# oval-group/GNN_branching

Hardware: NVIDIA B200
Metric: gnn_subdomains_scored_per_sec (higher is better)
Workload: dtype fp16x3 (fp32 accumulate)

## Files before the change

gnn_branching_b200/csrc/gnnb_api.cu:

```cuda
#include <math.h>
#include <stdio.h>
#include <stdlib.h>
#include <string.h>

#include <map>
#include <string>
#include <vector>

#include "gnnb_common.cuh"
#include "gnnb_train.cuh"

using namespace gnnb;

struct gnnb_ctx {
    int device = 0;
    int last_status = 0;
    std::string err;
    int64_t launches = 0;
    int math = GNNB_MATH_TC_FP16X3;
    int chunk = 0;
    int snapshot = 0;
    int fuse = 1;
    int rescore = 0;
    int64_t rescored = 0;
    bool have_gnn = false;
    float* d_gnn = nullptr;
    uint16_t* d_tc = nullptr;
    GnnParams gp{};
    float* d_train = nullptr;
    int64_t n_params = 0;
    size_t po_w[N_LIN] = {0}, po_b[N_LIN] = {0};
    int adam_steps = 0;
    float* train_ws = nullptr;
    size_t train_ws_cap = 0;
    float* kw_ws = nullptr;
    size_t kw_ws_cap = 0;
    int32_t* kw_iscratch = nullptr;
    int kw_iscratch_cap = 0;
    bool have_net = false;
    float* d_net = nullptr;
    std::vector<LayerDev> layers;
    std::vector<PropPlan*> plan_fwd, plan_bwd;
    std::vector<PropPlan*> plan_kw_own;
    std::vector<PropPlan*> plan_kw;
    std::vector<int> n;
    int zero_tap_layer = 0;
    std::vector<LayerTiling> tiling;
    std::vector<RowMap> rowmap;
    int32_t* d_maps = nullptr;
    LayerDev* d_layers = nullptr;
    int32_t* d_hidden_off = nullptr;
    int32_t* d_random_order = nullptr;
    const float** d_ptrs = nullptr;
    std::vector<int> hidden_off;
    int n_hidden = 0;
    std::vector<struct gnnb_queue*> queues;
    int ws_cap = 0;
    bool ws_host_staging = false;
    float* d_ws = nullptr;
    std::vector<float*> mu, relax_f, relax_b;
    std::vector<int32_t*> amb_cnt, amb_base, amb_rows;
    float* nb = nullptr;
    float* ws_scores = nullptr;
    float* ws_best = nullptr;
    int32_t* ws_idx = nullptr;
    struct Staging {
        std::vector<float*> inputs;
        float* mask = nullptr;
        float* best = nullptr;
        int32_t* idx = nullptr;
        float* scores = nullptr;
    } stg[2];
    float* res_best = nullptr;
    int32_t* res_idx = nullptr;
    int64_t res_cap = 0;
    cudaStream_t copy_stream = nullptr;
    cudaEvent_t ev_copied[2] = {nullptr, nullptr}, ev_free[2] = {nullptr, nullptr};
    unsigned long long* d_nan = nullptr;
    int32_t* d_resc = nullptr;
    int resc_cap = 0;
    RowGather* d_gather = nullptr;
    size_t gather_cap = 0;
    std::map<std::string, std::pair<float*, int64_t>> snaps;
    int profile = 0;
    struct Pending { int klass; int64_t rows; cudaEvent_t a, b; };
    std::vector<Pending> pending;
    std::vector<cudaEvent_t> ev_pool;
    double prof_ms[GNNB_K_COUNT] = {0};
    int64_t prof_launches[GNNB_K_COUNT] = {0};
    int64_t prof_rows[GNNB_K_COUNT] = {0};
};

struct gnnb_queue {
    gnnb_ctx* ctx;
    DomainQueue* q;
};

namespace {

int fail(gnnb_ctx* c, int status, const std::string& msg) {
    if (c) { c->last_status = status; c->err = msg; }
    return status;
}

int axis_taps(int i, int ksize, int stride, int pad, int n_out) {
    int t = 0;
    for (int k = 0; k < ksize; ++k) {
        const int a = i + pad - k;
        if (a >= 0 && a % stride == 0 && a / stride < n_out) ++t;
    }
    return t;
}

int first_zero_tap_layer(const std::vector<LayerDev>& layers) {
    for (size_t k = 1; k < layers.size(); ++k) {
        const LayerDev& L = layers[k];
        if (L.kind != GNNB_LAYER_CONV) continue;
        for (int y = 0; y < L.h_in; ++y)
            if (axis_taps(y, L.ksize, L.stride, L.pad, L.h_out) == 0) return (int)k + 1;
        for (int x = 0; x < L.w_in; ++x)
            if (axis_taps(x, L.ksize, L.stride, L.pad, L.w_out) == 0) return (int)k + 1;
    }
    return 0;
}

int check_zero_taps(gnnb_ctx* c) {
    if (!c->zero_tap_layer) return GNNB_OK;
    return fail(c, GNNB_ERR_UNSUPPORTED, "layer " + std::to_string(c->zero_tap_layer) +
                " (conv, stride > kernel) has input positions no tap reaches: the GNN's tap-count normalisation divides by zero");
}

template <class F>
void walk_inputs(const gnnb_frontier& fr, GnnInputs& in, const std::vector<int>& n, F f) {
    const int L = (int)n.size() - 2;
    auto at = [](const float* const* table, int k) { return table ? table[k] : nullptr; };
    for (int k = 0; k <= L + 1; ++k) {
        f(at(fr.lb, k), in.lb[k], (int64_t)n[k]);
        f(at(fr.ub, k), in.ub[k], (int64_t)n[k]);
    }
    for (int k = 0; k < L; ++k) {
        f(at(fr.dual, k), in.dual[k], (int64_t)n[k + 1] * 3);
        f(at(fr.prim_pre, k), in.pre[k], (int64_t)n[k + 1]);
        f(at(fr.prim_post, k), in.post[k], (int64_t)n[k + 1]);
    }
    f(fr.prim_out, in.pout, (int64_t)1);
    f(fr.primal_input, in.pin, (int64_t)n[0]);
    f(fr.wp, in.wp, (int64_t)n[L]);
    f(fr.bp, in.bp, (int64_t)1);
}

int frontier_inputs(gnnb_ctx* ctx, const gnnb_frontier* fr, bool mask, GnnInputs* out) {
    bool ok = !mask || fr->mask;
    walk_inputs(*fr, *out, ctx->n, [&](const float* src, const float*& slot, int64_t) { slot = src; ok = ok && src; });
    return ok ? GNNB_OK : fail(ctx, GNNB_ERR_INVALID, "null frontier array");
}

#define CU(call)                                                                                          \
    do {                                                                                                  \
        cudaError_t e__ = (call);                                                                         \
        if (e__ != cudaSuccess)                                                                           \
            return fail(ctx, GNNB_ERR_CUDA, std::string(#call) + ": " + cudaGetErrorString(e__));         \
    } while (0)

size_t align4(size_t x) { return (x + 3) & ~size_t(3); }

void free_workspace(gnnb_ctx* c) {
    if (c->d_ws) cudaFree(c->d_ws);
    c->d_ws = nullptr;
    c->ws_cap = 0;
    for (auto& kv : c->snaps) cudaFree(kv.second.first);
    c->snaps.clear();
}

int ensure_workspace(gnnb_ctx* ctx, int Bc, bool host_staging) {
    if (ctx->d_ws && ctx->ws_cap >= Bc && (ctx->ws_host_staging || !host_staging)) return GNNB_OK;
    free_workspace(ctx);
    const int L = (int)ctx->layers.size();
    int nmax = 0;
    for (int k = 0; k <= L; ++k) nmax = ctx->n[k] > nmax ? ctx->n[k] : nmax;
    size_t total = 0;
    auto take = [&](size_t elems) { size_t off = total; total += (elems + 63) & ~size_t(63); return off; };
    std::vector<size_t> o_mu(L + 2), o_rf(L + 1), o_rb(L + 1), o_lb(L + 2), o_ub(L + 2), o_du(L), o_pr(L), o_po(L);
    auto wrows = [&](int k) { return (size_t)Bc * (k <= L ? (size_t)ctx->rowmap[k].nslots : 128); };
    for (int k = 0; k <= L + 1; ++k) o_mu[k] = take(wrows(k) * P);
    for (int k = 1; k <= L; ++k) { o_rf[k] = take(wrows(k) * P); o_rb[k] = take(wrows(k) * P); }
    std::vector<size_t> o_ac(L + 1), o_ab(L + 1), o_ar(L + 1);
    for (int k = 1; k <= L; ++k) {
        const size_t rows = wrows(k), nt = rows / 128;
        o_ac[k] = take(nt + 1); o_ab[k] = take(nt + 1); o_ar[k] = take(rows);
    }
    size_t nb_rows = 0;
    for (int k = 0; k <= L; ++k) nb_rows = wrows(k) > nb_rows ? wrows(k) : nb_rows;
    const size_t o_nb = take(nb_rows * P);
    const size_t o_sc = take((size_t)Bc * ctx->n_hidden);
    const size_t o_best = take(Bc), o_idx = take(Bc);
    struct StgOff { std::vector<size_t> inputs; size_t mask, best, idx, sc; } so[2];
    if (host_staging) {
        GnnInputs unused(L);
        for (StgOff& o : so) {
            walk_inputs(gnnb_frontier{}, unused, ctx->n, [&](const float*, const float*&, int64_t per) {
                o.inputs.push_back(take((size_t)Bc * per));
            });
            o.mask = take((size_t)Bc * ctx->n_hidden);
            o.best = take((size_t)Bc * GNNB_TOPK_MAX); o.idx = take((size_t)Bc * GNNB_TOPK_MAX);
            o.sc = take((size_t)Bc * ctx->n_hidden);
        }
    }
    CU(cudaMalloc(&ctx->d_ws, total * sizeof(float)));
    float* base = ctx->d_ws;
    ctx->mu.assign(L + 2, nullptr); ctx->relax_f.assign(L + 1, nullptr); ctx->relax_b.assign(L + 1, nullptr);
    for (int k = 0; k <= L + 1; ++k) ctx->mu[k] = base + o_mu[k];
    for (int k = 1; k <= L; ++k) { ctx->relax_f[k] = base + o_rf[k]; ctx->relax_b[k] = base + o_rb[k]; }
    ctx->amb_cnt.assign(L + 1, nullptr); ctx->amb_base.assign(L + 1, nullptr); ctx->amb_rows.assign(L + 1, nullptr);
    for (int k = 1; k <= L; ++k) {
        ctx->amb_cnt[k] = reinterpret_cast<int32_t*>(base + o_ac[k]);
        ctx->amb_base[k] = reinterpret_cast<int32_t*>(base + o_ab[k]);
        ctx->amb_rows[k] = reinterpret_cast<int32_t*>(base + o_ar[k]);
    }
    ctx->nb = base + o_nb; ctx->ws_scores = base + o_sc; ctx->ws_best = base + o_best;
    ctx->ws_idx = reinterpret_cast<int32_t*>(base + o_idx);
    if (host_staging) {
        for (int i = 0; i < 2; ++i) {
            gnnb_ctx::Staging& g = ctx->stg[i];
            const StgOff& o = so[i];
            g.inputs.clear();
            for (size_t off : o.inputs) g.inputs.push_back(base + off);
            g.mask = base + o.mask;
            g.best = base + o.best; g.idx = reinterpret_cast<int32_t*>(base + o.idx); g.scores = base + o.sc;
        }
        if (!ctx->copy_stream) {
            CU(cudaStreamCreateWithFlags(&ctx->copy_stream, cudaStreamNonBlocking));
            for (int i = 0; i < 2; ++i) {
                CU(cudaEventCreateWithFlags(&ctx->ev_copied[i], cudaEventDisableTiming));
                CU(cudaEventCreateWithFlags(&ctx->ev_free[i], cudaEventDisableTiming));
            }
        }
    }
    ctx->ws_cap = Bc;
    ctx->ws_host_staging = host_staging;
    return GNNB_OK;
}

#define TRY_(expr) do { int s__ = (expr); if (s__ != GNNB_OK) return s__; } while (0)

int snap(gnnb_ctx* ctx, bool on, const std::string& name, const float* src, int64_t numel, cudaStream_t st) {
    if (!on) return GNNB_OK;
    auto it = ctx->snaps.find(name);
    if (it == ctx->snaps.end() || it->second.second < numel) {
        if (it != ctx->snaps.end()) cudaFree(it->second.first);
        float* p = nullptr;
        CU(cudaMalloc(&p, (size_t)numel * sizeof(float)));
        ctx->snaps[name] = std::make_pair(p, numel);
        it = ctx->snaps.find(name);
    }
    it->second.second = numel;
    CU(cudaMemcpyAsync(it->second.first, src, (size_t)numel * sizeof(float), cudaMemcpyDeviceToDevice, st));
    return GNNB_OK;
}

cudaEvent_t prof_event(gnnb_ctx* ctx) {
    if (!ctx->ev_pool.empty()) { cudaEvent_t e = ctx->ev_pool.back(); ctx->ev_pool.pop_back(); return e; }
    cudaEvent_t e = nullptr;
    cudaEventCreate(&e);
    return e;
}

struct ProfScope {
    gnnb_ctx* ctx; cudaStream_t st; cudaEvent_t a = nullptr, b = nullptr; int klass; int64_t rows;
    ProfScope(gnnb_ctx* c, int k, int64_t r, cudaStream_t s) : ctx(c), st(s), klass(k), rows(r) {
        if (ctx->profile) { a = prof_event(ctx); b = prof_event(ctx); cudaEventRecord(a, st); }
    }
    ~ProfScope() {
        if (ctx->profile) { cudaEventRecord(b, st); ctx->pending.push_back({klass, rows, a, b}); }
    }
};

int prof_collect(gnnb_ctx* ctx) {
    if (ctx->pending.empty()) return GNNB_OK;
    CU(cudaDeviceSynchronize());
    for (auto& p : ctx->pending) {
        float ms = 0.f;
        if (cudaEventElapsedTime(&ms, p.a, p.b) == cudaSuccess) {
            ctx->prof_ms[p.klass] += ms;
            ctx->prof_launches[p.klass] += 1;
            ctx->prof_rows[p.klass] += p.rows;
        }
        ctx->ev_pool.push_back(p.a);
        ctx->ev_pool.push_back(p.b);
    }
    ctx->pending.clear();
    return GNNB_OK;
}

int snap_img(gnnb_ctx* ctx, bool on, const std::string& name, const float* img, int k, int Bc, bool piece_major, cudaStream_t st) {
    if (!on) return GNNB_OK;
    const int64_t numel = (int64_t)Bc * ctx->n[k] * P;
    if (ctx->math != GNNB_MATH_TC_FP16X3) return snap(ctx, on, name, img, numel, st);
    TRY_(snap(ctx, on, name, img, numel, st));
    tc_unpack_tile_image(img, ctx->snaps[name].first, ctx->rowmap[k], (int64_t)Bc * ctx->rowmap[k].nslots, piece_major, st);
    return GNNB_OK;
}

#define TRY(expr) do { int s__ = (expr); if (s__ != GNNB_OK) return s__; } while (0)

int run_chunk(gnnb_ctx* ctx, const GnnInputs& in, const float* mask, int Bc, int math, const NanDoms& nd, float* scores, int k,
              float* best_score, int32_t* best_idx, gnnb_winner* winners, cudaStream_t st) {
    const int L = (int)ctx->layers.size();
    const GnnParams& g = ctx->gp;
    const bool tc = math == GNNB_MATH_TC_FP16X3;
    const bool snaps = ctx->snapshot && math == ctx->math;
    int64_t* lc = &ctx->launches;
    auto name = [](const char* fmt, int a, int b) { char buf[64]; snprintf(buf, sizeof buf, fmt, a, b); return std::string(buf); };

    auto R = [&](int k) { return (int64_t)Bc * (tc ? ctx->rowmap[k].nslots : ctx->n[k]); };
    const RowMap nomap{nullptr, 0, 0};
    auto M = [&](int k) { return tc ? ctx->rowmap[k] : nomap; };
    const bool fused = tc && ctx->fuse;

    const bool amb_all = tc && L <= AMB_MAX_LAYERS;
    if (amb_all) {
        ProfScope ps(ctx, GNNB_K_RELAX, 0, st);
        AmbLayers al{};
        al.n = L;
        for (int k = 1; k <= L; ++k) {
            al.lb[k - 1] = in.lb[k]; al.ub[k - 1] = in.ub[k]; al.map[k - 1] = M(k); al.rows[k - 1] = R(k);
            al.cnt[k - 1] = ctx->amb_cnt[k]; al.base[k - 1] = ctx->amb_base[k]; al.out_rows[k - 1] = ctx->amb_rows[k];
        }
        amb_compact_all(al, st, lc);
    }
    {
        std::vector<NodeInputs> nis(L + 1);
        for (int k = 1; k <= L; ++k)
            nis[k] = NodeInputs{in.lb[k], in.ub[k], in.dual[k - 1], in.pre[k - 1], in.post[k - 1], ctx->layers[k - 1].bias_node,
                                ctx->n[k], R(k), ctx->amb_rows[k], ctx->amb_base[k], M(k)};
        if (tc) {
            for (int k0 = 1; k0 <= L; k0 += AMB_MAX_LAYERS) {
                const int nl = (L - k0 + 1) < AMB_MAX_LAYERS ? (L - k0 + 1) : AMB_MAX_LAYERS;
                int64_t nodes = 0;
                for (int k = k0; k < k0 + nl; ++k) {
                    nodes += (int64_t)Bc * ctx->n[k];
                    if (!amb_all) amb_compact(in.lb[k], in.ub[k], M(k), nis[k].rows, ctx->amb_cnt[k], ctx->amb_base[k], ctx->amb_rows[k], st, lc);
                }
                ProfScope ps(ctx, GNNB_K_RELAX, nodes, st);
                tc_relax(g, &nis[k0], &ctx->relax_f[k0], &ctx->relax_b[k0], nl, st, lc);
            }
        }
        for (int k = 1; k <= L; ++k) {
            if (!tc) {
                ProfScope ps(ctx, GNNB_K_RELAX, (int64_t)Bc * ctx->n[k], st);
                simt_relax(g, nis[k], ctx->relax_f[k], ctx->relax_b[k], st, lc);
            }
            TRY(snap(ctx, snaps, name(tc ? "relaxp_f%d" : "relax_f%d", k, 0), ctx->relax_f[k], (int64_t)Bc * ctx->n[k] * P, st));
            TRY(snap(ctx, snaps, name(tc ? "relaxp_b%d" : "relax_b%d", k, 0), ctx->relax_b[k], (int64_t)Bc * ctx->n[k] * P, st));
        }
    }
    {
        ProfScope ps(ctx, GNNB_K_INPUT_EMBED, (int64_t)Bc * ctx->n[0], st);
        if (tc) tc_input_embed(g, in.lb[0], in.pin, in.ub[0], ctx->mu[0], M(0), R(0), st, lc);
        else simt_input_embed(g, in.lb[0], in.pin, in.ub[0], ctx->mu[0], R(0), st, lc);
    }
    TRY(snap_img(ctx, snaps, "mu0_embed", ctx->mu[0], 0, Bc, false, st));

    for (int t = 0; t < g.T; ++t) {
        const bool last = (t == g.T - 1);
        for (int k = 1; k <= L; ++k) {
            const int64_t rows = R(k), nodes = (int64_t)Bc * ctx->n[k];
            if (fused) {
                ProfScope ps(ctx, GNNB_K_LAYER_FWD, nodes, st);
                tc_fused(g, ctx->plan_fwd[k - 1], ctx->mu[k - 1], false, in.lb[k], in.ub[k], ctx->relax_f[k], ctx->amb_base[k],
                         ctx->mu[k], nullptr, M(k), 0, 0, rows, ctx->d_nan, nd, ctx->snapshot ? ctx->nb : nullptr, false, st, lc);
            } else {
                ProfScope ps(ctx, GNNB_K_PROP_FWD, nodes, st);
                if (tc) prop_tc_run(ctx->plan_fwd[k - 1], ctx->mu[k - 1], ctx->nb, Bc, st, lc);
                else prop_forward(ctx->layers[k - 1], ctx->mu[k - 1], ctx->nb, Bc, st, lc);
            }
            TRY(snap_img(ctx, snaps, name("t%d_fwd_nb%d", t, k), ctx->nb, k, Bc, true, st));
            if (!fused) {
                ProfScope ps(ctx, GNNB_K_UPDATE_FWD, nodes, st);
                if (tc) tc_update(g, false, in.lb[k], in.ub[k], ctx->nb, ctx->relax_f[k], ctx->amb_base[k], ctx->mu[k], nullptr, M(k), 0, 0, rows, ctx->d_nan, nd, st, lc);
                else simt_update(g, false, in.lb[k], in.ub[k], ctx->nb, ctx->relax_f[k], ctx->mu[k], nullptr, ctx->n[k], 0, 0, rows, ctx->d_nan, st, lc);
            }
            TRY(snap_img(ctx, snaps, name("t%d_fwd_mu%d", t, k), ctx->mu[k], k, Bc, false, st));
        }
        {
            ProfScope ps(ctx, GNNB_K_OUTPUT, Bc, st);
            output_node(g, in.wp, in.bp, ctx->mu[L], tc, tc ? ctx->rowmap[L].nslots : ctx->n[L], in.lb[L + 1], in.ub[L + 1], in.pout,
                        ctx->mu[L + 1], ctx->n[L], Bc, st, lc);
        }
        TRY(snap(ctx, snaps, name("t%d_mu_out", t, 0), ctx->mu[L + 1], (int64_t)Bc * P, st));
        for (int k = L; k >= 1; --k) {
            const int64_t rows = R(k), nodes = (int64_t)Bc * ctx->n[k];
            float* sc = last ? scores : nullptr;
            float* mu_k = (last && k == 1 && tc && !ctx->snapshot) ? nullptr : ctx->mu[k];
            const bool fused_k = fused && k < L;
            if (fused_k) {
                ProfScope ps(ctx, last ? GNNB_K_LAYER_BWD_SCORE : GNNB_K_LAYER_BWD, nodes, st);
                tc_fused(g, ctx->plan_bwd[k], ctx->mu[k + 1], true, in.lb[k], in.ub[k], ctx->relax_b[k], ctx->amb_base[k],
                         mu_k, sc, M(k), ctx->n_hidden, ctx->hidden_off[k], rows, ctx->d_nan, nd, ctx->snapshot ? ctx->nb : nullptr, false, st, lc);
            } else {
                ProfScope ps(ctx, GNNB_K_PROP_BWD, nodes, st);
                if (k == L && tc) prop_tc_property_backward(in.wp, ctx->mu[L + 1], ctx->nb, ctx->n[L], ctx->rowmap[L].nslots, Bc, st, lc);
                else if (k == L) prop_property_backward(in.wp, ctx->mu[L + 1], ctx->nb, ctx->n[L], Bc, st, lc);
                else if (tc) prop_tc_run(ctx->plan_bwd[k], ctx->mu[k + 1], ctx->nb, Bc, st, lc);
                else prop_backward(ctx->layers[k], ctx->mu[k + 1], ctx->nb, Bc, true, st, lc);
            }
            TRY(snap_img(ctx, snaps, name("t%d_bwd_nb%d", t, k), ctx->nb, k, Bc, true, st));
            if (!fused_k) {
                ProfScope ps(ctx, last ? GNNB_K_UPDATE_BWD_SCORE : GNNB_K_UPDATE_BWD, nodes, st);
                if (tc) tc_update(g, true, in.lb[k], in.ub[k], ctx->nb, ctx->relax_b[k], ctx->amb_base[k], mu_k, sc, M(k), ctx->n_hidden, ctx->hidden_off[k], rows, ctx->d_nan, nd, st, lc);
                else simt_update(g, true, in.lb[k], in.ub[k], ctx->nb, ctx->relax_b[k], ctx->mu[k], sc, ctx->n[k], ctx->n_hidden, ctx->hidden_off[k], rows, ctx->d_nan, st, lc);
            }
            TRY(snap_img(ctx, snaps, name("t%d_bwd_mu%d", t, k), ctx->mu[k], k, Bc, false, st));
        }
        if (!last && fused) {
            ProfScope ps(ctx, GNNB_K_INPUT_UPDATE, (int64_t)Bc * ctx->n[0], st);
            tc_fused(g, ctx->plan_bwd[0], ctx->mu[1], true, in.lb[0], in.ub[0], nullptr, nullptr, ctx->mu[0], nullptr, M(0), 0, 0, R(0),
                     ctx->d_nan, nd, nullptr, true, st, lc);
            TRY(snap_img(ctx, snaps, name("t%d_mu0", t, 0), ctx->mu[0], 0, Bc, false, st));
        } else if (!last) {
            {
                ProfScope ps(ctx, GNNB_K_PROP_BWD, (int64_t)Bc * ctx->n[0], st);
                if (tc) prop_tc_run(ctx->plan_bwd[0], ctx->mu[1], ctx->nb, Bc, st, lc);
                else prop_backward(ctx->layers[0], ctx->mu[1], ctx->nb, Bc, false, st, lc);
            }
            {
                ProfScope ps(ctx, GNNB_K_INPUT_UPDATE, (int64_t)Bc * ctx->n[0], st);
                if (tc) tc_input_update(g, in.lb[0], in.ub[0], ctx->nb, ctx->mu[0], M(0), R(0), st, lc);
                else simt_input_update(g, in.lb[0], in.ub[0], ctx->nb, ctx->mu[0], R(0), st, lc);
            }
            TRY(snap_img(ctx, snaps, name("t%d_mu0", t, 0), ctx->mu[0], 0, Bc, false, st));
        }
    }
    {
        ProfScope ps(ctx, GNNB_K_ARGMAX, Bc, st);
        if (k == 1) masked_argmax(scores, mask, ctx->n_hidden, Bc, best_score, best_idx, winners, st, lc);
        else masked_topk(scores, mask, ctx->n_hidden, Bc, k, best_score, best_idx, st, lc);
    }
    CU(cudaGetLastError());
    return GNNB_OK;
}

int ensure_nan_doms(gnnb_ctx* ctx, int B) {
    if (ctx->resc_cap >= B) return GNNB_OK;
    if (ctx->d_resc) { cudaFree(ctx->d_resc); ctx->d_resc = nullptr; ctx->resc_cap = 0; }
    CU(cudaMalloc(&ctx->d_resc, (1 + 2 * (size_t)B) * sizeof(int32_t)));
    CU(cudaMemset(ctx->d_resc, 0, (1 + 2 * (size_t)B) * sizeof(int32_t)));
    ctx->resc_cap = B;
    return GNNB_OK;
}

int ensure_kw_iscratch(gnnb_ctx* ctx, int B, cudaStream_t st) {
    if (ctx->kw_iscratch_cap >= B) return GNNB_OK;
    if (ctx->kw_iscratch) { CU(cudaStreamSynchronize(st)); cudaFree(ctx->kw_iscratch); ctx->kw_iscratch = nullptr; ctx->kw_iscratch_cap = 0; }
    CU(cudaMalloc(&ctx->kw_iscratch, (3 * (size_t)B + 1) * sizeof(int32_t)));
    ctx->kw_iscratch_cap = B;
    return GNNB_OK;
}

NanDoms nan_doms(gnnb_ctx* ctx) { return NanDoms{ctx->d_resc, ctx->d_resc + 1, ctx->d_resc + 1 + ctx->resc_cap, 0}; }

void reset_nan_doms(gnnb_ctx* ctx, cudaStream_t st) {
    cudaStreamSynchronize(st);
    cudaMemset(ctx->d_resc, 0, (1 + 2 * (size_t)ctx->resc_cap) * sizeof(int32_t));
}

int rescore_flagged(gnnb_ctx* ctx, const gnnb_frontier* in, int chunk, int k, float* best, int32_t* idx, gnnb_winner* winners,
                    float* scores, cudaStream_t st) {
    const bool host = in->mem == GNNB_MEM_HOST;
    const int nh = ctx->n_hidden;
    const NanDoms nd = nan_doms(ctx);
    int32_t count = 0;
    CU(cudaMemcpyAsync(&count, nd.count, sizeof count, cudaMemcpyDeviceToHost, st));
    CU(cudaStreamSynchronize(st));
    ctx->rescored = count;
    if (count == 0) return GNNB_OK;
    std::vector<int32_t> rows;
    if (host) {
        rows.resize(count);
        CU(cudaMemcpyAsync(rows.data(), nd.list, (size_t)count * sizeof(int32_t), cudaMemcpyDeviceToHost, st));
        CU(cudaStreamSynchronize(st));
    }
    CU(cudaMemsetAsync(nd.count, 0, sizeof(int32_t), st));
    CU(cudaMemsetAsync(ctx->d_nan, 0, sizeof(unsigned long long), st));
    gnnb_ctx::Staging& sg = ctx->stg[0];
    std::vector<RowGather> tab;
    GnnInputs cp((int)ctx->layers.size());
    walk_inputs(*in, cp, ctx->n, [&](const float* src, const float*& slot, int64_t per) {
        float* dst = sg.inputs[tab.size()];
        tab.push_back(RowGather{src, dst, per});
        slot = dst;
    });
    tab.push_back(RowGather{in->mask, sg.mask, nh});
    if (!host) {
        if (ctx->gather_cap < tab.size()) {
            if (ctx->d_gather) cudaFree(ctx->d_gather);
            ctx->d_gather = nullptr; ctx->gather_cap = 0;
            CU(cudaMalloc(&ctx->d_gather, tab.size() * sizeof(RowGather)));
            ctx->gather_cap = tab.size();
        }
        CU(cudaMemcpyAsync(ctx->d_gather, tab.data(), tab.size() * sizeof(RowGather), cudaMemcpyHostToDevice, st));
    }
    for (int s0 = 0, Bs = 0; s0 < count; s0 += Bs) {
        Bs = (count - s0) < chunk ? (count - s0) : chunk;
        if (host) {
            for (int i = 0; i < Bs; ++i)
                for (const RowGather& t : tab)
                    CU(cudaMemcpyAsync(t.dst + i * t.per, t.src + rows[s0 + i] * t.per, t.per * sizeof(float), cudaMemcpyHostToDevice, st));
        } else {
            gather_rows(ctx->d_gather, (int)tab.size(), nd.list + s0, Bs, st, &ctx->launches);
        }
        TRY(run_chunk(ctx, cp, sg.mask, Bs, GNNB_MATH_SIMT_FP32, NanDoms{nullptr, nullptr, nullptr, 0}, sg.scores, k, sg.best, sg.idx, nullptr, st));
        scatter_rescored(nd.list + s0, Bs, k, sg.best, sg.idx, sg.scores, nh, best, idx, winners, host ? nullptr : scores, nd.flag, st,
                         &ctx->launches);
        if (host && scores)
            for (int i = 0; i < Bs; ++i)
                CU(cudaMemcpyAsync(scores + (size_t)rows[s0 + i] * nh, sg.scores + (size_t)i * nh, (size_t)nh * sizeof(float),
                                   cudaMemcpyDeviceToHost, st));
    }
    CU(cudaEventRecord(ctx->ev_free[0], st));
    CU(cudaGetLastError());
    return GNNB_OK;
}

int upload_gnn(gnnb_ctx* ctx, const float* const* tensors, int T) {
    std::vector<size_t> o_w(N_LIN), o_b(N_LIN);
    size_t total = 0;
    for (int l = 0; l < N_LIN; ++l) {
        o_w[l] = total; total += align4((size_t)lin_in(l) * lin_out(l));
        o_b[l] = total; total += align4(lin_out(l));
    }
    std::vector<float> blob(total, 0.f);
    for (int l = 0; l < N_LIN; ++l) {
        const int K = lin_in(l), N = lin_out(l);
        const float* W = tensors[2 * l];
        for (int nn = 0; nn < N; ++nn)
            for (int k = 0; k < K; ++k) blob[o_w[l] + (size_t)k * N + nn] = W[(size_t)nn * K + k];
        memcpy(&blob[o_b[l]], tensors[2 * l + 1], sizeof(float) * N);
    }
    std::vector<float> cw((size_t)N_TCLIN * P * P, 0.f), cb((size_t)N_TCLIN * P, 0.f);
    auto compose = [&](int id, int outer, int half, int inner, bool add_outer_bias) {
        const float* Wo = tensors[2 * outer];
        const float* bo = tensors[2 * outer + 1];
        const int Ko = lin_in(outer);
        for (int nn = 0; nn < P; ++nn) {
            double bacc = add_outer_bias ? (double)bo[nn] : 0.0;
            for (int k = 0; k < P; ++k) {
                double acc = 0.0;
                if (inner < 0) acc = Wo[(size_t)nn * Ko + half * P + k];
                else
                    for (int j = 0; j < P; ++j) acc += (double)Wo[(size_t)nn * Ko + half * P + j] * (double)tensors[2 * inner][(size_t)j * P + k];
                cw[((size_t)id * P + nn) * P + k] = (float)acc;
            }
            if (inner >= 0)
                for (int j = 0; j < P; ++j) bacc += (double)Wo[(size_t)nn * Ko + half * P + j] * (double)tensors[2 * inner + 1][j];
            cb[(size_t)id * P + nn] = (float)bacc;
        }
    };
    compose(T_FWD_R, FC4, 0, FC1_1, false);
    compose(T_FWD_C, FC4, 1, FC3_2, true);
    compose(T_BWD_R, BC4, 0, BC2_1, false);
    compose(T_BWD_C, BC4, 1, BC3_1, true);
    compose(T_INP_C, INP_B2, 0, INP_B_1, true);
    compose(T_INP_NB, INP_B2, 1, -1, false);
    std::vector<size_t> o_tc(N_LIN, 0);
    size_t tc_total = 0;
    for (int l = 0; l < N_LIN; ++l)
        if (lin_in(l) >= P && lin_out(l) == P) { o_tc[l] = tc_total; tc_total += (size_t)tc_packed_elems(lin_in(l)); }
    std::vector<size_t> o_tcx(N_TCLIN, 0);
    for (int i = 0; i < N_TCLIN; ++i) { o_tcx[i] = tc_total; tc_total += (size_t)tc_packed_elems(P); }
    std::vector<uint16_t> tcblob(tc_total ? tc_total : 1, 0);
    for (int l = 0; l < N_LIN; ++l)
        if (lin_in(l) >= P && lin_out(l) == P) tc_pack_weight(tensors[2 * l], lin_in(l), &tcblob[o_tc[l]]);
    for (int i = 0; i < N_TCLIN; ++i) tc_pack_weight(&cw[(size_t)i * P * P], P, &tcblob[o_tcx[i]]);
    const size_t o_cb = total;
    total += cb.size();
    blob.resize(total, 0.f);
    memcpy(&blob[o_cb], cb.data(), cb.size() * sizeof(float));
    CU(cudaDeviceSynchronize());
    if (!ctx->d_gnn) CU(cudaMalloc(&ctx->d_gnn, total * sizeof(float)));
    if (!ctx->d_tc) CU(cudaMalloc(&ctx->d_tc, tcblob.size() * sizeof(uint16_t)));
    CU(cudaMemcpy(ctx->d_gnn, blob.data(), total * sizeof(float), cudaMemcpyHostToDevice));
    CU(cudaMemcpy(ctx->d_tc, tcblob.data(), tcblob.size() * sizeof(uint16_t), cudaMemcpyHostToDevice));
    for (int l = 0; l < N_LIN; ++l) {
        ctx->gp.wt[l] = ctx->d_gnn + o_w[l];
        ctx->gp.bias[l] = ctx->d_gnn + o_b[l];
        ctx->gp.tc[l] = (lin_in(l) >= P && lin_out(l) == P) ? ctx->d_tc + o_tc[l] : nullptr;
    }
    for (int i = 0; i < N_TCLIN; ++i) {
        ctx->gp.tcx_w[i] = ctx->d_tc + o_tcx[i];
        ctx->gp.tcx_b[i] = ctx->d_gnn + o_cb + (size_t)i * P;
    }
    ctx->gp.T = T;
    if (!ctx->d_train) {
        size_t np = 0;
        for (int l = 0; l < N_LIN; ++l) {
            ctx->po_w[l] = np; np += align4((size_t)lin_in(l) * lin_out(l));
            ctx->po_b[l] = np; np += align4(lin_out(l));
        }
        ctx->n_params = (int64_t)np;
        CU(cudaMalloc(&ctx->d_train, 4 * np * sizeof(float)));
        CU(cudaMemset(ctx->d_train, 0, 4 * np * sizeof(float)));
        ctx->adam_steps = 0;
    }
    {
        std::vector<float> master((size_t)ctx->n_params, 0.f);
        for (int l = 0; l < N_LIN; ++l) {
            memcpy(&master[ctx->po_w[l]], tensors[2 * l], sizeof(float) * lin_in(l) * lin_out(l));
            memcpy(&master[ctx->po_b[l]], tensors[2 * l + 1], sizeof(float) * lin_out(l));
        }
        CU(cudaMemcpy(ctx->d_train, master.data(), master.size() * sizeof(float), cudaMemcpyHostToDevice));
    }
    ctx->have_gnn = true;
    return GNNB_OK;
}

TrainParams train_params(gnnb_ctx* ctx) {
    TrainParams tp;
    float* grad = ctx->d_train + ctx->n_params;
    for (int l = 0; l < N_LIN; ++l) {
        tp.w[l] = ctx->d_train + ctx->po_w[l]; tp.b[l] = ctx->d_train + ctx->po_b[l];
        tp.dw[l] = grad + ctx->po_w[l]; tp.db[l] = grad + ctx->po_b[l];
    }
    return tp;
}

int download_quarter(gnnb_ctx* ctx, int quarter, float* const* tensors, const int64_t* numels, int n_tensors) {
    if (!ctx || !tensors || !numels) return fail(ctx, GNNB_ERR_INVALID, "null argument");
    if (!ctx->have_gnn) return fail(ctx, GNNB_ERR_STATE, "gnnb_set_gnn_weights must be called first");
    if (n_tensors != 2 * N_LIN) return fail(ctx, GNNB_ERR_INVALID, "expected 52 tensors (weight, bias of 26 linears)");
    for (int l = 0; l < N_LIN; ++l)
        if (numels[2 * l] != (int64_t)lin_in(l) * lin_out(l) || numels[2 * l + 1] != lin_out(l))
            return fail(ctx, GNNB_ERR_INVALID, "tensor " + std::to_string(2 * l) + " has the wrong number of elements");
    CU(cudaSetDevice(ctx->device));
    CU(cudaDeviceSynchronize());
    std::vector<float> host((size_t)ctx->n_params);
    CU(cudaMemcpy(host.data(), ctx->d_train + (size_t)quarter * ctx->n_params, host.size() * sizeof(float), cudaMemcpyDeviceToHost));
    for (int l = 0; l < N_LIN; ++l) {
        memcpy(tensors[2 * l], &host[ctx->po_w[l]], sizeof(float) * lin_in(l) * lin_out(l));
        memcpy(tensors[2 * l + 1], &host[ctx->po_b[l]], sizeof(float) * lin_out(l));
    }
    return GNNB_OK;
}

}

extern "C" {

int gnnb_abi_version(void) { return 1; }

int gnnb_create(gnnb_ctx** out, int device) {
    if (!out) return GNNB_ERR_INVALID;
    *out = nullptr;
    gnnb_ctx* ctx = new gnnb_ctx();
    ctx->device = device;
    cudaError_t e = cudaSetDevice(device);
    if (e != cudaSuccess) { delete ctx; return GNNB_ERR_CUDA; }
    cudaDeviceProp prop;
    e = cudaGetDeviceProperties(&prop, device);
    if (e != cudaSuccess) { delete ctx; return GNNB_ERR_CUDA; }
    if (prop.major != 10) {
        fprintf(stderr, "libgnnb: device %d is sm_%d%d; this library is built for sm_100a (B200) only\n", device, prop.major, prop.minor);
        delete ctx;
        return GNNB_ERR_UNSUPPORTED;
    }
    if (cudaMalloc(&ctx->d_nan, sizeof(unsigned long long)) != cudaSuccess ||
        cudaMemset(ctx->d_nan, 0, sizeof(unsigned long long)) != cudaSuccess ||
        simt_init() != 0 || prop_init(64 * 1024) != 0 || tc_init() != 0 || prop_tc_init() != 0 || kw_init() != 0 || train_init() != 0) {
        fprintf(stderr, "libgnnb: initialisation failed: %s\n", cudaGetErrorString(cudaGetLastError()));
        if (ctx->d_nan) cudaFree(ctx->d_nan);
        delete ctx;
        return GNNB_ERR_CUDA;
    }
    *out = ctx;
    return GNNB_OK;
}

void gnnb_destroy(gnnb_ctx* ctx) {
    if (!ctx) return;
    cudaSetDevice(ctx->device);
    free_workspace(ctx);
    if (ctx->d_gnn) cudaFree(ctx->d_gnn);
    if (ctx->d_tc) cudaFree(ctx->d_tc);
    if (ctx->d_train) cudaFree(ctx->d_train);
    if (ctx->train_ws) cudaFree(ctx->train_ws);
    if (ctx->kw_ws) cudaFree(ctx->kw_ws);
    if (ctx->kw_iscratch) cudaFree(ctx->kw_iscratch);
    if (ctx->d_net) cudaFree(ctx->d_net);
    if (ctx->d_maps) cudaFree(ctx->d_maps);
    if (ctx->d_layers) cudaFree(ctx->d_layers);
    if (ctx->d_hidden_off) cudaFree(ctx->d_hidden_off);
    if (ctx->d_random_order) cudaFree(ctx->d_random_order);
    if (ctx->d_ptrs) cudaFree(ctx->d_ptrs);
    if (ctx->d_nan) cudaFree(ctx->d_nan);
    if (ctx->d_resc) cudaFree(ctx->d_resc);
    if (ctx->d_gather) cudaFree(ctx->d_gather);
    for (PropPlan* p : ctx->plan_fwd) prop_plan_free(p);
    for (PropPlan* p : ctx->plan_bwd) prop_plan_free(p);
    for (PropPlan* p : ctx->plan_kw_own) prop_plan_free(p);
    if (ctx->copy_stream) cudaStreamDestroy(ctx->copy_stream);
    if (ctx->res_best) cudaFree(ctx->res_best);
    if (ctx->res_idx) cudaFree(ctx->res_idx);
    for (int i = 0; i < 2; ++i) { if (ctx->ev_copied[i]) cudaEventDestroy(ctx->ev_copied[i]); if (ctx->ev_free[i]) cudaEventDestroy(ctx->ev_free[i]); }
    for (auto& p : ctx->pending) { cudaEventDestroy(p.a); cudaEventDestroy(p.b); }
    for (auto e : ctx->ev_pool) cudaEventDestroy(e);
    for (gnnb_queue* q : ctx->queues) q->ctx = nullptr;
    delete ctx;
}

int gnnb_set_gnn_weights(gnnb_ctx* ctx, const float* const* tensors, const int64_t* numels, int n_tensors, int T, int p) {
    if (!ctx || !tensors || !numels) return fail(ctx, GNNB_ERR_INVALID, "null argument");
    if (p != P) return fail(ctx, GNNB_ERR_UNSUPPORTED, "embedding size p must be 64");
    if (T < 1) return fail(ctx, GNNB_ERR_INVALID, "T must be >= 1");
    if (n_tensors != 2 * N_LIN) return fail(ctx, GNNB_ERR_INVALID, "expected 52 tensors (weight, bias of 26 linears)");
    for (int l = 0; l < N_LIN; ++l) {
        if (numels[2 * l] != (int64_t)lin_in(l) * lin_out(l) || numels[2 * l + 1] != lin_out(l))
            return fail(ctx, GNNB_ERR_INVALID, "tensor " + std::to_string(2 * l) + " has the wrong number of elements");
    }
    CU(cudaSetDevice(ctx->device));
    return upload_gnn(ctx, tensors, T);
}

int gnnb_set_network(gnnb_ctx* ctx, const gnnb_layer_desc* layers, int n_layers, int c0, int h0, int w0) {
    if (!ctx || !layers || n_layers < 1) return fail(ctx, GNNB_ERR_INVALID, "null argument");
    if (!ctx->queues.empty()) return fail(ctx, GNNB_ERR_STATE, "gnnb_set_network while domain queues of the previous network exist");
    CU(cudaSetDevice(ctx->device));
    std::vector<LayerDev> devs(n_layers);
    std::vector<int> n(n_layers + 2);
    n[0] = c0 * h0 * w0;
    int pc = c0, ph = h0, pw = w0;
    bool flat = false;
    size_t total = 0;
    std::vector<size_t> o_w(n_layers), o_b(n_layers);
    for (int k = 0; k < n_layers; ++k) {
        const gnnb_layer_desc& d = layers[k];
        LayerDev& L = devs[k];
        L.kind = d.kind;
        L.c_in = d.c_in; L.h_in = d.h_in; L.w_in = d.w_in; L.c_out = d.c_out; L.h_out = d.h_out; L.w_out = d.w_out;
        L.ksize = d.ksize; L.stride = d.stride; L.pad = d.pad;
        L.n_in = d.c_in * d.h_in * d.w_in;
        L.n_out = d.c_out * d.h_out * d.w_out;
        if (!d.weight || !d.bias) return fail(ctx, GNNB_ERR_INVALID, "layer weight/bias is null");
        if (L.n_in != n[k]) return fail(ctx, GNNB_ERR_INVALID, "layer " + std::to_string(k) + ": input size does not match the previous layer");
        size_t wn;
        if (d.kind == GNNB_LAYER_CONV) {
            if (flat || d.c_in != pc || d.h_in != ph || d.w_in != pw) return fail(ctx, GNNB_ERR_INVALID, "conv layer input shape mismatch");
            if (d.ksize < 1 || d.stride < 1 || d.pad < 0) return fail(ctx, GNNB_ERR_INVALID, "bad conv geometry");
            if (d.h_out != (d.h_in + 2 * d.pad - d.ksize) / d.stride + 1 || d.w_out != (d.w_in + 2 * d.pad - d.ksize) / d.stride + 1)
                return fail(ctx, GNNB_ERR_INVALID, "conv output shape mismatch");
            if ((d.h_out - 1) * d.stride - 2 * d.pad + d.ksize != d.h_in || (d.w_out - 1) * d.stride - 2 * d.pad + d.ksize != d.w_in)
                return fail(ctx, GNNB_ERR_UNSUPPORTED, "conv geometry needs output_padding in the backward pass");
            if ((size_t)d.c_in * d.ksize * d.ksize * d.c_out * sizeof(float) > 64 * 1024)
                return fail(ctx, GNNB_ERR_UNSUPPORTED, "conv weights exceed the 64 KB shared-memory staging buffer");
            wn = (size_t)d.c_out * d.c_in * d.ksize * d.ksize;
            pc = d.c_out; ph = d.h_out; pw = d.w_out;
        } else if (d.kind == GNNB_LAYER_LINEAR) {
            if (d.h_in != 1 || d.w_in != 1 || d.h_out != 1 || d.w_out != 1) return fail(ctx, GNNB_ERR_INVALID, "linear layers use c_in/c_out only");
            wn = (size_t)L.n_out * L.n_in;
            flat = true;
        } else {
            return fail(ctx, GNNB_ERR_INVALID, "unknown layer kind");
        }
        n[k + 1] = L.n_out;
        o_w[k] = total; total += align4(wn);
        o_b[k] = total; total += align4(L.n_out);
    }
    n[n_layers + 1] = 1;
    std::vector<float> blob(total, 0.f);
    for (int k = 0; k < n_layers; ++k) {
        const gnnb_layer_desc& d = layers[k];
        const LayerDev& L = devs[k];
        const size_t wn = d.kind == GNNB_LAYER_CONV ? (size_t)d.c_out * d.c_in * d.ksize * d.ksize : (size_t)L.n_out * L.n_in;
        memcpy(&blob[o_w[k]], d.weight, wn * sizeof(float));
        const int per = d.kind == GNNB_LAYER_CONV ? d.h_out * d.w_out : 1;
        for (int j = 0; j < L.n_out; ++j) blob[o_b[k] + j] = d.bias[j / per];
    }
    struct Staged {
        float* d_net = nullptr;
        int32_t* d_maps = nullptr;
        LayerDev* d_layers = nullptr;
        int32_t *d_hidden_off = nullptr, *d_random_order = nullptr;
        const float** d_ptrs = nullptr;
        std::vector<PropPlan*> plan_fwd, plan_bwd, plan_kw_own;
        bool keep = false;
        ~Staged() {
            if (keep) return;
            if (d_net) cudaFree(d_net);
            if (d_maps) cudaFree(d_maps);
            if (d_layers) cudaFree(d_layers);
            if (d_hidden_off) cudaFree(d_hidden_off);
            if (d_random_order) cudaFree(d_random_order);
            if (d_ptrs) cudaFree(d_ptrs);
            for (PropPlan* p : plan_fwd) prop_plan_free(p);
            for (PropPlan* p : plan_bwd) prop_plan_free(p);
            for (PropPlan* p : plan_kw_own) prop_plan_free(p);
        }
    } sg;
    CU(cudaMalloc(&sg.d_net, total * sizeof(float)));
    CU(cudaMemcpy(sg.d_net, blob.data(), total * sizeof(float), cudaMemcpyHostToDevice));
    for (int k = 0; k < n_layers; ++k) { devs[k].weight = sg.d_net + o_w[k]; devs[k].bias_node = sg.d_net + o_b[k]; }
    sg.plan_fwd.assign(n_layers, nullptr);
    sg.plan_bwd.assign(n_layers, nullptr);
    sg.plan_kw_own.assign(n_layers, nullptr);
    std::vector<LayerTiling> tiling(n_layers + 1);
    std::vector<RowMap> rowmap(n_layers + 1, RowMap{nullptr, 0, 0});
    tiling[0] = make_tiling(c0, h0, w0);
    for (int k = 0; k < n_layers; ++k)
        tiling[k + 1] = devs[k].kind == GNNB_LAYER_CONV ? make_tiling(devs[k].c_out, devs[k].h_out, devs[k].w_out)
                                                       : make_tiling(devs[k].n_out, 1, 1);
    {
        size_t total_slots = 0;
        for (const LayerTiling& t : tiling) total_slots += t.node_of_slot.size();
        CU(cudaMalloc(&sg.d_maps, total_slots * sizeof(int32_t)));
        size_t off = 0;
        for (int k = 0; k <= n_layers; ++k) {
            const LayerTiling& t = tiling[k];
            CU(cudaMemcpy(sg.d_maps + off, t.node_of_slot.data(), t.node_of_slot.size() * sizeof(int32_t), cudaMemcpyHostToDevice));
            rowmap[k] = RowMap{sg.d_maps + off, n[k], (int)t.node_of_slot.size()};
            off += t.node_of_slot.size();
        }
    }
    for (int k = 0; k < n_layers; ++k) {
        sg.plan_fwd[k] = prop_plan_build(devs[k], layers[k].weight, false, false, tiling[k + 1], tiling[k]);
        sg.plan_bwd[k] = prop_plan_build(devs[k], layers[k].weight, true, k > 0, tiling[k], tiling[k + 1]);
        if (!sg.plan_fwd[k] || !sg.plan_bwd[k]) return fail(ctx, GNNB_ERR_CUDA, "building the propagation plans failed");
        if (k > 0 && devs[k].kind == GNNB_LAYER_CONV) {
            sg.plan_kw_own[k] = prop_plan_build(devs[k], layers[k].weight, true, false, tiling[k], tiling[k + 1]);
            if (!sg.plan_kw_own[k]) return fail(ctx, GNNB_ERR_CUDA, "building the propagation plans failed");
        }
    }
    std::vector<int> hidden_off(n_layers + 2, 0);
    int n_hidden = 0;
    for (int k = 1; k <= n_layers; ++k) { hidden_off[k] = n_hidden; n_hidden += n[k]; }
    CU(cudaMalloc(&sg.d_layers, n_layers * sizeof(LayerDev)));
    CU(cudaMemcpy(sg.d_layers, devs.data(), n_layers * sizeof(LayerDev), cudaMemcpyHostToDevice));
    CU(cudaMalloc(&sg.d_hidden_off, (n_layers + 1) * sizeof(int32_t)));
    CU(cudaMemcpy(sg.d_hidden_off, hidden_off.data() + 1, (n_layers + 1) * sizeof(int32_t), cudaMemcpyHostToDevice));
    CU(cudaMalloc(&sg.d_random_order, n_layers * sizeof(int32_t)));
    CU(cudaMalloc(&sg.d_ptrs, 2 * (n_layers + 2) * sizeof(float*)));
    CU(cudaDeviceSynchronize());
    ctx->have_net = false;
    free_workspace(ctx);
    if (ctx->d_net) cudaFree(ctx->d_net);
    if (ctx->d_maps) cudaFree(ctx->d_maps);
    if (ctx->d_layers) cudaFree(ctx->d_layers);
    if (ctx->d_hidden_off) cudaFree(ctx->d_hidden_off);
    if (ctx->d_random_order) cudaFree(ctx->d_random_order);
    if (ctx->d_ptrs) cudaFree(ctx->d_ptrs);
    for (PropPlan* p : ctx->plan_fwd) prop_plan_free(p);
    for (PropPlan* p : ctx->plan_bwd) prop_plan_free(p);
    for (PropPlan* p : ctx->plan_kw_own) prop_plan_free(p);
    sg.keep = true;
    ctx->d_net = sg.d_net; ctx->d_maps = sg.d_maps; ctx->d_layers = sg.d_layers; ctx->d_hidden_off = sg.d_hidden_off;
    ctx->d_random_order = sg.d_random_order; ctx->d_ptrs = sg.d_ptrs;
    ctx->plan_fwd = sg.plan_fwd; ctx->plan_bwd = sg.plan_bwd; ctx->plan_kw_own = sg.plan_kw_own;
    ctx->plan_kw.assign(n_layers, nullptr);
    for (int k = 0; k < n_layers; ++k) ctx->plan_kw[k] = sg.plan_kw_own[k] ? sg.plan_kw_own[k] : sg.plan_bwd[k];
    ctx->tiling = tiling; ctx->rowmap = rowmap;
    ctx->layers = devs;
    ctx->n = n;
    ctx->zero_tap_layer = first_zero_tap_layer(devs);
    ctx->hidden_off = hidden_off;
    ctx->n_hidden = n_hidden;
    ctx->have_net = true;
    return GNNB_OK;
}

int gnnb_set_option(gnnb_ctx* ctx, const char* key, int64_t value) {
    if (!ctx || !key) return fail(ctx, GNNB_ERR_INVALID, "null argument");
    const std::string k(key);
    if (k == "math") {
        if (value != GNNB_MATH_TC_FP16X3 && value != GNNB_MATH_SIMT_FP32) return fail(ctx, GNNB_ERR_INVALID, "unknown math mode");
        if (value == GNNB_MATH_TC_FP16X3 && !tc_available()) return fail(ctx, GNNB_ERR_UNSUPPORTED, "tensor-core path not built");
        ctx->math = (int)value;
    } else if (k == "chunk") {
        if (value < 0) return fail(ctx, GNNB_ERR_INVALID, "chunk must be >= 0");
        ctx->chunk = (int)value;
    } else if (k == "fuse") {
        ctx->fuse = value ? 1 : 0;
    } else if (k == "snapshot") {
        ctx->snapshot = value ? 1 : 0;
    } else if (k == "profile") {
        ctx->profile = value ? 1 : 0;
    } else if (k == "rescore") {
        ctx->rescore = value ? 1 : 0;
    } else {
        return fail(ctx, GNNB_ERR_INVALID, "unknown option " + k);
    }
    return GNNB_OK;
}

int64_t gnnb_get_option(gnnb_ctx* ctx, const char* key) {
    if (!ctx || !key) return -1;
    const std::string k(key);
    if (k == "math") return ctx->math;
    if (k == "chunk") return ctx->chunk;
    if (k == "snapshot") return ctx->snapshot;
    if (k == "fuse") return ctx->fuse;
    if (k == "profile") return ctx->profile;
    if (k == "rescore") return ctx->rescore;
    if (k == "rescored") return ctx->rescored;
    if (k == "n_hidden") return ctx->n_hidden;
    if (k == "workspace_domains") return ctx->ws_cap;
    if (k.rfind("plan_density_pct_", 0) == 0) {
        const bool bwd = k[17] == 'b';
        const size_t i = (size_t)atoi(k.c_str() + 18);
        const auto& v = bwd ? ctx->plan_bwd : ctx->plan_fwd;
        return i < v.size() ? (int64_t)(100.0 * prop_plan_density(v[i])) : -1;
    }
    return -1;
}

static int score_impl(gnnb_ctx* ctx, const gnnb_frontier* in, int k, float* best_score, int32_t* best_idx, gnnb_winner* winners,
                      float* scores, void* stream) {
    if (!ctx || !in || ((!best_score || !best_idx) && !winners)) return fail(ctx, GNNB_ERR_INVALID, "null argument");
    if (!ctx->have_gnn || !ctx->have_net) return fail(ctx, GNNB_ERR_STATE, "gnnb_set_gnn_weights and gnnb_set_network must be called first");
    if (in->B < 0) return fail(ctx, GNNB_ERR_INVALID, "negative batch");
    ctx->rescored = 0;
    TRY(check_zero_taps(ctx));
    if (in->B == 0) return GNNB_OK;
    GnnInputs cp((int)ctx->layers.size());
    TRY(frontier_inputs(ctx, in, true, &cp));
    CU(cudaSetDevice(ctx->device));
    cudaStream_t st = (cudaStream_t)stream;
    const bool host = in->mem == GNNB_MEM_HOST;
    int chunk = ctx->chunk > 0 ? ctx->chunk : 1024;
    if (chunk > in->B) chunk = in->B;
    const bool resc = ctx->rescore && ctx->math == GNNB_MATH_TC_FP16X3;
    TRY(ensure_workspace(ctx, chunk, host || resc));
    NanDoms nd{nullptr, nullptr, nullptr, 0};
    if (resc) {
        TRY(ensure_nan_doms(ctx, in->B));
        nd = nan_doms(ctx);
    }
    const int64_t n_res = (int64_t)in->B * k;
    if (host && !winners && ctx->res_cap < n_res) {
        if (ctx->res_best) cudaFree(ctx->res_best);
        if (ctx->res_idx) cudaFree(ctx->res_idx);
        ctx->res_best = nullptr; ctx->res_idx = nullptr; ctx->res_cap = 0;
        CU(cudaMalloc(&ctx->res_best, (size_t)n_res * sizeof(float)));
        CU(cudaMalloc(&ctx->res_idx, (size_t)n_res * sizeof(int32_t)));
        ctx->res_cap = n_res;
    }

    int wave = 0, ramp = host ? (chunk < 128 ? chunk : 128) : chunk;
    for (int c0 = 0, Bc = 0; c0 < in->B; c0 += Bc, ++wave) {
        Bc = (in->B - c0) < ramp ? (in->B - c0) : ramp;
        ramp = ramp + ramp / 2 > chunk ? chunk : ramp + ramp / 2;
        gnnb_ctx::Staging& sg = ctx->stg[wave & 1];
        cudaStream_t cs = host ? ctx->copy_stream : st;
        if (host) CU(cudaStreamWaitEvent(cs, ctx->ev_free[wave & 1], 0));
        auto stage = [&](const float* src, float* dst, size_t per_domain) -> const float* {
            const float* p = src + (size_t)c0 * per_domain;
            if (!host) return p;
            cudaMemcpyAsync(dst, p, (size_t)Bc * per_domain * sizeof(float), cudaMemcpyHostToDevice, cs);
            return dst;
        };
        size_t a = 0;
        walk_inputs(*in, cp, ctx->n, [&](const float* src, const float*& slot, int64_t per) {
            slot = stage(src, host ? sg.inputs[a++] : nullptr, per);
        });
        const float* mask = stage(in->mask, sg.mask, ctx->n_hidden);
        CU(cudaGetLastError());
        if (host) {
            CU(cudaEventRecord(ctx->ev_copied[wave & 1], cs));
            CU(cudaStreamWaitEvent(st, ctx->ev_copied[wave & 1], 0));
        }

        float* d_scores = host ? sg.scores : (scores ? scores + (size_t)c0 * ctx->n_hidden : ctx->ws_scores);
        float* d_best = winners ? nullptr : (host ? ctx->res_best : best_score) + (size_t)c0 * k;
        int32_t* d_idx = winners ? nullptr : (host ? ctx->res_idx : best_idx) + (size_t)c0 * k;
        {
            nd.dom0 = c0;
            const int rc = run_chunk(ctx, cp, mask, Bc, ctx->math, nd, d_scores, k, d_best, d_idx, winners ? winners + c0 : nullptr, st);
            if (rc != GNNB_OK) {
                if (host) cudaStreamSynchronize(ctx->copy_stream);
                cudaStreamSynchronize(st);
                if (resc) reset_nan_doms(ctx, st);
                return rc;
            }
        }
        if (host) {
            if (scores)
                CU(cudaMemcpyAsync(scores + (size_t)c0 * ctx->n_hidden, d_scores, (size_t)Bc * ctx->n_hidden * sizeof(float),
                                   cudaMemcpyDeviceToHost, st));
            CU(cudaEventRecord(ctx->ev_free[wave & 1], st));
        }
    }
    if (resc) {
        const int rc = rescore_flagged(ctx, in, chunk, k, winners ? nullptr : (host ? ctx->res_best : best_score),
                                       winners ? nullptr : (host ? ctx->res_idx : best_idx), winners, scores, st);
        if (rc != GNNB_OK) {
            reset_nan_doms(ctx, st);
            return rc;
        }
    }
    if (host) {
        if (!winners) {
            CU(cudaMemcpyAsync(best_score, ctx->res_best, (size_t)n_res * sizeof(float), cudaMemcpyDeviceToHost, st));
            CU(cudaMemcpyAsync(best_idx, ctx->res_idx, (size_t)n_res * sizeof(int32_t), cudaMemcpyDeviceToHost, st));
        }
        return gnnb_check(ctx, stream, nullptr);
    }
    return GNNB_OK;
}

int gnnb_score(gnnb_ctx* ctx, const gnnb_frontier* in, float* best_score, int32_t* best_idx, float* scores, void* stream) {
    if (!best_score || !best_idx) return fail(ctx, GNNB_ERR_INVALID, "null argument");
    return score_impl(ctx, in, 1, best_score, best_idx, nullptr, scores, stream);
}

int gnnb_score_winners(gnnb_ctx* ctx, const gnnb_frontier* in, gnnb_winner* winners, float* scores, void* stream) {
    if (!winners) return fail(ctx, GNNB_ERR_INVALID, "null argument");
    if (in && in->mem == GNNB_MEM_HOST && scores) return fail(ctx, GNNB_ERR_INVALID, "dense scores of a HOST frontier: use gnnb_score");
    return score_impl(ctx, in, 1, nullptr, nullptr, winners, scores, stream);
}

int gnnb_score_topk(gnnb_ctx* ctx, const gnnb_frontier* in, int32_t k, float* top_score, int32_t* top_idx, float* scores, void* stream) {
    if (k < 1 || k > GNNB_TOPK_MAX) return fail(ctx, GNNB_ERR_INVALID, "k must be in [1, GNNB_TOPK_MAX]");
    if (!top_score || !top_idx) return fail(ctx, GNNB_ERR_INVALID, "null argument");
    return score_impl(ctx, in, k, top_score, top_idx, nullptr, scores, stream);
}

int gnnb_topk(gnnb_ctx* ctx, int32_t B, int32_t n, const float* scores, const float* mask, int32_t k, float* top_score,
              int32_t* top_idx, void* stream) {
    if (!ctx) return GNNB_ERR_INVALID;
    if (k < 1 || k > GNNB_TOPK_MAX) return fail(ctx, GNNB_ERR_INVALID, "k must be in [1, GNNB_TOPK_MAX]");
    if (!scores || !top_score || !top_idx) return fail(ctx, GNNB_ERR_INVALID, "null argument");
    if (B < 0 || n < 0) return fail(ctx, GNNB_ERR_INVALID, "negative size");
    if (B == 0) return GNNB_OK;
    CU(cudaSetDevice(ctx->device));
    cudaStream_t st = (cudaStream_t)stream;
    {
        ProfScope ps(ctx, GNNB_K_ARGMAX, B, st);
        masked_topk(scores, mask, n, B, k, top_score, top_idx, st, &ctx->launches);
    }
    CU(cudaGetLastError());
    return GNNB_OK;
}

int gnnb_babsr(gnnb_ctx* ctx, const gnnb_frontier* in, int32_t sparsest_layer, float decision_threshold,
               const int32_t* random_order, const int32_t* icp_counter_in, int32_t* decision, int32_t* icp_counter_out,
               int32_t* kind, float* scores, void* stream) {
    if (!ctx || !in || !random_order || !decision || !icp_counter_out) return fail(ctx, GNNB_ERR_INVALID, "null argument");
    if (!ctx->have_net) return fail(ctx, GNNB_ERR_STATE, "gnnb_set_network must be called first");
    if (in->B < 0) return fail(ctx, GNNB_ERR_INVALID, "negative batch");
    if (in->B == 0) return GNNB_OK;
    if (!in->lb || !in->ub || !in->wp || !in->mask) return fail(ctx, GNNB_ERR_INVALID, "null frontier field");
    const int L = (int)ctx->layers.size(), B = in->B;
    if (L > babsr_max_layers()) return fail(ctx, GNNB_ERR_UNSUPPORTED, "too many layers for the BaBSR kernel");
    CU(cudaSetDevice(ctx->device));
    cudaStream_t st = (cudaStream_t)stream;
    const bool host = in->mem == GNNB_MEM_HOST;
    const std::vector<int>& n = ctx->n;
    int nmax = 0;
    for (int k = 0; k <= L; ++k) nmax = n[k] > nmax ? n[k] : nmax;
    float* tmp = nullptr;
    std::vector<const float*> ptrs(2 * (L + 2), nullptr);
    const float *d_wp = in->wp, *d_mask = in->mask;
    const int32_t* d_cin = icp_counter_in;
    int32_t *d_dec = decision, *d_cout = icp_counter_out, *d_kind = kind;
    float* d_scores = scores;
    if (host) {
        size_t total = 0;
        auto take = [&](size_t elems) { size_t o = total; total += align4(elems); return o; };
        std::vector<size_t> o_lb(L + 2), o_ub(L + 2);
        for (int k = 1; k <= L; ++k) { o_lb[k] = take((size_t)B * n[k]); o_ub[k] = take((size_t)B * n[k]); }
        const size_t o_wp = take((size_t)B * n[L]), o_mask = take((size_t)B * ctx->n_hidden), o_cin = take(B), o_dec = take(2 * (size_t)B),
                     o_cout = take(B), o_kind = take(B), o_sc = take(scores ? (size_t)B * ctx->n_hidden : 0);
        CU(cudaMalloc(&tmp, total * sizeof(float)));
        auto up = [&](size_t off, const void* src, size_t elems) {
            cudaMemcpyAsync(tmp + off, src, elems * sizeof(float), cudaMemcpyHostToDevice, st);
            return tmp + off;
        };
        for (int k = 1; k <= L; ++k) {
            if (!in->lb[k] || !in->ub[k]) { cudaFree(tmp); return fail(ctx, GNNB_ERR_INVALID, "null bound array"); }
            ptrs[k] = up(o_lb[k], in->lb[k], (size_t)B * n[k]);
            ptrs[L + 2 + k] = up(o_ub[k], in->ub[k], (size_t)B * n[k]);
        }
        d_wp = up(o_wp, in->wp, (size_t)B * n[L]);
        d_mask = up(o_mask, in->mask, (size_t)B * ctx->n_hidden);
        d_cin = icp_counter_in ? reinterpret_cast<const int32_t*>(up(o_cin, icp_counter_in, B)) : nullptr;
        d_dec = reinterpret_cast<int32_t*>(tmp + o_dec); d_cout = reinterpret_cast<int32_t*>(tmp + o_cout);
        d_kind = kind ? reinterpret_cast<int32_t*>(tmp + o_kind) : nullptr;
        d_scores = scores ? tmp + o_sc : nullptr;
    } else {
        for (int k = 1; k <= L; ++k) {
            if (!in->lb[k] || !in->ub[k]) return fail(ctx, GNNB_ERR_INVALID, "null bound array");
            ptrs[k] = in->lb[k];
            ptrs[L + 2 + k] = in->ub[k];
        }
    }
    cudaError_t e = cudaMemcpyAsync(ctx->d_ptrs, ptrs.data(), ptrs.size() * sizeof(float*), cudaMemcpyHostToDevice, st);
    if (e == cudaSuccess) e = cudaMemcpyAsync(ctx->d_random_order, random_order, L * sizeof(int32_t), cudaMemcpyHostToDevice, st);
    int rc = 0;
    if (e == cudaSuccess)
        rc = babsr_run(ctx->d_layers, L, ctx->n_hidden, nmax, ctx->d_ptrs, ctx->d_ptrs + (L + 2), d_wp, d_mask, ctx->d_hidden_off,
                       ctx->d_random_order, d_cin, sparsest_layer, decision_threshold, d_dec, d_cout, d_kind, d_scores, B, st,
                       &ctx->launches);
    if (e == cudaSuccess && rc == 0 && host) {
        cudaMemcpyAsync(decision, d_dec, 2 * (size_t)B * sizeof(int32_t), cudaMemcpyDeviceToHost, st);
        cudaMemcpyAsync(icp_counter_out, d_cout, (size_t)B * sizeof(int32_t), cudaMemcpyDeviceToHost, st);
        if (kind) cudaMemcpyAsync(kind, d_kind, (size_t)B * sizeof(int32_t), cudaMemcpyDeviceToHost, st);
        if (scores) cudaMemcpyAsync(scores, d_scores, (size_t)B * ctx->n_hidden * sizeof(float), cudaMemcpyDeviceToHost, st);
        e = cudaStreamSynchronize(st);
    }
    if (tmp) { cudaStreamSynchronize(st); cudaFree(tmp); }
    if (e != cudaSuccess) return fail(ctx, GNNB_ERR_CUDA, std::string("gnnb_babsr: ") + cudaGetErrorString(e));
    if (rc != 0) return fail(ctx, GNNB_ERR_UNSUPPORTED, "a layer is too large for the BaBSR kernel's shared-memory buffers");
    CU(cudaGetLastError());
    return GNNB_OK;
}

int gnnb_score_grad(gnnb_ctx* ctx, const gnnb_frontier* in, int32_t n_terms, const int32_t* term_domain, const int32_t* term_index,
                    const float* term_coeff, float* term_scores, void* stream) {
    if (!ctx || !in || !term_domain || !term_index || !term_coeff) return fail(ctx, GNNB_ERR_INVALID, "null argument");
    if (!ctx->have_gnn || !ctx->have_net) return fail(ctx, GNNB_ERR_STATE, "gnnb_set_gnn_weights and gnnb_set_network must be called first");
    if (in->B < 1 || n_terms < 1) return fail(ctx, GNNB_ERR_INVALID, "need at least one subdomain and one term");
    TRY(check_zero_taps(ctx));
    GnnInputs ti((int)ctx->layers.size());
    TRY(frontier_inputs(ctx, in, false, &ti));
    for (int i = 0; i < n_terms; ++i)
        if (term_domain[i] < 0 || term_domain[i] >= in->B || term_index[i] < 0 || term_index[i] >= ctx->n_hidden)
            return fail(ctx, GNNB_ERR_INVALID, "term " + std::to_string(i) + " is out of range");
    CU(cudaSetDevice(ctx->device));
    cudaStream_t st = (cudaStream_t)stream;
    const int B = in->B;
    float* tmp = nullptr;
    if (in->mem == GNNB_MEM_HOST) {
        size_t total = 0;
        walk_inputs(*in, ti, ctx->n, [&](const float*, const float*&, int64_t per) { total += align4((size_t)B * per); });
        CU(cudaMalloc(&tmp, total * sizeof(float)));
        float* dst = tmp;
        walk_inputs(*in, ti, ctx->n, [&](const float* src, const float*& slot, int64_t per) {
            cudaMemcpyAsync(dst, src, (size_t)B * per * sizeof(float), cudaMemcpyHostToDevice, st);
            slot = dst;
            dst += align4((size_t)B * per);
        });
    }
    cudaMemsetAsync(ctx->d_train + ctx->n_params, 0, (size_t)ctx->n_params * sizeof(float), st);
    std::string err;
    const int rc = train_backward(ctx->gp, train_params(ctx), ctx->layers, ctx->n, ctx->hidden_off, ti, B, n_terms, term_domain, term_index,
                                  term_coeff, term_scores, &ctx->train_ws, &ctx->train_ws_cap, st, &ctx->launches, &err);
    if (tmp) { cudaStreamSynchronize(st); cudaFree(tmp); }
    if (rc != GNNB_OK) return fail(ctx, rc, err);
    return GNNB_OK;
}

int gnnb_get_gradients(gnnb_ctx* ctx, float* const* tensors, const int64_t* numels, int n_tensors) {
    return download_quarter(ctx, 1, tensors, numels, n_tensors);
}

int gnnb_get_gnn_weights(gnnb_ctx* ctx, float* const* tensors, const int64_t* numels, int n_tensors) {
    return download_quarter(ctx, 0, tensors, numels, n_tensors);
}

// ... 291 lines not shown
```

gnn_branching_b200/csrc/gnnb_common.cuh:

```cuda
#pragma once

#include <cuda_runtime.h>
#include <stdint.h>

#include <string>
#include <vector>

#include "../../include/gnnb.h"

namespace gnnb {

constexpr int P = 64;

enum Lin : int {
    INP_F = 0, INP_F_1, INP_B, INP_B_1, INP_B2, INP_B2_2, FC1, FC1_1, FC3, FC3_2, FC4, FC4_2,
    OUT1, OUT2, OUT3, BC1, BC1_1, BC1_2, BC2, BC2_1, BC3, BC3_1, BC4, BC4_1, FNODE, FSCORE, N_LIN
};

__host__ __device__ constexpr int lin_in(int l) {
    return l == INP_F ? 3 : l == INP_B ? 2 : (l == FC1 || l == BC1) ? 7 : l == OUT1 ? 4
         : (l == INP_B2 || l == FC3 || l == FC4 || l == OUT2 || l == BC3 || l == BC4) ? 2 * P
         : l == BC2 ? 3 * P : P;
}
__host__ __device__ constexpr int lin_out(int l) { return l == FSCORE ? 1 : P; }

enum TcLin : int {
    T_FWD_R = 0,
    T_FWD_C,
    T_BWD_R,
    T_BWD_C,
    T_INP_C,
    T_INP_NB,
    N_TCLIN
};

struct GnnParams {
    const float* wt[N_LIN];
    const float* bias[N_LIN];
    const uint16_t* tc[N_LIN];
    const uint16_t* tcx_w[N_TCLIN];
    const float* tcx_b[N_TCLIN];
    int T;
};

struct LayerDev {
    int kind;
    int c_in, h_in, w_in, c_out, h_out, w_out, ksize, stride, pad;
    int n_in, n_out;
    const float* weight;
    const float* bias_node;
};

struct RowMap {
    const int32_t* node_of_slot;
    int n;
    int nslots;
};
__device__ __forceinline__ int64_t natural_row(const RowMap& m, int64_t grow) {
    const int64_t b = grow / m.nslots;
    const int node = __ldg(m.node_of_slot + (grow - b * m.nslots));
    return node < 0 ? -1 : b * m.n + node;
}
struct LayerTiling {
    std::vector<int32_t> node_of_slot, slot_of_node;
    int ntiles = 0;
};
LayerTiling make_tiling(int C, int H, int W);

struct NodeInputs {
    const float* lb;
    const float* ub;
    const float* dual;
    const float* prim_pre;
    const float* prim_post;
    const float* bias_node;
    int n;
    int64_t rows;
    const int32_t* amb_rows;
    const int32_t* amb_base;
    RowMap map;
};

struct NanDoms {
    int32_t* count;
    int32_t* flag;
    int32_t* list;
    int dom0;
};

void simt_relax(const GnnParams& g, const NodeInputs& in, float* relax_f, float* relax_b, cudaStream_t st, int64_t* launches);
void simt_update(const GnnParams& g, bool backward, const float* lb, const float* ub, const float* nb, const float* relax,
                 float* mu_out, float* scores , int n, int64_t score_stride, int64_t score_off, int64_t rows,
                 unsigned long long* nan_count, cudaStream_t st, int64_t* launches);
void simt_input_embed(const GnnParams& g, const float* lb0, const float* x, const float* ub0, float* mu0, int64_t rows,
                      cudaStream_t st, int64_t* launches);
void simt_input_update(const GnnParams& g, const float* lb0, const float* ub0, const float* nb, float* mu0, int64_t rows,
                       cudaStream_t st, int64_t* launches);

int simt_init();

void tc_relax(const GnnParams& g, const NodeInputs* in, float* const* relax_f, float* const* relax_b, int n_layers, cudaStream_t st,
              int64_t* launches);
void tc_update(const GnnParams& g, bool backward, const float* lb, const float* ub, const float* nb, const float* relax,
               const int32_t* amb_base, float* mu_out, float* scores, RowMap map, int64_t score_stride, int64_t score_off, int64_t rows,
               unsigned long long* nan_count, const NanDoms& nan_doms, cudaStream_t st, int64_t* launches);
struct PropPlan;
void tc_fused(const GnnParams& g, const PropPlan* plan, const float* mu_in, bool backward, const float* lb, const float* ub,
              const float* relax, const int32_t* amb_base, float* mu_out, float* scores, RowMap map, int64_t score_stride, int64_t score_off,
              int64_t rows, unsigned long long* nan_count, const NanDoms& nan_doms, float* nb_dbg, bool input_layer, cudaStream_t st,
              int64_t* launches);
void amb_compact(const float* lb, const float* ub, RowMap map, int64_t rows, int32_t* cnt, int32_t* amb_base, int32_t* amb_rows,
                 cudaStream_t st, int64_t* launches);
constexpr int AMB_MAX_LAYERS = 16;
struct AmbLayers {
    const float* lb[AMB_MAX_LAYERS];
    const float* ub[AMB_MAX_LAYERS];
    RowMap map[AMB_MAX_LAYERS];
    int64_t rows[AMB_MAX_LAYERS];
    int32_t* cnt[AMB_MAX_LAYERS];
    int32_t* base[AMB_MAX_LAYERS];
    int32_t* out_rows[AMB_MAX_LAYERS];
    int tile0[AMB_MAX_LAYERS + 1];
    int n;
};
void amb_compact_all(AmbLayers a, cudaStream_t st, int64_t* launches);
void tc_input_embed(const GnnParams& g, const float* lb0, const float* x, const float* ub0, float* mu0, RowMap map, int64_t rows,
                    cudaStream_t st, int64_t* launches);
void tc_input_update(const GnnParams& g, const float* lb0, const float* ub0, const float* nb, float* mu0, RowMap map, int64_t rows,
                     cudaStream_t st, int64_t* launches);
int64_t tc_pack_weight(const float* w_host, int K, uint16_t* dst_host);
int64_t tc_packed_elems(int K);
int tc_init();
bool tc_available();
void tc_unpack_tile_image(const float* img, float* out, RowMap map, int64_t rows, bool piece_major, cudaStream_t st);

int prop_init(int max_smem_bytes);
void prop_forward(const LayerDev& L, const float* mu_prev, float* nb, int Bc, cudaStream_t st, int64_t* launches);
void prop_backward(const LayerDev& L, const float* mu_next, float* nb, int Bc, bool normalise, cudaStream_t st, int64_t* launches);
void prop_property_backward(const float* wp, const float* mu_out, float* nb, int nL, int Bc, cudaStream_t st, int64_t* launches);
void output_node(const GnnParams& g, const float* wp, const float* bp, const float* mu_L, bool mu_image, int mu_stride, const float* lb_out,
                 const float* ub_out, const float* prim_out, float* mu_out, int nL, int Bc, cudaStream_t st, int64_t* launches);
void masked_argmax(const float* scores, const float* mask, int n_hidden, int Bc, float* best_score, int32_t* best_idx,
                   gnnb_winner* winners, cudaStream_t st, int64_t* launches);
void masked_topk(const float* scores, const float* mask, int n, int Bc, int k, float* top_score, int32_t* top_idx, cudaStream_t st,
                 int64_t* launches);
struct RowGather { const float* src; float* dst; int64_t per; };
struct GnnInputs {
    std::vector<const float*> lb, ub;
    std::vector<const float*> dual, pre, post;
    const float *pout = nullptr, *pin = nullptr, *wp = nullptr, *bp = nullptr;
    explicit GnnInputs(int L) : lb(L + 2), ub(L + 2), dual(L), pre(L), post(L) {}
};
void gather_rows(const RowGather* tab, int n_arrays, const int32_t* rows, int n, cudaStream_t st, int64_t* launches);
void scatter_rescored(const int32_t* rows, int n, int k, const float* sub_best, const int32_t* sub_idx, const float* sub_scores,
                      int n_hidden, float* best_score, int32_t* best_idx, gnnb_winner* winners, float* scores, int32_t* flag,
                      cudaStream_t st, int64_t* launches);

struct PropPlan;
int prop_tc_init();
PropPlan* prop_plan_build(const LayerDev& L, const float* host_weight, bool backward, bool normalise, const LayerTiling& out,
                          const LayerTiling& in);
void prop_plan_free(PropPlan* p);
double prop_plan_density(const PropPlan* p);
void prop_tc_run(const PropPlan* plan, const float* mu_in, float* nb_img, int Bc, cudaStream_t st, int64_t* launches);
void prop_tc_property_backward(const float* wp, const float* mu_out, float* nb_img, int nL, int nslots, int Bc, cudaStream_t st, int64_t* launches);

int babsr_max_layers();
int babsr_run(const LayerDev* d_layers, int L, int n_hidden, int nmax, const float* const* d_lb, const float* const* d_ub,
              const float* wp, const float* mask, const int32_t* d_hidden_off, const int32_t* d_random_order,
              const int32_t* counter_in, int sparsest_layer, float threshold, int32_t* decision, int32_t* counter_out,
              int32_t* kind, float* scores, int B, cudaStream_t st, int64_t* launches);

struct DomainQueue;
int queue_create(int device, const std::vector<int>& n, int n_hidden, int64_t capacity, DomainQueue** out, std::string* err);
void queue_destroy(DomainQueue* q);
const std::string& queue_error(const DomainQueue* q);
int64_t queue_size(const DomainQueue* q);
int64_t queue_capacity(const DomainQueue* q);
int queue_global_lb(DomainQueue* q, float* out, cudaStream_t st);
int queue_add(DomainQueue* q, int B, const float* lower, const float* upper, const float* const* lb, const float* const* ub,
              const int8_t* mask, const int32_t* decision, const uint8_t* keep, int32_t* added, cudaStream_t st, int64_t* launches);
int queue_pick(DomainQueue* q, int max_B, float threshold, bool discard, int32_t* picked, float* lower, float* upper, float* const* lb,
               float* const* ub, int8_t* mask, int32_t* decision, cudaStream_t st, int64_t* launches);
int queue_prune(DomainQueue* q, float threshold, cudaStream_t st, int64_t* launches);
float* queue_stage(DomainQueue* q, size_t bytes);

struct KwTc { const std::vector<PropPlan*>* plans; const std::vector<RowMap>* maps; };
int kw_init();
int kw_bounds(const std::vector<LayerDev>& layers, const std::vector<int>& n, int B, const float* x, float eps, const float* wp, const float* bp,
              const float* const* prov_lb, const float* const* prov_ub, float* const* out_lb, float* const* out_ub, const KwTc* tc, float** ws,
              size_t* ws_cap, cudaStream_t st, int64_t* launches, std::string* err);
int child_bounds(const std::vector<LayerDev>& layers, const std::vector<int>& n, int B, const float* x, float eps, const float* wp, const float* bp,
                 const float* const* parent_lb, const float* const* parent_ub, const int32_t* dec_layer, const int32_t* dec_index,
                 const int32_t* choice, float* const* out_lb, float* const* out_ub, int8_t* const* out_mask, int32_t* second_pass,
                 int32_t* iscratch, const KwTc* tc, float** ws, size_t* ws_cap, cudaStream_t st, int64_t* launches, std::string* err);

int root_bounds(const std::vector<LayerDev>& layers, const std::vector<int>& n, int B, const float* x, float eps, const float* wp, const float* bp,
                float* const* out_lb, float* const* out_ub, int8_t* const* out_mask, int32_t* second_pass, int32_t* iscratch, const KwTc* tc,
                float** ws, size_t* ws_cap, cudaStream_t st, int64_t* launches, std::string* err);

struct Ratio { float r0, r1, beta, amb; };
__device__ __forceinline__ Ratio compute_ratio(float l, float u) {
    Ratio r;
    float lt = l - fmaxf(l, 0.0f);
    float ut = fmaxf(u, 0.0f);
    if (u != u) ut = u;
    if (l != l) lt = l;
    r.r0 = __fdiv_rn(ut, __fsub_rn(ut, lt));
    r.beta = __fmul_rn(__fmul_rn(-1.0f, lt), r.r0);
    r.amb = (r.beta > 0.0f) ? 1.0f : 0.0f;
    r.r1 = __fadd_rn(__fmul_rn(__fsub_rn(1.0f, __fmul_rn(2.0f, __fmul_rn(r.r0, r.amb))), r.amb), r.r0);
    return r;
}

}
```

gnn_branching_b200/csrc/gnnb_tc.cu:

```cuda
#include "gnnb_prop_body.cuh"
#include "gnnb_umma.cuh"

namespace gnnb {
namespace {

using namespace tcx;

constexpr uint32_t ACOL = 0, DCOL = 64, WG_COLS = 128;

struct WG {
    uint32_t land;
    uint32_t mbar_mma, mbar_tma;
    uint32_t ph_mma, ph_tma;
    uint32_t tmem;
    uint32_t tmem0;
    uint32_t acol;
    int t;
    int bar_threads;
    int wg;
    bool lead_warp;
};

__device__ __forceinline__ void wg_barrier(const WG& c) { named_bar(1 + c.wg, c.bar_threads); }

__device__ __forceinline__ void issue_ts(const WG& c, uint32_t b_hi, uint32_t b_lo, uint32_t N, uint32_t dcol, bool accumulate) {
    const uint32_t idesc = make_idesc(N);
    const uint32_t d = c.tmem0 + dcol, a = c.tmem0 + c.acol;
#pragma unroll
    for (int pass = 0; pass < 3; ++pass) {
        const uint64_t bd = make_desc(pass == 2 ? b_lo : b_hi);
#pragma unroll
        for (int k = 0; k < 4; ++k)
            umma_ts(d, a + 16 * k + (pass == 1 ? 8 : 0), bd + 2 * k, idesc, (accumulate || pass > 0 || k > 0) ? 1u : 0u);
    }
}
__device__ __forceinline__ void issue_ss(const WG& c, uint32_t b_hi, uint32_t b_lo, uint32_t N, uint32_t dcol, bool accumulate) {
    const uint32_t idesc = make_idesc(N);
    const uint32_t d = c.tmem0 + dcol;
#pragma unroll
    for (int pass = 0; pass < 3; ++pass) {
        const uint64_t ad = make_desc_nosw(pass == 1 ? c.land + APLANE : c.land, NB_PIECE, 128u);
        const uint64_t bd = make_desc(pass == 2 ? b_lo : b_hi);
#pragma unroll
        for (int k = 0; k < 4; ++k)
            umma(d, ad + (uint64_t)(k * ((2 * NB_PIECE) >> 4)), bd + 2 * k, idesc, (accumulate || pass > 0 || k > 0) ? 1u : 0u);
    }
}

__device__ __forceinline__ void gemm_sync(const WG& c) {
    tmem_st_wait();
    tc_fence_before();
    wg_barrier(c);
}
__device__ __forceinline__ void gemm_finish(WG& c) {
    mbar_wait(c.mbar_mma, c.ph_mma);
    c.ph_mma ^= 1u;
    tc_fence_after();
}
__device__ __forceinline__ void gemm_ts_start(WG& c, uint32_t b_hi, uint32_t b_lo, uint32_t N, uint32_t dcol, bool accumulate = false) {
    gemm_sync(c);
    if (c.lead_warp) {
        tc_fence_after();
        if (elect_one()) {
            issue_ts(c, b_hi, b_lo, N, dcol, accumulate);
            umma_commit(c.mbar_mma);
        }
        __syncwarp();
    }
}
__device__ __forceinline__ void gemm_ts(WG& c, uint32_t b_hi, uint32_t b_lo, uint32_t N, uint32_t dcol, bool accumulate = false) {
    gemm_ts_start(c, b_hi, b_lo, N, dcol, accumulate);
    gemm_finish(c);
}
__device__ __forceinline__ void gemm_ss(WG& c, uint32_t b_hi, uint32_t b_lo, uint32_t N, uint32_t dcol, bool accumulate = false) {
    gemm_sync(c);
    if (c.lead_warp) {
        tc_fence_after();
        mbar_wait(c.mbar_tma, c.ph_tma);
        if (elect_one()) {
            issue_ss(c, b_hi, b_lo, N, dcol, accumulate);
            umma_commit(c.mbar_mma);
        }
        __syncwarp();
    }
    c.ph_tma ^= 1u;
    gemm_finish(c);
}

__device__ __forceinline__ void a_store16(const WG& c, int ks, const float (&v)[16]) {
    uint32_t w[16];
#pragma unroll
    for (int i = 0; i < 8; ++i) split2(v[2 * i], v[2 * i + 1], w[i], w[8 + i]);
    tmem_st16(c.tmem + c.acol + 16 * ks, w);
}

__device__ __forceinline__ float4 lds4(const float* p) { return *reinterpret_cast<const float4*>(p); }
__device__ __forceinline__ void lds16(const float* p, float (&b)[16]) {
#pragma unroll
    for (int i = 0; i < 4; ++i) {
        const float4 x = lds4(p + 4 * i);
        b[4 * i] = x.x; b[4 * i + 1] = x.y; b[4 * i + 2] = x.z; b[4 * i + 3] = x.w;
    }
}

__device__ __forceinline__ float4 ldg4_now(const float* p) {
    float4 v;
    asm volatile("ld.global.nc.v4.f32 {%0, %1, %2, %3}, [%4];" : "=f"(v.x), "=f"(v.y), "=f"(v.z), "=f"(v.w) : "l"(p));
    return v;
}
__device__ __forceinline__ float ldg1_now(const float* p) {
    float v;
    asm volatile("ld.global.nc.f32 %0, [%1];" : "=f"(v) : "l"(p));
    return v;
}
__device__ __forceinline__ int ldgi_now(const int32_t* p) {
    int v;
    asm volatile("ld.global.nc.s32 %0, [%1];" : "=r"(v) : "l"(p));
    return v;
}

template <bool RELU>
__device__ __forceinline__ void epilogue_to_a(const WG& c, uint32_t dcol, const float* __restrict__ bias_s) {
#pragma unroll
    for (int q = 0; q < 4; ++q) {
        float v[16], bb[16];
        tmem_ld16_sync(c.tmem + dcol + q * 16, v);
        lds16(bias_s + q * 16, bb);
#pragma unroll
        for (int j = 0; j < 16; ++j) {
            const float x = v[j] + bb[j];
            v[j] = RELU ? relu_nan(x) : x;
        }
        a_store16(c, q, v);
    }
}

template <int K>
__device__ __forceinline__ void first_layer_to_a(const WG& c, const float (&feat)[K], const float* __restrict__ wt_s,
                                                 const float* __restrict__ bias_s) {
#pragma unroll
    for (int q = 0; q < 4; ++q) {
        float o[16];
        lds16(bias_s + q * 16, o);
#pragma unroll
        for (int k = 0; k < K; ++k) {
            float w[16];
            lds16(wt_s + k * P + q * 16, w);
#pragma unroll
            for (int j = 0; j < 16; ++j) o[j] = fmaf(feat[k], w[j], o[j]);
        }
#pragma unroll
        for (int j = 0; j < 16; ++j) o[j] = relu_nan(o[j]);
        a_store16(c, q, o);
    }
}

template <bool TO_A>
__device__ __forceinline__ bool epilogue_to_mu(const WG& c, uint32_t dcol, const float* __restrict__ bias_s, float rowscale,
                                               bool valid, bool stage = true) {
    bool bad = false;
#pragma unroll
    for (int q = 0; q < 4; ++q) {
        float v[16], bb[16];
        tmem_ld16_sync(c.tmem + dcol + q * 16, v);
        lds16(bias_s + q * 16, bb);
#pragma unroll
        for (int j = 0; j < 16; ++j) {
            v[j] = (v[j] + bb[j]) * rowscale;
            bad |= (v[j] != v[j]);
        }
        uint32_t w[16];
#pragma unroll
        for (int i = 0; i < 8; ++i) split2(v[2 * i], v[2 * i + 1], w[i], w[8 + i]);
#pragma unroll
        for (int h = 0; h < 2 && stage; ++h) {
            const uint32_t off = swz((uint32_t)c.t, (uint32_t)(q * 2 + h));
            asm volatile("st.shared.v4.b32 [%0], {%1, %2, %3, %4};" ::"r"(c.land + off), "r"(w[4 * h]), "r"(w[4 * h + 1]),
                         "r"(w[4 * h + 2]), "r"(w[4 * h + 3]) : "memory");
            asm volatile("st.shared.v4.b32 [%0], {%1, %2, %3, %4};" ::"r"(c.land + APLANE + off), "r"(w[8 + 4 * h]),
                         "r"(w[8 + 4 * h + 1]), "r"(w[8 + 4 * h + 2]), "r"(w[8 + 4 * h + 3]) : "memory");
        }
        if (TO_A) tmem_st16(c.tmem + c.acol + 16 * q, w);
    }
    return bad && valid;
}
__device__ __forceinline__ void commit_tile(const WG& c, void* dst_tile) {
    fence_proxy_async();
    wg_barrier(c);
    if (c.t == 0) bulk_s2g(dst_tile, c.land, ABUF);
}
__device__ __forceinline__ void request_nb(const WG& c, const void* src) {
    if (c.t == 0) {
        bulk_wait_read();
        mbar_expect_tx(c.mbar_tma, ABUF);
        bulk_g2s(c.land, src, ABUF, c.mbar_tma);
    }
}

__device__ __forceinline__ void epilogue_to_rlx(const WG& c, uint32_t dcol, const float* __restrict__ bias_s, float rowscale,
                                                float* __restrict__ dst_tile) {
#pragma unroll
    for (int q = 0; q < 4; ++q) {
        float v[16], bb[16];
        tmem_ld16_sync(c.tmem + dcol + q * 16, v);
        lds16(bias_s + q * 16, bb);
#pragma unroll
        for (int h = 0; h < 4; ++h) {
            const float4 o = make_float4((v[h * 4 + 0] + bb[h * 4 + 0]) * rowscale, (v[h * 4 + 1] + bb[h * 4 + 1]) * rowscale,
                                         (v[h * 4 + 2] + bb[h * 4 + 2]) * rowscale, (v[h * 4 + 3] + bb[h * 4 + 3]) * rowscale);
            *reinterpret_cast<float4*>(dst_tile + ((size_t)(q * 4 + h) * TILE + c.t) * 4) = o;
        }
    }
}

constexpr int NWG = 4;
struct Tail {
    float bias[6][P];
    float w_small[2][8 * P];
    float vec[P];
    uint64_t mbar[1 + 2 * NWG];
    uint32_t tmem_slot;
    int32_t wcnt[NWG][4];
};

struct CtaSetup {
    unsigned char* base;
    uint32_t w;
    Tail* tail;
    uint32_t tmem_base;
};

__device__ __forceinline__ unsigned char* smem_dyn() {
    extern __shared__ unsigned char smem_raw_[];
    return smem_raw_;
}

template <bool LAND, int NW>
__device__ __forceinline__ CtaSetup cta_setup(unsigned char* smem_raw, uint32_t wbytes, const uint16_t* const (&wsrc)[NW],
                                              const uint32_t (&woff)[NW], const uint32_t (&wlen)[NW]) {
    CtaSetup s;
    s.base = smem_raw + ((1024u - (smem_u32(smem_raw) & 1023u)) & 1023u);
    s.w = smem_u32(s.base);
    s.tail = reinterpret_cast<Tail*>(s.base + wbytes + (LAND ? NWG * ABUF : 0));
    if (threadIdx.x == 0) {
        for (int i = 0; i < 1 + 2 * NWG; ++i) mbar_init(smem_u32(&s.tail->mbar[i]), 1);
        fence_mbar_init();
    }
    __syncwarp();
    if (threadIdx.x < 32) tmem_alloc(smem_u32(&s.tail->tmem_slot), 512);
    tc_fence_before();
    __syncthreads();
    tc_fence_after();
    s.tmem_base = s.tail->tmem_slot;
    if (threadIdx.x == 0) {
        const uint32_t mb = smem_u32(&s.tail->mbar[0]);
        uint32_t total = 0;
        for (int i = 0; i < NW; ++i) total += wlen[i];
        mbar_expect_tx(mb, total);
        for (int i = 0; i < NW; ++i) bulk_g2s(s.w + woff[i], wsrc[i], wlen[i], mb);
    }
    return s;
}
__device__ __forceinline__ WG make_wg(const CtaSetup& s, uint32_t wbytes) {
    WG c;
    c.wg = uniform((int)(threadIdx.x >> 7));
    c.lead_warp = (uniform((int)(threadIdx.x >> 5)) & 3) == 0;
    c.t = threadIdx.x & 127;
    c.land = s.w + wbytes + (uint32_t)c.wg * ABUF;
    c.mbar_mma = smem_u32(&s.tail->mbar[1 + 2 * c.wg]);
    c.mbar_tma = smem_u32(&s.tail->mbar[2 + 2 * c.wg]);
    c.ph_mma = 0;
    c.ph_tma = 0;
    c.acol = ACOL;
    c.bar_threads = 128;
    c.tmem0 = ((uint32_t)uniform((int)s.tmem_base) & 0x0000FFFFu) + (uint32_t)c.wg * WG_COLS;
    c.tmem = s.tmem_base + ((uint32_t)((c.t >> 5) * 32) << 16) + (uint32_t)c.wg * WG_COLS;
    return c;
}
__device__ __forceinline__ void cta_teardown(const CtaSetup& s) {
    tc_fence_before();
    __syncthreads();
    if (threadIdx.x < 32) tmem_dealloc(s.tmem_base, 512);
}
__device__ __forceinline__ void copy_vec(float* dst, const float* __restrict__ src, int n, float scale = ASCALE) {
    for (int i = threadIdx.x; i < n; i += blockDim.x) dst[i] = src[i] * scale;
}

constexpr uint32_t UPD_W3 = 0, UPD_WC = 4 * WPLANE, UPD_W42 = 6 * WPLANE, UPD_FN = 8 * WPLANE, UPD_WBYTES = 10 * WPLANE;

struct UpdArgs {
    GnnParams g;
    int backward;
    const float *lb, *ub;
    const uint16_t* nb_img;
    const float* rlx;
    const int32_t* amb_base;
    uint16_t* mu_out;
    float* scores;
    RowMap map;
    int64_t score_stride, score_off;
    int Bc;
    unsigned long long* nan_count;
    NanDoms nan_doms;
};

__device__ __forceinline__ bool nan_watch(const NanDoms& nd, int dom, bool nan_row) {
    if (nan_row && nd.flag != nullptr && atomicExch(nd.flag + nd.dom0 + dom, 1) == 0) nd.list[atomicAdd(nd.count, 1)] = nd.dom0 + dom;
    return nan_row;
}

__device__ __forceinline__ void update_body(const UpdArgs& a, unsigned char* smem_raw, int rank, int nranks, bool pdl = false) {
    const GnnParams& g = a.g;
    const int backward = a.backward;
    const float* __restrict__ lb = a.lb;
    const float* __restrict__ ub = a.ub;
    const uint16_t* __restrict__ nb_img = a.nb_img;
    const float* __restrict__ rlx = a.rlx;
    const int32_t* __restrict__ amb_base = a.amb_base;
    uint16_t* __restrict__ mu_out = a.mu_out;
    float* __restrict__ scores = a.scores;
    const RowMap map = a.map;
    const int64_t score_stride = a.score_stride, score_off = a.score_off;
    const int l3 = backward ? BC3 : FC3, l4b = backward ? BC4_1 : FC4_2, lc = backward ? T_BWD_C : T_FWD_C;
    const uint16_t* const wsrc[4] = {g.tc[l3], g.tcx_w[lc], g.tc[l4b], g.tc[FNODE]};
    const uint32_t woff[4] = {UPD_W3, UPD_WC, UPD_W42, UPD_FN};
    const uint32_t wlen[4] = {4 * WPLANE, 2 * WPLANE, 2 * WPLANE, 2 * WPLANE};
    CtaSetup s = cta_setup<true, 4>(smem_raw, UPD_WBYTES, wsrc, woff, wlen);
    Tail& tl = *s.tail;
    copy_vec(tl.bias[0], g.bias[l3], P); copy_vec(tl.bias[1], g.tcx_b[lc], P); copy_vec(tl.bias[2], g.bias[l4b], P);
    copy_vec(tl.bias[3], g.bias[FNODE], P); copy_vec(tl.vec, g.wt[FSCORE], P, 1.0f);
    const float bscore = g.bias[FSCORE][0];
    __syncthreads();
    mbar_wait(smem_u32(&tl.mbar[0]), 0);
    if (pdl) { pdl_trigger(); pdl_wait(); }
    WG c = make_wg(s, UPD_WBYTES);
    const uint32_t W = s.w;
    const int tiles_per_dom = map.nslots / TILE;
    const int64_t nitems = (int64_t)tiles_per_dom * ((a.Bc + NWG - 1) / NWG);
    bool bad = false;
    GNNB_TR_DECL;
    int64_t nrow_n = -1;
    float l_n = 0.f, u_n = 1.f;
    int slot0_n = 0;
    auto fetch_row = [&](int64_t it) {
        nrow_n = -1; l_n = 0.f; u_n = 1.f; slot0_n = 0;
        if (it >= nitems) return;
        const int d = (int)(it / tiles_per_dom) * NWG + c.wg;
        if (d >= a.Bc) return;
        const int64_t tl_ = (int64_t)d * tiles_per_dom + it % tiles_per_dom;
        nrow_n = natural_row(map, tl_ * TILE + c.t);
        if (nrow_n >= 0) { l_n = ldg1_now(lb + nrow_n); u_n = ldg1_now(ub + nrow_n); }
        slot0_n = __ldg(amb_base + tl_);
    };
    fetch_row(rank);
    for (int64_t item = rank; item < nitems; item += nranks) {
        const int dom = (int)(item / tiles_per_dom) * NWG + c.wg;
        const int64_t nrow = nrow_n;
        const float l = l_n, u = u_n;
        const int slot0 = slot0_n;
        if (dom >= a.Bc) {
            fetch_row(item + nranks);
            continue;
        }
        const int64_t tile = (int64_t)dom * tiles_per_dom + item % tiles_per_dom;
        const int64_t row0 = tile * TILE, grow = row0 + c.t;
        request_nb(c, nb_img + (size_t)tile * (ABUF / 2));
        fetch_row(item + nranks);
        const Ratio q = compute_ratio(l, u);
        const float gate = (q.r0 != 0.0f) ? 1.0f : 0.0f;
        const bool amb = (q.amb != 0.0f) && nrow >= 0;
        const unsigned bal = __ballot_sync(0xffffffffu, amb);
        if ((c.t & 31) == 0) tl.wcnt[c.wg][c.t >> 5] = __popc(bal);
        GNNB_TR(0);
        gemm_ss(c, W + UPD_W3, W + UPD_W3 + 2 * WPLANE, 128, 0);
        GNNB_TR(1);
        if (c.t == 0 && item + nranks < nitems) {
            const int64_t nitem = item + nranks;
            const int ndom = (int)(nitem / tiles_per_dom) * NWG + c.wg;
            if (ndom < a.Bc) prefetch_l2(nb_img + (size_t)((int64_t)ndom * tiles_per_dom + nitem % tiles_per_dom) * (ABUF / 2), ABUF);
        }
        int slot = slot0 + __popc(bal & ((1u << (c.t & 31)) - 1u));
#pragma unroll
        for (int w = 0; w < 3; ++w) slot += (w < (c.t >> 5)) ? tl.wcnt[c.wg][w] : 0;
        const float* rt = rlx + (size_t)(slot >> 7) * (TILE * P) + (size_t)(slot & (TILE - 1)) * 4;
        if (amb) {
#pragma unroll
            for (int i = 0; i < 16; ++i) asm volatile("prefetch.global.L2 [%0];" ::"l"(rt + (size_t)i * (TILE * 4)));
        }
#pragma unroll
        for (int qd = 0; qd < 4; ++qd) {
            float a[16], b[16], bb[16];
            {
                uint32_t ra[16], rb[16];
                tmem_ld16(c.tmem + qd * 16, ra);
                tmem_ld16(c.tmem + 64 + qd * 16, rb);
                tmem_wait16(ra, a);
                tmem_wait16(rb, b);
            }
            lds16(tl.bias[0] + qd * 16, bb);
#pragma unroll
            for (int j = 0; j < 16; ++j) a[j] = relu_nan(fmaf(q.r0, a[j], fmaf(q.r1, b[j], bb[j])));
            a_store16(c, qd, a);
        }
        GNNB_TR(2);
        gemm_ts_start(c, W + UPD_WC, W + UPD_WC + WPLANE, 64, DCOL);
        float4 rx[16];
        {
#pragma unroll
            for (int i = 0; i < 16; ++i) rx[i] = amb ? ldg4_now(rt + (size_t)i * (TILE * 4)) : make_float4(0.f, 0.f, 0.f, 0.f);
        }
        gemm_finish(c);
        GNNB_TR(3);
#pragma unroll
        for (int qd = 0; qd < 4; ++qd) {
            float v[16], bb[16];
            tmem_ld16_sync(c.tmem + DCOL + qd * 16, v);
            lds16(tl.bias[1] + qd * 16, bb);
#pragma unroll
            for (int h = 0; h < 4; ++h) {
                const float4 x = rx[qd * 4 + h];
                v[h * 4 + 0] = relu_nan(v[h * 4 + 0] + x.x + bb[h * 4 + 0]);
                v[h * 4 + 1] = relu_nan(v[h * 4 + 1] + x.y + bb[h * 4 + 1]);
                v[h * 4 + 2] = relu_nan(v[h * 4 + 2] + x.z + bb[h * 4 + 2]);
                v[h * 4 + 3] = relu_nan(v[h * 4 + 3] + x.w + bb[h * 4 + 3]);
            }
            a_store16(c, qd, v);
        }
        GNNB_TR(4);
        gemm_ts(c, W + UPD_W42, W + UPD_W42 + WPLANE, 64, DCOL);
        GNNB_TR(5);
        if (scores == nullptr) {
            bad |= nan_watch(a.nan_doms, dom, epilogue_to_mu<false>(c, DCOL, tl.bias[2], gate, nrow >= 0));
            commit_tile(c, mu_out + (size_t)tile * (ABUF / 2));
        } else {
            bad |= nan_watch(a.nan_doms, dom, epilogue_to_mu<true>(c, DCOL, tl.bias[2], gate, nrow >= 0, mu_out != nullptr));
            if (mu_out != nullptr) commit_tile(c, mu_out + (size_t)tile * (ABUF / 2));
            gemm_ts(c, W + UPD_FN, W + UPD_FN + WPLANE, 64, DCOL);
            float sc = 0.f;
#pragma unroll
            for (int qd = 0; qd < 4; ++qd) {
                float v[16], bb[16], ww[16];
                tmem_ld16_sync(c.tmem + DCOL + qd * 16, v);
                lds16(tl.bias[3] + qd * 16, bb);
                lds16(tl.vec + qd * 16, ww);
#pragma unroll
                for (int j = 0; j < 16; ++j) sc = fmaf(relu_nan(v[j] + bb[j]), ww[j], sc);
            }
            if (nrow >= 0) scores[(nrow / map.n) * score_stride + score_off + (nrow % map.n)] = fmaf(sc, AINV, bscore);
        }
        GNNB_TR(6);
        GNNB_TR_NEXT();
    }
    GNNB_TR_PRINT("update[top gemm1 epi1 gemm2 epi2 gemm3 epi3]", 7);
    if (bad) atomicAdd(a.nan_count, 1ULL);
    if (c.t == 0) bulk_wait_all();
    cta_teardown(s);
}

__global__ void __launch_bounds__(128 * NWG, 1) k_tc_update(UpdArgs a) {
    update_body(a, smem_dyn(), (int)blockIdx.x, (int)gridDim.x, true);
}

namespace fz {
constexpr int PD = 2;
constexpr int CW = 2;
constexpr int NS_MAX = 8;
constexpr uint32_t W_KS = 8192;
constexpr uint32_t B_ROWS = 16;
constexpr uint32_t B_DOM = B_ROWS * 128;
constexpr uint32_t B_PLANE = PD * B_DOM;
constexpr uint32_t B_STAGE = 2 * B_PLANE;
constexpr uint32_t STAGE = W_KS + B_STAGE;
constexpr uint32_t STG_PLANE = 32 * 128;
constexpr uint32_t STG_WARP = 2 * STG_PLANE;
constexpr uint32_t STG_BYTES = CW * 4 * STG_WARP;
constexpr uint32_t INF_WN = 0, INF_WI = 2 * WPLANE, INF_B22 = 4 * WPLANE;
constexpr int THREADS = 768;
constexpr int GATHER_WARP0 = 2, GATHER_WARPS = 6, CHAIN_WARP0 = 8;
constexpr uint32_t ACC_COL = 0, ACC_WIN = PD * 64, D_COL = 256, D_WIN = 128;

struct Tail {
    float bias[4][P];
    float vec[P];
    uint64_t wts, full[NS_MAX], empty[NS_MAX], acc_full[2], acc_empty[2], mma[CW];
    uint32_t tmem_slot;
    int32_t wcnt[2 * CW][4];
};
constexpr size_t smem_for(uint32_t wbytes, int staging, int n_stages) {
    return 1024 + wbytes + (size_t)staging * (STG_BYTES / 2) + (size_t)n_stages * STAGE + sizeof(Tail);
}
constexpr size_t SMEM_MAX = 232448;
}

struct FusedArgs {
    UpdArgs u;
    PropPlanDev plan;
    const uint16_t* mu_in;
    uint16_t* nb_dbg;
    int n_stages;
    int mma_group;
    int input_layer;
};

__device__ __forceinline__ void tmem_ld32_sync(uint32_t taddr, float (&v0)[16], float (&v1)[16]) {
    uint32_t r0[16], r1[16];
    tmem_ld16(taddr, r0);
    tmem_ld16(taddr + 16, r1);
    tmem_wait16(r0, v0);
    tmem_wait16(r1, v1);
}

__device__ __forceinline__ void split16(const float (&v)[16], uint32_t (&w)[16]) {
#pragma unroll
    for (int i = 0; i < 8; ++i) split2(v[2 * i], v[2 * i + 1], w[i], w[8 + i]);
}
__device__ __forceinline__ void sts128(uint32_t addr, uint32_t a, uint32_t b, uint32_t c, uint32_t d) {
    asm volatile("st.shared.v4.b32 [%0], {%1, %2, %3, %4};" ::"r"(addr), "r"(a), "r"(b), "r"(c), "r"(d) : "memory");
}

#ifdef GNNB_TRACE
__device__ long long g_e3_trace[4];
#define E3TR(i) do { if (blockIdx.x == 1 && threadIdx.x == fz::CHAIN_WARP0 * 32) { const long long n_ = clock64(); g_e3_trace[i] += n_ - e3t_; e3t_ = n_; } } while (0)
#else
#define E3TR(i) do {} while (0)
#endif
struct NoOp { __device__ __forceinline__ void operator()() const {} };
template <bool TO_A, class Between = NoOp>
__device__ __forceinline__ bool epilogue_to_mu_pair(const WG& c, int h, int pair_bar, uint32_t dcol, const float* __restrict__ bias_s,
                                                    float rowscale, bool valid, unsigned char* img, uint32_t stage, Between between = Between()) {
    bool bad = false;
#ifdef GNNB_TRACE
    long long e3t_ = clock64();
#endif
    const uint32_t rl = (uint32_t)c.t & 31u;
    const bool issuer = h == 0 && rl == 0;
    unsigned char* dst = img + ((uint32_t)c.t >> 5) * fz::STG_PLANE;
    uint32_t lo[TO_A ? 16 : 1];
    if (img != nullptr) {
        if (issuer) bulk_wait_read();
        named_bar(pair_bar, 64);
    }
    E3TR(0);
    {
        float v0[16], v1[16];
        tmem_ld32_sync(c.tmem + dcol + h * 32, v0, v1);
        E3TR(1);
#pragma unroll
        for (int qq = 0; qq < 2; ++qq) {
            float (&v)[16] = qq ? v1 : v0;
            const int q = 2 * h + qq;
            float bb[16];
            lds16(bias_s + q * 16, bb);
#pragma unroll
            for (int j = 0; j < 16; ++j) {
                v[j] = (v[j] + bb[j]) * rowscale;
                bad |= (v[j] != v[j]);
            }
            uint32_t w[16];
            split16(v, w);
            if (img != nullptr) {
                const uint32_t o0 = stage + swz(rl, (uint32_t)(2 * q)), o1 = stage + swz(rl, (uint32_t)(2 * q + 1));
                sts128(o0, w[0], w[1], w[2], w[3]);
                sts128(o1, w[4], w[5], w[6], w[7]);
                if (!TO_A) {
                    sts128(o0 + fz::STG_PLANE, w[8], w[9], w[10], w[11]);
                    sts128(o1 + fz::STG_PLANE, w[12], w[13], w[14], w[15]);
                }
            }
            if (TO_A) {
#pragma unroll
                for (int i = 0; i < 8; ++i) lo[qq * 8 + i] = w[8 + i];
                tmem_st16(c.tmem + c.acol + 16 * q, w);
            }
        }
    }
    E3TR(2);
    if (!TO_A) between();
    if (img != nullptr) {
        fence_proxy_async();
        named_bar(pair_bar, 64);
        if (!TO_A) {
            if (issuer) {
                bulk_s2g_nocommit(dst, stage, fz::STG_PLANE);
                bulk_s2g_nocommit(dst + APLANE, stage + fz::STG_PLANE, fz::STG_PLANE);
                bulk_commit();
            }
        } else {
            if (issuer) { bulk_s2g(dst, stage, fz::STG_PLANE); bulk_wait_read(); }
            named_bar(pair_bar, 64);
#pragma unroll
            for (int qq = 0; qq < 2; ++qq) {
                const int q = 2 * h + qq;
                sts128(stage + swz(rl, (uint32_t)(2 * q)), lo[qq * 8], lo[qq * 8 + 1], lo[qq * 8 + 2], lo[qq * 8 + 3]);
                sts128(stage + swz(rl, (uint32_t)(2 * q + 1)), lo[qq * 8 + 4], lo[qq * 8 + 5], lo[qq * 8 + 6], lo[qq * 8 + 7]);
            }
            fence_proxy_async();
            named_bar(pair_bar, 64);
            if (issuer) bulk_s2g(dst + APLANE, stage, fz::STG_PLANE);
        }
    }
    E3TR(3);
    return bad && valid;
}

struct ItemCursor {
    int pair, tile, dq, dr, ntiles, npairs;
    __device__ __forceinline__ ItemCursor(int rank, int nranks, int ntiles_, int npairs_)
        : pair(rank / ntiles_), tile(rank % ntiles_), dq(nranks / ntiles_), dr(nranks % ntiles_), ntiles(ntiles_), npairs(npairs_) {}
    __device__ __forceinline__ bool valid() const { return pair < npairs; }
    __device__ __forceinline__ void next() {
        tile += dr; pair += dq;
        if (tile >= ntiles) { tile -= ntiles; ++pair; }
    }
};

template <bool INPUT_LAYER>
__device__ __forceinline__ void fused_body(const FusedArgs& fa) {
    using namespace fz;
    const UpdArgs& a = fa.u;
    const GnnParams& g = a.g;
    const PropPlanDev& plan = fa.plan;
    const bool with_score = a.scores != nullptr;
    const uint32_t wbytes = with_score ? UPD_WBYTES : UPD_FN;
    const int NS = fa.n_stages;
    unsigned char* base = smem_dyn();
    base += (1024u - (smem_u32(base) & 1023u)) & 1023u;
    const uint32_t stg_warp = a.mu_out == nullptr ? 0u : (with_score ? STG_PLANE : STG_WARP), stg_bytes = CW * 4 * stg_warp;
    const uint32_t W = smem_u32(base), stg = W + wbytes, ring = stg + stg_bytes;
    fz::Tail* tl = reinterpret_cast<fz::Tail*>(base + wbytes + stg_bytes + (size_t)NS * STAGE);
    const int warp = uniform((int)(threadIdx.x >> 5)), lane = threadIdx.x & 31;
    if (threadIdx.x == 0) {
        mbar_init(smem_u32(&tl->wts), 1);
        for (int i = 0; i < NS; ++i) { mbar_init(smem_u32(&tl->full[i]), 1 + 32); mbar_init(smem_u32(&tl->empty[i]), 1); }
        for (int i = 0; i < 2; ++i) { mbar_init(smem_u32(&tl->acc_full[i]), 1); mbar_init(smem_u32(&tl->acc_empty[i]), PD); }
        for (int i = 0; i < CW; ++i) mbar_init(smem_u32(&tl->mma[i]), 1);
        fence_mbar_init();
    }
    __syncwarp();
    if (warp == 0) tmem_alloc(smem_u32(&tl->tmem_slot), 512);
    tc_fence_before();
    __syncthreads();
    tc_fence_after();
    const uint32_t tmem_base = tl->tmem_slot;
    const int l3 = a.backward ? BC3 : FC3, l4b = a.backward ? BC4_1 : FC4_2, lc = a.backward ? T_BWD_C : T_FWD_C;
    constexpr bool inp = INPUT_LAYER;
    if (threadIdx.x == 0) {
        const uint32_t mb = smem_u32(&tl->wts);
        if (!inp) {
            mbar_expect_tx(mb, wbytes);
            bulk_g2s(W + UPD_W3, g.tc[l3], 4 * WPLANE, mb);
            bulk_g2s(W + UPD_WC, g.tcx_w[lc], 2 * WPLANE, mb);
            bulk_g2s(W + UPD_W42, g.tc[l4b], 2 * WPLANE, mb);
            if (with_score) bulk_g2s(W + UPD_FN, g.tc[FNODE], 2 * WPLANE, mb);
        } else {
            mbar_expect_tx(mb, 6 * WPLANE);
            bulk_g2s(W + INF_WN, g.tcx_w[T_INP_NB], 2 * WPLANE, mb);
            bulk_g2s(W + INF_WI, g.tcx_w[T_INP_C], 2 * WPLANE, mb);
            bulk_g2s(W + INF_B22, g.tc[INP_B2_2], 2 * WPLANE, mb);
        }
    }
    if (!inp) {
        copy_vec(tl->bias[0], g.bias[l3], P); copy_vec(tl->bias[1], g.tcx_b[lc], P); copy_vec(tl->bias[2], g.bias[l4b], P);
        copy_vec(tl->bias[3], g.bias[FNODE], P); copy_vec(tl->vec, g.wt[FSCORE], P, 1.0f);
    } else {
        copy_vec(tl->bias[0], g.tcx_b[T_INP_C], P); copy_vec(tl->bias[1], g.bias[INP_B2_2], P); copy_vec(tl->bias[2], g.bias[INP_B], P);
        copy_vec(tl->bias[3], g.wt[INP_B], 2 * P);
    }
    __syncthreads();
    pdl_trigger(); pdl_wait();

    const int ntiles = plan.ntiles, npairs = (a.Bc + PD - 1) / PD;
    const int rank = (int)blockIdx.x, nranks = (int)gridDim.x;

    if (warp == 0) {
        if (lane == 0) {
            uint32_t slot = 0, ph = 0;
            for (ItemCursor cur(rank, nranks, ntiles, npairs); cur.valid(); cur.next()) {
                const int ks0 = plan.tile_ks0[cur.tile], ks1 = plan.tile_ks0[cur.tile + 1];
                for (int ks = ks0; ks < ks1; ++ks) {
                    mbar_wait(smem_u32(&tl->empty[slot]), ph ^ 1u);
                    const uint32_t full = smem_u32(&tl->full[slot]);
                    mbar_expect_tx(full, W_KS);
                    bulk_g2s(ring + slot * STAGE, plan.ks_w + (size_t)ks * (W_KS / 2), W_KS, full);
                    if (++slot == (uint32_t)NS) { slot = 0; ph ^= 1u; }
                }
            }
        }
    } else if (warp == 1) {
        const uint32_t idesc = (1u << 4) | (1u << 16) | ((uint32_t)(PD * 64 >> 3) << 17) | ((uint32_t)(TILE >> 4) << 24);
        uint32_t t = 0, it = 0, slot = 0, ph = 0;
        const int group = fa.mma_group;
        const uint64_t d_a_hi = make_desc_nosw(ring, NB_PIECE, 128u), d_a_lo = make_desc_nosw(ring + W_KS / 2, NB_PIECE, 128u);
        const uint64_t d_b_hi = make_desc_mn(ring + W_KS, B_DOM), d_b_lo = make_desc_mn(ring + W_KS + B_PLANE, B_DOM);
        uint32_t lag_slot0 = 0, lag_slot1 = 0, lag_ph0 = 0, lag_ph1 = 0;
        bool have_lag = false, have_prev = false;
#ifdef GNNB_TRACE
        long long t_acc = 0, t_b = 0, t_lag = 0, t_all = clock64(), t0_;
#define FTR_BEGIN() t0_ = clock64()
#define FTR_END(x) x += clock64() - t0_
#else
#define FTR_BEGIN()
#define FTR_END(x)
#endif
        for (ItemCursor cur(rank, nranks, ntiles, npairs); cur.valid(); cur.next(), ++it) {
            const int ks0 = uniform(plan.tile_ks0[cur.tile]), ks1 = uniform(plan.tile_ks0[cur.tile + 1]);
            const uint32_t buf = it & 1u, bufph = (it >> 1) & 1u;
            FTR_BEGIN();
            mbar_wait(smem_u32(&tl->acc_empty[buf]), bufph ^ 1u);
            FTR_END(t_acc);
            tc_fence_after();
            const uint32_t d = (tmem_base & 0x0000FFFFu) + ACC_COL + buf * ACC_WIN;
            uint32_t accum = 0;
            for (int ks = ks0; ks < ks1;) {
                const int n = ks1 - ks < group ? ks1 - ks : group;
                FTR_BEGIN();
                if (have_lag) mbar_wait(smem_u32(&tl->empty[lag_slot0]), lag_ph0);
                FTR_END(t_lag);
                lag_slot0 = lag_slot1; lag_ph0 = lag_ph1; have_lag = have_prev;
                for (int i = 0; i < n; ++i, ++t) {
                    FTR_BEGIN();
                    mbar_wait(smem_u32(&tl->full[slot]), ph);
                    FTR_END(t_b);
                    tc_fence_after();
                    const uint64_t soff = (uint64_t)(slot * (STAGE >> 4));
                    const uint64_t a_hi = d_a_hi + soff, a_lo = d_a_lo + soff, b_hi = d_b_hi + soff, b_lo = d_b_lo + soff;
                    if (elect_one()) {
                        umma(d, a_hi, b_hi, idesc, accum);
                        umma(d, a_lo, b_hi, idesc, 1u);
                        umma(d, a_hi, b_lo, idesc, 1u);
                        umma_commit(smem_u32(&tl->empty[slot]));
                    }
                    __syncwarp();
                    accum = 1u;
                    lag_slot1 = slot; lag_ph1 = ph;
                    if (++slot == (uint32_t)NS) { slot = 0; ph ^= 1u; }
                }
                have_prev = true;
                ks += n;
            }
            if (elect_one()) umma_commit(smem_u32(&tl->acc_full[buf]));
            __syncwarp();
        }
#ifdef GNNB_TRACE
        if (rank == 1 && lane == 0) printf("TRACE fused-mma: items %u ksteps %u total %lld | wait acc_empty %lld, lag %lld, stage full %lld\n", it, t,
                                           clock64() - t_all, t_acc, t_lag, t_b);
#endif
    } else if (warp >= GATHER_WARP0 && warp < GATHER_WARP0 + GATHER_WARPS) {
        const int gw = warp - GATHER_WARP0;
        const int GW = GATHER_WARPS < NS ? GATHER_WARPS : NS;
        const unsigned char* mu_bytes = reinterpret_cast<const unsigned char*>(fa.mu_in);
#ifdef GNNB_TRACE
        long long g_wait = 0, g_all = clock64();
#endif
        uint32_t slot = 0, ph = 0;
        int turn = 0;
        for (ItemCursor cur(rank, nranks, ntiles, npairs); cur.valid(); cur.next()) {
            const int ks0 = __ldg(plan.tile_ks0 + cur.tile), ks1 = __ldg(plan.tile_ks0 + cur.tile + 1);
            const int dm0 = cur.pair * PD;
            const uint32_t jp = (uint32_t)(lane & 7);
            const unsigned char* base0 = mu_bytes + (int64_t)dm0 * (plan.nslots_in >> 7) * (int64_t)ABUF + jp * 16u;
            const uint32_t sz0 = dm0 < a.Bc ? 16u : 0u, sz1 = dm0 + 1 < a.Bc ? 16u : 0u;
            const unsigned char* base1 = sz1 ? base0 + (int64_t)(plan.nslots_in >> 7) * (int64_t)ABUF : base0;
            for (int ks = ks0; ks < ks1; ++ks) {
                const uint32_t slot_ = slot, ph_ = ph;
                const bool mine = turn == gw;
                if (++slot == (uint32_t)NS) { slot = 0; ph ^= 1u; }
                if (++turn == GW) turn = 0;
                if (!mine) continue;
                const int idx = __ldg(plan.ks_rows + (size_t)ks * 16 + (lane & 15));
                const int off = idx < 0 ? -1 : (idx << 7) + ((idx >> 7) << 14);
#ifdef GNNB_TRACE
                const long long g0_ = clock64();
#endif
                mbar_wait(smem_u32(&tl->empty[slot_]), ph_ ^ 1u);
#ifdef GNNB_TRACE
                g_wait += clock64() - g0_;
#endif
                const uint32_t dst0 = ring + slot_ * STAGE + W_KS;
#pragma unroll
                for (int q = 0; q < 4; ++q) {
                    const int k = q * 4 + (lane >> 3);
                    const int o = __shfl_sync(0xffffffffu, off, k);
                    const bool ok = o >= 0;
                    const uint32_t oo = ok ? (uint32_t)o : 0u, r7 = (oo >> 7) & 7u;
                    const uint32_t dst = dst0 + swz((uint32_t)k, jp ^ r7);
                    const uint32_t z0 = ok ? sz0 : 0u, z1 = ok ? sz1 : 0u;
                    cp_async16_sz(dst, base0 + oo, z0);
                    cp_async16_sz(dst + B_PLANE, base0 + oo + APLANE, z0);
                    cp_async16_sz(dst + B_DOM, base1 + oo, z1);
                    cp_async16_sz(dst + B_DOM + B_PLANE, base1 + oo + APLANE, z1);
                }
                cp_async_arrive(smem_u32(&tl->full[slot_]));
            }
        }
#ifdef GNNB_TRACE
        if (rank == 1 && gw == 0 && lane == 0) printf("TRACE fused-gather: total %lld, wait stage empty %lld\n", clock64() - g_all, g_wait);
#endif
    } else if (warp >= CHAIN_WARP0) {
        const float* __restrict__ lb = a.lb;
        const float* __restrict__ ub = a.ub;
        const float* __restrict__ rlx = a.rlx;
        const int32_t* __restrict__ amb_base = a.amb_base;
        float* __restrict__ scores = a.scores;
        const RowMap map = a.map;
        const float bscore = g.bias[FSCORE][0];
        const int cw = warp - CHAIN_WARP0;
        const int j = uniform(cw >> 3), h = uniform((cw >> 2) & 1);
        WG c;
        c.wg = j;
        c.bar_threads = 256;
        c.lead_warp = (cw & 7) == 0;
        c.t = threadIdx.x & 127;
        c.land = 0;
        c.mbar_mma = smem_u32(&tl->mma[j]);
        c.mbar_tma = 0;
        c.ph_mma = 0;
        c.ph_tma = 0;
        c.acol = ACC_COL;
        c.tmem0 = (uint32_t)uniform((int)tmem_base) & 0x0000FFFFu;
        c.tmem = tmem_base + ((uint32_t)((c.t >> 5) * 32) << 16);
        const uint32_t D = D_COL + D_WIN * (uint32_t)j;
        const int pw = j * 4 + (cw & 3);
        const uint32_t stage = stg + (uint32_t)pw * stg_warp;
        const int pair_bar = 3 + pw;
        const int Q0 = 2 * h;
        mbar_wait(smem_u32(&tl->wts), 0);
        bool bad = false;
        int node_n = -1, node_nn = -1;
        float l_n = 0.f, u_n = 1.f;
        int slot0_n = 0;
        auto fetch_node = [&](const ItemCursor& cu) -> int {
            if (!cu.valid() || cu.pair * PD + j >= a.Bc) return -1;
            return ldgi_now(map.node_of_slot + cu.tile * TILE + c.t);
        };
        auto fetch_bounds = [&](const ItemCursor& cu, int node_) {
            node_n = node_; l_n = 0.f; u_n = 1.f; slot0_n = 0;
            if (!cu.valid()) return;
            const int d_ = cu.pair * PD + j;
            if (d_ >= a.Bc) return;
            if (node_ >= 0) { l_n = ldg1_now(lb + (int64_t)d_ * map.n + node_); u_n = ldg1_now(ub + (int64_t)d_ * map.n + node_); }
            if (amb_base != nullptr) slot0_n = ldgi_now(amb_base + (int64_t)d_ * ntiles + cu.tile);
        };
        ItemCursor cur(rank, nranks, ntiles, npairs), cur1 = cur, cur2 = cur;
        cur1.next();
        cur2.next(); cur2.next();
        fetch_bounds(cur, fetch_node(cur));
        node_nn = fetch_node(cur1);
        uint32_t it = 0;
#ifdef GNNB_TRACE
        long long c_wait = 0, c_ph[8] = {0, 0, 0, 0, 0, 0, 0, 0}, c_all = clock64(), c0_;
        int c_tiles = 0;
#define CTR(i) do { const long long n_ = clock64(); c_ph[i] += n_ - c0_; c0_ = n_; } while (0)
#else
#define CTR(i) do {} while (0)
#endif
        auto start_item = [&](const ItemCursor& cu, uint32_t it_, int node_, float l_, float u_) -> bool {
            const uint32_t buf = it_ & 1u, bufph = (it_ >> 1) & 1u;
            const int dom_ = cu.pair * PD + j;
#ifdef GNNB_TRACE
            const long long w0_ = clock64();
#endif
            mbar_wait(smem_u32(&tl->acc_full[buf]), bufph);
#ifdef GNNB_TRACE
            c_wait += clock64() - w0_;
#endif
            tc_fence_after();
            if (dom_ >= a.Bc) {
                if (h == 0 && c.t == 0) mbar_arrive(smem_u32(&tl->acc_empty[buf]));
                return false;
            }
            const int64_t tile = (int64_t)dom_ * ntiles + cu.tile;
            c.acol = ACC_COL + buf * ACC_WIN + 64u * (uint32_t)j;
            {
                unsigned char* dbg = fa.nb_dbg ? reinterpret_cast<unsigned char*>(fa.nb_dbg) + tile * (int64_t)ABUF + (uint32_t)c.t * 16u : nullptr;
                float v0[16], v1[16];
                tmem_ld32_sync(c.tmem + c.acol + h * 32, v0, v1);
#pragma unroll
                for (int qq = 0; qq < 2; ++qq) {
                    const int qd = Q0 + qq;
                    uint32_t w[16];
                    split16(qq ? v1 : v0, w);
                    tmem_st16(c.tmem + c.acol + 16 * qd, w);
                    if (dbg != nullptr) {
#pragma unroll
                        for (int hh = 0; hh < 2; ++hh) {
                            const uint32_t off = (uint32_t)(qd * 2 + hh) * NB_PIECE;
                            *reinterpret_cast<uint4*>(dbg + off) = make_uint4(w[4 * hh], w[4 * hh + 1], w[4 * hh + 2], w[4 * hh + 3]);
                            *reinterpret_cast<uint4*>(dbg + APLANE + off) = make_uint4(w[8 + 4 * hh], w[8 + 4 * hh + 1], w[8 + 4 * hh + 2], w[8 + 4 * hh + 3]);
                        }
                    }
                }
            }
            if (inp) {
                {
                    const float* w0 = &tl->bias[3][0];
#pragma unroll
                    for (int qq = 0; qq < 2; ++qq) {
                        const int qd = Q0 + qq;
                        float o[16], wl[16], wu[16];
                        lds16(tl->bias[2] + qd * 16, o);
                        lds16(w0 + qd * 16, wl);
                        lds16(w0 + P + qd * 16, wu);
#pragma unroll
                        for (int i = 0; i < 16; ++i) o[i] = relu_nan(fmaf(node_ >= 0 ? l_ : 0.f, wl[i], fmaf(node_ >= 0 ? u_ : 0.f, wu[i], o[i])));
                        uint32_t w[16];
                        split16(o, w);
                        tmem_st16(c.tmem + D + 64 + 16 * qd, w);
                    }
                }
                gemm_sync(c);
                if (c.lead_warp) {
                    tc_fence_after();
                    if (elect_one()) {
                        WG c2 = c;
                        c2.acol = D + 64;
                        issue_ts(c, W + INF_WN, W + INF_WN + WPLANE, 64, D, false);
                        issue_ts(c2, W + INF_WI, W + INF_WI + WPLANE, 64, D, true);
                        umma_commit(c.mbar_mma);
                    }
                    __syncwarp();
                }
            } else {
                gemm_ts_start(c, W + UPD_W3, W + UPD_W3 + 2 * WPLANE, 128, D);
            }
            return true;
        };
        bool have = cur.valid() ? start_item(cur, 0, node_n, l_n, u_n) : false;
        for (; cur.valid(); cur.next(), cur1.next(), cur2.next(), ++it) {
            const uint32_t buf = it & 1u;
            const uint32_t acc_empty = smem_u32(&tl->acc_empty[buf]);
            const int dom = cur.pair * PD + j;
            const int node = node_n;
            const float l = l_n, u = u_n;
            const int slot0 = slot0_n;
            fetch_bounds(cur1, node_nn);
            node_nn = fetch_node(cur2);
            auto advance = [&]() { have = cur1.valid() ? start_item(cur1, it + 1, node_n, l_n, u_n) : false; };
            if (!have) {
                advance();
                continue;
            }
            const int64_t tile = (int64_t)dom * ntiles + cur.tile;
#ifdef GNNB_TRACE
            c0_ = clock64(); ++c_tiles;
#endif
            const Ratio q = compute_ratio(l, u);
            const float gate = (q.r0 != 0.0f) ? 1.0f : 0.0f;
            const bool amb = (q.amb != 0.0f) && node >= 0;
            const unsigned bal = __ballot_sync(0xffffffffu, amb);
            if ((c.t & 31) == 0) tl->wcnt[j * 2 + h][c.t >> 5] = __popc(bal);
            unsigned char* img = a.mu_out ? reinterpret_cast<unsigned char*>(a.mu_out) + tile * (int64_t)ABUF : nullptr;
            if (inp) {
                gemm_finish(c);
                if (h == 0 && c.t == 0) mbar_arrive(acc_empty);
                c.acol = D + 64;
                CTR(1);
                {
                    float v0[16], v1[16];
                    tmem_ld32_sync(c.tmem + D + h * 32, v0, v1);
#pragma unroll
                    for (int qq = 0; qq < 2; ++qq) {
                        float (&v)[16] = qq ? v1 : v0;
                        const int qd = Q0 + qq;
                        float bb[16];
                        lds16(tl->bias[0] + qd * 16, bb);
#pragma unroll
                        for (int i = 0; i < 16; ++i) v[i] = relu_nan(v[i] + bb[i]);
                        a_store16(c, qd, v);
                    }
                }
                CTR(2);
                gemm_ts_start(c, W + INF_B22, W + INF_B22 + WPLANE, 64, D);
                gemm_finish(c);
                CTR(3);
                bad |= nan_watch(a.nan_doms, dom, epilogue_to_mu_pair<false>(c, h, pair_bar, D, tl->bias[1], 1.0f, node >= 0, img, stage, advance));
                CTR(6);
                continue;
            }
            gemm_finish(c);
            if (h == 0 && c.t == 0) mbar_arrive(acc_empty);
            c.acol = D + 64;
            CTR(1);
#pragma unroll
            for (int qq = 0; qq < 2; ++qq) {
                const int qd = Q0 + qq;
                float x[16], y[16], bb[16];
                {
                    uint32_t ra[16], rb[16];
                    tmem_ld16(c.tmem + D + qd * 16, ra);
                    tmem_ld16(c.tmem + D + 64 + qd * 16, rb);
                    tmem_wait16(ra, x);
                    tmem_wait16(rb, y);
                }
                lds16(tl->bias[0] + qd * 16, bb);
#pragma unroll
                for (int i = 0; i < 16; ++i) x[i] = relu_nan(fmaf(q.r0, x[i], fmaf(q.r1, y[i], bb[i])));
                a_store16(c, qd, x);
            }
            CTR(2);
            gemm_ts_start(c, W + UPD_WC, W + UPD_WC + WPLANE, 64, D);
            int slot = slot0 + __popc(bal & ((1u << (c.t & 31)) - 1u));
#pragma unroll
            for (int w = 0; w < 3; ++w) slot += (w < (c.t >> 5)) ? tl->wcnt[j * 2 + h][w] : 0;
            const float* rt = rlx + (size_t)(slot >> 7) * (TILE * P) + (size_t)(slot & (TILE - 1)) * 4 + (size_t)(8 * h) * (TILE * 4);
            float4 rx[8];
#pragma unroll
            for (int i = 0; i < 8; ++i) rx[i] = amb ? ldg4_now(rt + (size_t)i * (TILE * 4)) : make_float4(0.f, 0.f, 0.f, 0.f);
            gemm_finish(c);
            CTR(3);
            {
                float v0[16], v1[16];
                tmem_ld32_sync(c.tmem + D + h * 32, v0, v1);
#pragma unroll
                for (int qq = 0; qq < 2; ++qq) {
                    float (&v)[16] = qq ? v1 : v0;
                    const int qd = Q0 + qq;
                    float bb[16];
                    lds16(tl->bias[1] + qd * 16, bb);
#pragma unroll
                    for (int hh = 0; hh < 4; ++hh) {
                        const float4 x = rx[qq * 4 + hh];
                        v[hh * 4 + 0] = relu_nan(v[hh * 4 + 0] + x.x + bb[hh * 4 + 0]);
                        v[hh * 4 + 1] = relu_nan(v[hh * 4 + 1] + x.y + bb[hh * 4 + 1]);
                        v[hh * 4 + 2] = relu_nan(v[hh * 4 + 2] + x.z + bb[hh * 4 + 2]);
                        v[hh * 4 + 3] = relu_nan(v[hh * 4 + 3] + x.w + bb[hh * 4 + 3]);
                    }
                    a_store16(c, qd, v);
                }
            }
            CTR(4);
            gemm_ts_start(c, W + UPD_W42, W + UPD_W42 + WPLANE, 64, D);
            gemm_finish(c);
            CTR(5);
            if (!with_score) {
                bad |= nan_watch(a.nan_doms, dom, epilogue_to_mu_pair<false>(c, h, pair_bar, D, tl->bias[2], gate, node >= 0, img, stage, advance));
            } else {
                bad |= nan_watch(a.nan_doms, dom, epilogue_to_mu_pair<true>(c, h, pair_bar, D, tl->bias[2], gate, node >= 0, img, stage));
                gemm_ts_start(c, W + UPD_FN, W + UPD_FN + WPLANE, 64, D);
                gemm_finish(c);
                float sc = 0.f;
                {
                    float v0[16], v1[16];
                    tmem_ld32_sync(c.tmem + D + h * 32, v0, v1);
#pragma unroll
                    for (int qq = 0; qq < 2; ++qq) {
                        const int qd = Q0 + qq;
                        float bb[16], ww[16];
                        lds16(tl->bias[3] + qd * 16, bb);
                        lds16(tl->vec + qd * 16, ww);
#pragma unroll
                        for (int i = 0; i < 16; ++i) sc = fmaf(relu_nan((qq ? v1 : v0)[i] + bb[i]), ww[i], sc);
                    }
                }
                if (h == 1) {
                    tmem_st1(c.tmem + D + 64, __float_as_uint(sc));
                    tmem_st_wait();
                }
                tc_fence_before();
                wg_barrier(c);
                tc_fence_after();
                if (h == 0) {
                    sc += __uint_as_float(tmem_ld1_sync(c.tmem + D + 64));
                    if (node >= 0) scores[(int64_t)dom * a.score_stride + a.score_off + node] = fmaf(sc, AINV, bscore);
                }
                advance();
            }
            CTR(6);
        }
#ifdef GNNB_TRACE
        if (rank == 1 && threadIdx.x == CHAIN_WARP0 * 32)
            printf("TRACE fused-chain wg0: tiles %d total %lld | wait acc_full %lld | per tile: convert %lld gemm1 %lld epi1 %lld gemm2 %lld epi2 %lld gemm3 %lld epi3 %lld\n",
                   c_tiles, clock64() - c_all, c_wait, c_ph[0] / max(c_tiles, 1), c_ph[1] / max(c_tiles, 1), c_ph[2] / max(c_tiles, 1), c_ph[3] / max(c_tiles, 1),
                   c_ph[4] / max(c_tiles, 1), c_ph[5] / max(c_tiles, 1), c_ph[6] / max(c_tiles, 1));
        if (rank == 1 && threadIdx.x == CHAIN_WARP0 * 32) {
            printf("TRACE fused-e3 (cumulative over launches): wait prev store %lld, tmem load %lld, compute + stage %lld, fence + issue %lld\n",
                   g_e3_trace[0], g_e3_trace[1], g_e3_trace[2], g_e3_trace[3]);
        }
#endif
        if (bad) atomicAdd(a.nan_count, 1ULL);
        if (h == 0 && (c.t & 31) == 0) bulk_wait_all();
    }
    tc_fence_before();
    __syncthreads();
    if (warp == 0) tmem_dealloc(tmem_base, 512);
}

__global__ void __launch_bounds__(fz::THREADS, 1) k_tc_fused(FusedArgs fa) { fused_body<false>(fa); }
__global__ void __launch_bounds__(fz::THREADS, 1) k_tc_fused_input(FusedArgs fa) { fused_body<true>(fa); }

constexpr uint32_t RLX_FR = 0, RLX_BC11 = 2 * WPLANE, RLX_BC12 = 4 * WPLANE, RLX_BC2 = 6 * WPLANE, RLX_BR = 12 * WPLANE;
constexpr uint32_t RLX_WBYTES = 14 * WPLANE;

struct RelaxLayers {
    NodeInputs in[AMB_MAX_LAYERS];
    float* rlx_f[AMB_MAX_LAYERS];
    float* rlx_b[AMB_MAX_LAYERS];
    int n;
};

__global__ void __launch_bounds__(128 * NWG, 1) k_tc_relax(GnnParams g, const __grid_constant__ RelaxLayers rl) {
    const uint16_t* const wsrc[5] = {g.tcx_w[T_FWD_R], g.tc[BC1_1], g.tc[BC1_2], g.tc[BC2], g.tcx_w[T_BWD_R]};
    const uint32_t woff[5] = {RLX_FR, RLX_BC11, RLX_BC12, RLX_BC2, RLX_BR};
    const uint32_t wlen[5] = {2 * WPLANE, 2 * WPLANE, 2 * WPLANE, 6 * WPLANE, 2 * WPLANE};
    CtaSetup s = cta_setup<false, 5>(smem_dyn(), RLX_WBYTES, wsrc, woff, wlen);
    Tail& tl = *s.tail;
    copy_vec(tl.bias[0], g.tcx_b[T_FWD_R], P); copy_vec(tl.bias[1], g.bias[BC1_1], P); copy_vec(tl.bias[2], g.bias[BC1_2], P);
    copy_vec(tl.bias[3], g.bias[BC2], P); copy_vec(tl.bias[4], g.tcx_b[T_BWD_R], P);
    copy_vec(tl.w_small[0], g.wt[FC1], 7 * P); copy_vec(tl.w_small[1], g.wt[BC1], 7 * P);
    copy_vec(tl.bias[5], g.bias[FC1], P); copy_vec(tl.vec, g.bias[BC1], P);
    __syncthreads();
    mbar_wait(smem_u32(&tl.mbar[0]), 0);
    pdl_trigger(); pdl_wait();
    WG c = make_wg(s, RLX_WBYTES);
    const uint32_t W = s.w;
    int tile0[AMB_MAX_LAYERS + 1];
    tile0[0] = 0;
#pragma unroll 1
    for (int k = 0; k < rl.n; ++k) {
        const int namb_k = __ldg(rl.in[k].amb_base + (rl.in[k].rows + TILE - 1) / TILE);
        tile0[k + 1] = tile0[k] + (namb_k + TILE - 1) / TILE;
    }
    const int total_tiles = tile0[rl.n];
    int k = 0;
    for (int gt = (int)blockIdx.x * NWG + c.wg; gt < total_tiles; gt += (int)gridDim.x * NWG) {
        while (gt >= tile0[k + 1]) ++k;
        const NodeInputs& in = rl.in[k];
        float* __restrict__ rlx_f = rl.rlx_f[k];
        float* __restrict__ rlx_b = rl.rlx_b[k];
        const int64_t tile = gt - tile0[k];
        const int64_t namb = __ldg(in.amb_base + (in.rows + TILE - 1) / TILE);
        const int64_t slot = tile * TILE + c.t;
        float l = 0.f, u = 1.f, d1 = 0.f, d2 = 0.f, pp = 0.f, po = 0.f, bs = 0.f;
        if (slot < namb) {
            const int64_t grow = natural_row(in.map, __ldg(in.amb_rows + slot));
            l = in.lb[grow]; u = in.ub[grow];
            d1 = in.dual[grow * 3 + 1]; d2 = in.dual[grow * 3 + 2];
            pp = in.prim_pre[grow]; po = in.prim_post[grow];
            bs = in.bias_node[grow % in.map.n];
        }
        const Ratio q = compute_ratio(l, u);
        {
            const float feat[7] = {q.beta, l, u, d1 - d2, pp, po, bs};
            first_layer_to_a<7>(c, feat, tl.w_small[0], tl.bias[5]);
        }
        gemm_ts(c, W + RLX_FR, W + RLX_FR + WPLANE, 64, DCOL);
        epilogue_to_rlx(c, DCOL, tl.bias[0], q.amb, rlx_f + (size_t)tile * (TILE * P));
        {
            const float feat[7] = {l, u, q.beta, -d2 + d1, po, pp, bs};
            first_layer_to_a<7>(c, feat, tl.w_small[1], tl.vec);
        }
        gemm_ts(c, W + RLX_BC11, W + RLX_BC11 + WPLANE, 64, DCOL);
        epilogue_to_a<true>(c, DCOL, tl.bias[1]);
        gemm_ts(c, W + RLX_BC12, W + RLX_BC12 + WPLANE, 64, DCOL);
        epilogue_to_a<false>(c, DCOL, tl.bias[2]);
        float acc[64];
        gemm_ts(c, W + RLX_BC2, W + RLX_BC2 + 3 * WPLANE, 64, DCOL);
#pragma unroll
        for (int qd = 0; qd < 4; ++qd) {
            float v[16], bb[16];
            tmem_ld16_sync(c.tmem + DCOL + qd * 16, v);
            lds16(tl.bias[3] + qd * 16, bb);
#pragma unroll
            for (int j = 0; j < 16; ++j) acc[qd * 16 + j] = v[j] + bb[j];
        }
        gemm_ts(c, W + RLX_BC2 + WPLANE, W + RLX_BC2 + 4 * WPLANE, 64, DCOL);
        {
            const float nd2 = -d2;
#pragma unroll
            for (int qd = 0; qd < 4; ++qd) {
                float v[16];
                tmem_ld16_sync(c.tmem + DCOL + qd * 16, v);
#pragma unroll
                for (int j = 0; j < 16; ++j) acc[qd * 16 + j] = fmaf(nd2, v[j], acc[qd * 16 + j]);
            }
        }
        gemm_ts(c, W + RLX_BC2 + 2 * WPLANE, W + RLX_BC2 + 5 * WPLANE, 64, DCOL);
#pragma unroll
        for (int qd = 0; qd < 4; ++qd) {
            float v[16];
            tmem_ld16_sync(c.tmem + DCOL + qd * 16, v);
#pragma unroll
            for (int j = 0; j < 16; ++j) v[j] = relu_nan(fmaf(d1, v[j], acc[qd * 16 + j]));
            a_store16(c, qd, v);
        }
        gemm_ts(c, W + RLX_BR, W + RLX_BR + WPLANE, 64, DCOL);
        epilogue_to_rlx(c, DCOL, tl.bias[4], q.amb, rlx_b + (size_t)tile * (TILE * P));
    }
    cta_teardown(s);
}

constexpr uint32_t EMB_WBYTES = 2 * WPLANE;

__global__ void __launch_bounds__(128 * NWG, 1) k_tc_input_embed(GnnParams g, const float* __restrict__ lb0,
                                                                 const float* __restrict__ x, const float* __restrict__ ub0,
                                                                 uint16_t* __restrict__ mu0, RowMap map, int64_t rows) {
    const uint16_t* const wsrc[1] = {g.tc[INP_F_1]};
    const uint32_t woff[1] = {0};
    const uint32_t wlen[1] = {2 * WPLANE};
    CtaSetup s = cta_setup<true, 1>(smem_dyn(), EMB_WBYTES, wsrc, woff, wlen);
    Tail& tl = *s.tail;
    copy_vec(tl.bias[0], g.bias[INP_F_1], P); copy_vec(tl.bias[5], g.bias[INP_F], P); copy_vec(tl.w_small[0], g.wt[INP_F], 3 * P);
    __syncthreads();
    mbar_wait(smem_u32(&tl.mbar[0]), 0);
    pdl_trigger(); pdl_wait();
    WG c = make_wg(s, EMB_WBYTES);
    const int64_t ntiles = (rows + TILE - 1) / TILE;
    for (int64_t tile = (int64_t)blockIdx.x * NWG + c.wg; tile < ntiles; tile += (int64_t)gridDim.x * NWG) {
        const int64_t row0 = tile * TILE, grow = row0 + c.t;
        float feat[3] = {0.f, 0.f, 0.f};
        const int64_t nrow = grow < rows ? natural_row(map, grow) : -1;
        if (nrow >= 0) { feat[0] = lb0[nrow]; feat[1] = x[nrow]; feat[2] = ub0[nrow]; }
        first_layer_to_a<3>(c, feat, tl.w_small[0], tl.bias[5]);
        if (c.t == 0) bulk_wait_read();
        gemm_ts(c, s.w, s.w + WPLANE, 64, DCOL);
        epilogue_to_mu<false>(c, DCOL, tl.bias[0], 1.0f, nrow >= 0);
        commit_tile(c, mu0 + (size_t)tile * (ABUF / 2));
    }
    if (c.t == 0) bulk_wait_all();
    cta_teardown(s);
}

constexpr uint32_t INU_WI = 0, INU_WN = 2 * WPLANE, INU_B22 = 4 * WPLANE, INU_WBYTES = 6 * WPLANE;

__global__ void __launch_bounds__(128 * NWG, 1) k_tc_input_update(GnnParams g, const float* __restrict__ lb0,
                                                                  const float* __restrict__ ub0, const uint16_t* __restrict__ nb_img,
                                                                  uint16_t* __restrict__ mu0, RowMap map, int64_t rows) {
    const uint16_t* const wsrc[3] = {g.tcx_w[T_INP_C], g.tcx_w[T_INP_NB], g.tc[INP_B2_2]};
    const uint32_t woff[3] = {INU_WI, INU_WN, INU_B22};
    const uint32_t wlen[3] = {2 * WPLANE, 2 * WPLANE, 2 * WPLANE};
    CtaSetup s = cta_setup<true, 3>(smem_dyn(), INU_WBYTES, wsrc, woff, wlen);
    Tail& tl = *s.tail;
    copy_vec(tl.bias[0], g.tcx_b[T_INP_C], P); copy_vec(tl.bias[1], g.bias[INP_B2_2], P);
    copy_vec(tl.bias[5], g.bias[INP_B], P); copy_vec(tl.w_small[0], g.wt[INP_B], 2 * P);
    __syncthreads();
    mbar_wait(smem_u32(&tl.mbar[0]), 0);
    pdl_trigger(); pdl_wait();
    WG c = make_wg(s, INU_WBYTES);
    const uint32_t W = s.w;
    const int64_t ntiles = (rows + TILE - 1) / TILE;
    const int64_t tile_step = (int64_t)gridDim.x * NWG;
    for (int64_t tile = (int64_t)blockIdx.x * NWG + c.wg; tile < ntiles; tile += tile_step) {
        const int64_t row0 = tile * TILE, grow = row0 + c.t;
        request_nb(c, nb_img + (size_t)tile * (ABUF / 2));
        float feat[2] = {0.f, 0.f};
        const int64_t nrow = grow < rows ? natural_row(map, grow) : -1;
        if (nrow >= 0) { feat[0] = lb0[nrow]; feat[1] = ub0[nrow]; }
        first_layer_to_a<2>(c, feat, tl.w_small[0], tl.bias[5]);
        gemm_sync(c);
        if (c.lead_warp) {
            tc_fence_after();
            if (elect_one()) issue_ts(c, W + INU_WI, W + INU_WI + WPLANE, 64, DCOL, false);
            __syncwarp();
            mbar_wait(c.mbar_tma, c.ph_tma);
            if (elect_one()) {
                issue_ss(c, W + INU_WN, W + INU_WN + WPLANE, 64, DCOL, true);
                umma_commit(c.mbar_mma);
            }
            __syncwarp();
        }
        c.ph_tma ^= 1u;
        gemm_finish(c);
        epilogue_to_a<true>(c, DCOL, tl.bias[0]);
        gemm_ts(c, W + INU_B22, W + INU_B22 + WPLANE, 64, DCOL);
        epilogue_to_mu<false>(c, DCOL, tl.bias[1], 1.0f, nrow >= 0);
        commit_tile(c, mu0 + (size_t)tile * (ABUF / 2));
    }
    if (c.t == 0) bulk_wait_all();
    cta_teardown(s);
}

constexpr size_t smem_bytes(uint32_t wbytes, bool land) { return 1024 + wbytes + (land ? NWG * ABUF : 0) + sizeof(Tail); }

int grid_for(int64_t rows) {
    const int64_t tiles = (rows + TILE - 1) / TILE, ctas = (tiles + NWG - 1) / NWG;
    return (int)(ctas < 1 ? 1 : (ctas < 148 ? ctas : 148));
}

__global__ void k_unpack_tile_image(const uint16_t* __restrict__ img, float* __restrict__ out, RowMap map, int64_t rows,
                                    int piece_major) {
    const int64_t i = (int64_t)blockIdx.x * blockDim.x + threadIdx.x;
    if (i >= rows * 8) return;
    const int64_t row = i >> 3;
    const int64_t nrow = natural_row(map, row);
    if (nrow < 0) return;
    const int chunk = (int)(i & 7);
    const int64_t tile = row / TILE;
    const uint32_t r = (uint32_t)(row % TILE);
    const uint32_t off = piece_major ? (uint32_t)chunk * NB_PIECE + r * 16u : swz(r, (uint32_t)chunk);
    const __half* hi = reinterpret_cast<const __half*>(img) + tile * (ABUF / 2) + off / 2;
    const __half* lo = hi + APLANE / 2;
    for (int j = 0; j < 8; ++j) out[nrow * P + chunk * 8 + j] = (__half2float(hi[j]) + __half2float(lo[j])) * AINV;
}

__device__ __forceinline__ bool row_is_ambiguous(const float* __restrict__ lb, const float* __restrict__ ub, const RowMap& map,
                                                 int64_t row, int64_t rows) {
    const int64_t nrow = row < rows ? natural_row(map, row) : -1;
    return nrow >= 0 && compute_ratio(lb[nrow], ub[nrow]).amb != 0.0f;
}
__global__ void __launch_bounds__(TILE) k_amb_count(const float* __restrict__ lb, const float* __restrict__ ub, RowMap map,
                                                    int64_t rows, int32_t* __restrict__ cnt) {
    const int64_t row = (int64_t)blockIdx.x * TILE + threadIdx.x;
    const bool amb = row_is_ambiguous(lb, ub, map, row, rows);
    const int total = __syncthreads_count(amb);
    if (threadIdx.x == 0) cnt[blockIdx.x] = total;
}
__global__ void __launch_bounds__(1024) k_amb_scan(const int32_t* __restrict__ cnt, int32_t* __restrict__ base, int n) {
    __shared__ int32_t part[1024];
    const int per = (n + 1023) / 1024, lo = threadIdx.x * per, hi = min(n, lo + per);
    int32_t sum = 0;
    for (int i = lo; i < hi; ++i) sum += cnt[i];
    part[threadIdx.x] = sum;
    __syncthreads();
    for (int off = 1; off < 1024; off <<= 1) {
        const int32_t v = threadIdx.x >= off ? part[threadIdx.x - off] : 0;
        __syncthreads();
        part[threadIdx.x] += v;
        __syncthreads();
    }
    int32_t run = part[threadIdx.x] - sum;
    for (int i = lo; i < hi; ++i) { base[i] = run; run += cnt[i]; }
    if (threadIdx.x == 1023) base[n] = part[1023];
}
__global__ void __launch_bounds__(TILE) k_amb_fill(const float* __restrict__ lb, const float* __restrict__ ub, RowMap map,
                                                   int64_t rows, const int32_t* __restrict__ base, int32_t* __restrict__ amb_rows) {
    __shared__ int32_t wc[4];
    const int64_t row = (int64_t)blockIdx.x * TILE + threadIdx.x;
    const bool amb = row_is_ambiguous(lb, ub, map, row, rows);
    const unsigned bal = __ballot_sync(0xffffffffu, amb);
    const int lane = threadIdx.x & 31, warp = threadIdx.x >> 5;
    if (lane == 0) wc[warp] = __popc(bal);
    __syncthreads();
    int slot = base[blockIdx.x] + __popc(bal & ((1u << lane) - 1u));
    for (int w = 0; w < warp; ++w) slot += wc[w];
    if (amb) amb_rows[slot] = (int32_t)row;
}

__device__ __forceinline__ int amb_layer_of(const AmbLayers& a, int tile) {
    int k = 0;
    while (k + 1 < a.n && tile >= a.tile0[k + 1]) ++k;
    return k;
}
__global__ void __launch_bounds__(TILE) k_amb_count_all(AmbLayers a) {
    const int k = amb_layer_of(a, (int)blockIdx.x), tile = (int)blockIdx.x - a.tile0[k];
    const int64_t row = (int64_t)tile * TILE + threadIdx.x;
    const bool amb = row_is_ambiguous(a.lb[k], a.ub[k], a.map[k], row, a.rows[k]);
    const int total = __syncthreads_count(amb);
    if (threadIdx.x == 0) a.cnt[k][tile] = total;
}
__global__ void __launch_bounds__(1024) k_amb_scan_all(AmbLayers a) {
    __shared__ int32_t part[1024];
    const int k = blockIdx.x, n = a.tile0[k + 1] - a.tile0[k];
    const int32_t* __restrict__ cnt = a.cnt[k];
    int32_t* __restrict__ base = a.base[k];
    const int per = (n + 1023) / 1024, lo = threadIdx.x * per, hi = min(n, lo + per);
    int32_t sum = 0;
    for (int i = lo; i < hi; ++i) sum += cnt[i];
    part[threadIdx.x] = sum;
    __syncthreads();
    for (int off = 1; off < 1024; off <<= 1) {
        const int32_t v = threadIdx.x >= off ? part[threadIdx.x - off] : 0;
        __syncthreads();
        part[threadIdx.x] += v;
        __syncthreads();
    }
    int32_t run = part[threadIdx.x] - sum;
    for (int i = lo; i < hi; ++i) { base[i] = run; run += cnt[i]; }
    if (threadIdx.x == 1023) base[n] = part[1023];
}
__global__ void __launch_bounds__(TILE) k_amb_fill_all(AmbLayers a) {
    __shared__ int32_t wc[4];
    const int k = amb_layer_of(a, (int)blockIdx.x), tile = (int)blockIdx.x - a.tile0[k];
    const int64_t row = (int64_t)tile * TILE + threadIdx.x;
    const bool amb = row_is_ambiguous(a.lb[k], a.ub[k], a.map[k], row, a.rows[k]);
    const unsigned bal = __ballot_sync(0xffffffffu, amb);
    const int lane = threadIdx.x & 31, warp = threadIdx.x >> 5;
    if (lane == 0) wc[warp] = __popc(bal);
    __syncthreads();
    int slot = a.base[k][tile] + __popc(bal & ((1u << lane) - 1u));
    for (int w = 0; w < warp; ++w) slot += wc[w];
    if (amb) a.out_rows[k][slot] = (int32_t)row;
}

}

void amb_compact_all(AmbLayers a, cudaStream_t st, int64_t* launches) {
    a.tile0[0] = 0;
    for (int k = 0; k < a.n; ++k) a.tile0[k + 1] = a.tile0[k] + (int)((a.rows[k] + TILE - 1) / TILE);
    k_amb_count_all<<<a.tile0[a.n], TILE, 0, st>>>(a);
    k_amb_scan_all<<<a.n, 1024, 0, st>>>(a);
    k_amb_fill_all<<<a.tile0[a.n], TILE, 0, st>>>(a);
    *launches += 3;
}

void amb_compact(const float* lb, const float* ub, RowMap map, int64_t rows, int32_t* cnt, int32_t* amb_base, int32_t* amb_rows,
                 cudaStream_t st, int64_t* launches) {
    const int ntiles = (int)((rows + TILE - 1) / TILE);
    k_amb_count<<<ntiles, TILE, 0, st>>>(lb, ub, map, rows, cnt);
    k_amb_scan<<<1, 1024, 0, st>>>(cnt, amb_base, ntiles);
    k_amb_fill<<<ntiles, TILE, 0, st>>>(lb, ub, map, rows, amb_base, amb_rows);
    *launches += 3;
}

bool tc_available() { return true; }

int tc_init() {
    cudaError_t e;
    if ((e = cudaFuncSetAttribute(k_tc_update, cudaFuncAttributeMaxDynamicSharedMemorySize, (int)smem_bytes(UPD_WBYTES, true))) != cudaSuccess) return e;
    if ((e = cudaFuncSetAttribute(k_tc_fused, cudaFuncAttributeMaxDynamicSharedMemorySize, (int)fz::SMEM_MAX)) != cudaSuccess) return e;
    if ((e = cudaFuncSetAttribute(k_tc_fused_input, cudaFuncAttributeMaxDynamicSharedMemorySize, (int)fz::SMEM_MAX)) != cudaSuccess) return e;
    if ((e = cudaFuncSetAttribute(k_tc_relax, cudaFuncAttributeMaxDynamicSharedMemorySize, (int)smem_bytes(RLX_WBYTES, false))) != cudaSuccess) return e;
    if ((e = cudaFuncSetAttribute(k_tc_input_embed, cudaFuncAttributeMaxDynamicSharedMemorySize, (int)smem_bytes(EMB_WBYTES, true))) != cudaSuccess) return e;
    if ((e = cudaFuncSetAttribute(k_tc_input_update, cudaFuncAttributeMaxDynamicSharedMemorySize, (int)smem_bytes(INU_WBYTES, true))) != cudaSuccess) return e;
    return 0;
}

int64_t tc_packed_elems(int K) { return (int64_t)2 * (K / 64) * 64 * 64; }

int64_t tc_pack_weight(const float* w, int K, uint16_t* dst) {
    const int nblk = K / 64;
    for (int n = 0; n < 64; ++n)
        for (int k = 0; k < K; ++k) {
            uint16_t hi, lo;
            split_host(w[(size_t)n * K + k], hi, lo);
            const int kb = k / 64, kk = k % 64;
            const size_t e = (size_t)(swz((uint32_t)n, (uint32_t)(kk / 8)) + (kk % 8) * 2) / 2;
            dst[(size_t)kb * 4096 + e] = hi;
            dst[(size_t)(nblk + kb) * 4096 + e] = lo;
        }
    return tc_packed_elems(K);
}

void tc_relax(const GnnParams& g, const NodeInputs* in, float* const* relax_f, float* const* relax_b, int n_layers, cudaStream_t st,
              int64_t* launches) {
    RelaxLayers rl;
    rl.n = n_layers;
    int64_t rows = 0;
    for (int k = 0; k < n_layers; ++k) { rl.in[k] = in[k]; rl.rlx_f[k] = relax_f[k]; rl.rlx_b[k] = relax_b[k]; rows += in[k].rows; }
    launch_pdl(k_tc_relax, grid_for(rows), 128 * NWG, smem_bytes(RLX_WBYTES, false), st, g, rl);
    ++*launches;
}

namespace {
UpdArgs make_upd_args(const GnnParams& g, bool backward, const float* lb, const float* ub, const float* nb, const float* relax,
                      const int32_t* amb_base, float* mu_out, float* scores, RowMap map, int64_t score_stride, int64_t score_off,
                      int64_t rows, unsigned long long* nan_count, const NanDoms& nan_doms) {
    UpdArgs a;
    a.g = g; a.backward = backward ? 1 : 0; a.lb = lb; a.ub = ub; a.nb_img = reinterpret_cast<const uint16_t*>(nb); a.rlx = relax;
    a.amb_base = amb_base; a.mu_out = reinterpret_cast<uint16_t*>(mu_out); a.scores = scores; a.map = map;
    a.score_stride = score_stride; a.score_off = score_off; a.Bc = (int)(rows / map.nslots); a.nan_count = nan_count;
    a.nan_doms = nan_doms;
    return a;
}
}

void tc_update(const GnnParams& g, bool backward, const float* lb, const float* ub, const float* nb, const float* relax,
               const int32_t* amb_base, float* mu_out, float* scores, RowMap map, int64_t score_stride, int64_t score_off, int64_t rows,
               unsigned long long* nan_count, const NanDoms& nan_doms, cudaStream_t st, int64_t* launches) {
    const UpdArgs a = make_upd_args(g, backward, lb, ub, nb, relax, amb_base, mu_out, scores, map, score_stride, score_off, rows, nan_count,
                                    nan_doms);
    const int64_t nitems = (int64_t)(map.nslots / TILE) * ((a.Bc + NWG - 1) / NWG);
    launch_pdl(k_tc_update, (int)(nitems < 1 ? 1 : (nitems < 148 ? nitems : 148)), 128 * NWG, smem_bytes(UPD_WBYTES, true), st, a);
    ++*launches;
}

void tc_fused(const GnnParams& g, const PropPlan* plan, const float* mu_in, bool backward, const float* lb, const float* ub,
              const float* relax, const int32_t* amb_base, float* mu_out, float* scores, RowMap map, int64_t score_stride, int64_t score_off,
              int64_t rows, unsigned long long* nan_count, const NanDoms& nan_doms, float* nb_dbg, bool input_layer, cudaStream_t st,
              int64_t* launches) {
    FusedArgs fa;
    fa.input_layer = input_layer ? 1 : 0;
    fa.u = make_upd_args(g, backward, lb, ub, nullptr, relax, amb_base, mu_out, scores, map, score_stride, score_off, rows, nan_count,
                         nan_doms);
    fa.plan = prop_plan_dev(plan);
    fa.mu_in = reinterpret_cast<const uint16_t*>(mu_in);
    fa.nb_dbg = reinterpret_cast<uint16_t*>(nb_dbg);
    const uint32_t wbytes = scores ? UPD_WBYTES : UPD_FN;
    const int staging = mu_out == nullptr ? 0 : (scores ? 1 : 2);
    const int ns = (int)((fz::SMEM_MAX - fz::smem_for(wbytes, staging, 0)) / fz::STAGE);
    fa.n_stages = ns > fz::NS_MAX ? fz::NS_MAX : ns;
    fa.mma_group = prop_plan_ksteps_per_tile(plan) >= 48.0 ? 4 : 2;
    if (fa.mma_group > fa.n_stages / 2) fa.mma_group = fa.n_stages / 2;
    const int64_t nitems = (int64_t)fa.plan.ntiles * ((fa.u.Bc + fz::PD - 1) / fz::PD);
    launch_pdl(input_layer ? k_tc_fused_input : k_tc_fused, (int)(nitems < 1 ? 1 : (nitems < 148 ? nitems : 148)), fz::THREADS,
               fz::smem_for(wbytes, staging, fa.n_stages), st, fa);
    ++*launches;
}

void tc_input_embed(const GnnParams& g, const float* lb0, const float* x, const float* ub0, float* mu0, RowMap map, int64_t rows,
                    cudaStream_t st, int64_t* launches) {
    launch_pdl(k_tc_input_embed, grid_for(rows), 128 * NWG, smem_bytes(EMB_WBYTES, true), st, g, lb0, x, ub0, reinterpret_cast<uint16_t*>(mu0), map, rows);
    ++*launches;
}

void tc_input_update(const GnnParams& g, const float* lb0, const float* ub0, const float* nb, float* mu0, RowMap map, int64_t rows,
                     cudaStream_t st, int64_t* launches) {
    launch_pdl(k_tc_input_update, grid_for(rows), 128 * NWG, smem_bytes(INU_WBYTES, true), st,
               g, lb0, ub0, reinterpret_cast<const uint16_t*>(nb), reinterpret_cast<uint16_t*>(mu0), map, (int64_t)rows);
    ++*launches;
}

void tc_unpack_tile_image(const float* img, float* out, RowMap map, int64_t rows, bool piece_major, cudaStream_t st) {
    const int64_t n = rows * 8;
    k_unpack_tile_image<<<(unsigned)((n + 255) / 256), 256, 0, st>>>(reinterpret_cast<const uint16_t*>(img), out, map, rows, piece_major ? 1 : 0);
}

}
```

Measured before the change: 275,100.

## Fold final input-node linear layer into the first forward layer's weights

Precomposes the last linear layer of the input-node embed and input-update paths with the first layer's FC3 weights on the host. mu0 then stores the pre-linear (ReLU) activations, and the folded bias term is applied per node, scaled by the row sums of the first network layer's weights. This drops one tensor-core GEMM and its weight staging from the input embed and input update kernels. In exchange, the first forward layer uses a new fused-fold kernel variant with a wider 2P-input weight, and snapshot unfolding needs an extra debug kernel.

```diff
diff --git a/gnn_branching_b200/csrc/gnnb_api.cu b/gnn_branching_b200/csrc/gnnb_api.cu
--- a/gnn_branching_b200/csrc/gnnb_api.cu
+++ b/gnn_branching_b200/csrc/gnnb_api.cu
@@ -39,6 +39,7 @@
     int kw_iscratch_cap = 0;
     bool have_net = false;
     float* d_net = nullptr;
+    const float* d_fold_s = nullptr;
     std::vector<LayerDev> layers;
     std::vector<PropPlan*> plan_fwd, plan_bwd;
     std::vector<PropPlan*> plan_kw_own;
@@ -292,12 +293,18 @@
     return GNNB_OK;
 }
 
-int snap_img(gnnb_ctx* ctx, bool on, const std::string& name, const float* img, int k, int Bc, bool piece_major, cudaStream_t st) {
+int snap_img(gnnb_ctx* ctx, bool on, const std::string& name, const float* img, int k, int Bc, bool piece_major, cudaStream_t st,
+             int unfold = FOLD_NONE) {
     if (!on) return GNNB_OK;
     const int64_t numel = (int64_t)Bc * ctx->n[k] * P;
     if (ctx->math != GNNB_MATH_TC_FP16X3) return snap(ctx, on, name, img, numel, st);
     TRY_(snap(ctx, on, name, img, numel, st));
-    tc_unpack_tile_image(img, ctx->snaps[name].first, ctx->rowmap[k], (int64_t)Bc * ctx->rowmap[k].nslots, piece_major, st);
+    float* out = ctx->snaps[name].first;
+    tc_unpack_tile_image(img, out, ctx->rowmap[k], (int64_t)Bc * ctx->rowmap[k].nslots, piece_major, st);
+    if (unfold != FOLD_NONE) {
+        const int lin = unfold == FOLD_EMBED ? INP_F_1 : INP_B2_2;
+        tc_unfold_rows(out, (int64_t)Bc * ctx->n[k], ctx->n[k], ctx->gp.wt[lin], ctx->gp.bias[lin], k == 0 ? nullptr : ctx->d_fold_s, st);
+    }
     return GNNB_OK;
 }
 
@@ -359,25 +366,29 @@
         if (tc) tc_input_embed(g, in.lb[0], in.pin, in.ub[0], ctx->mu[0], M(0), R(0), st, lc);
         else simt_input_embed(g, in.lb[0], in.pin, in.ub[0], ctx->mu[0], R(0), st, lc);
     }
-    TRY(snap_img(ctx, snaps, "mu0_embed", ctx->mu[0], 0, Bc, false, st));
+    TRY(snap_img(ctx, snaps, "mu0_embed", ctx->mu[0], 0, Bc, false, st, tc ? FOLD_EMBED : FOLD_NONE));
 
     for (int t = 0; t < g.T; ++t) {
         const bool last = (t == g.T - 1);
+        const int fold1 = !tc ? FOLD_NONE : t == 0 ? FOLD_EMBED : FOLD_UPDATE;
         for (int k = 1; k <= L; ++k) {
             const int64_t rows = R(k), nodes = (int64_t)Bc * ctx->n[k];
+            const int fold = k == 1 ? fold1 : FOLD_NONE;
             if (fused) {
                 ProfScope ps(ctx, GNNB_K_LAYER_FWD, nodes, st);
                 tc_fused(g, ctx->plan_fwd[k - 1], ctx->mu[k - 1], false, in.lb[k], in.ub[k], ctx->relax_f[k], ctx->amb_base[k],
-                         ctx->mu[k], nullptr, M(k), 0, 0, rows, ctx->d_nan, nd, ctx->snapshot ? ctx->nb : nullptr, false, st, lc);
+                         ctx->mu[k], nullptr, M(k), 0, 0, rows, ctx->d_nan, nd, ctx->snapshot ? ctx->nb : nullptr, false, fold, ctx->d_fold_s,
+                         st, lc);
             } else {
                 ProfScope ps(ctx, GNNB_K_PROP_FWD, nodes, st);
                 if (tc) prop_tc_run(ctx->plan_fwd[k - 1], ctx->mu[k - 1], ctx->nb, Bc, st, lc);
                 else prop_forward(ctx->layers[k - 1], ctx->mu[k - 1], ctx->nb, Bc, st, lc);
             }
-            TRY(snap_img(ctx, snaps, name("t%d_fwd_nb%d", t, k), ctx->nb, k, Bc, true, st));
+            TRY(snap_img(ctx, snaps, name("t%d_fwd_nb%d", t, k), ctx->nb, k, Bc, true, st, fold));
             if (!fused) {
                 ProfScope ps(ctx, GNNB_K_UPDATE_FWD, nodes, st);
-                if (tc) tc_update(g, false, in.lb[k], in.ub[k], ctx->nb, ctx->relax_f[k], ctx->amb_base[k], ctx->mu[k], nullptr, M(k), 0, 0, rows, ctx->d_nan, nd, st, lc);
+                if (tc) tc_update(g, false, in.lb[k], in.ub[k], ctx->nb, ctx->relax_f[k], ctx->amb_base[k], ctx->mu[k], nullptr, M(k), 0, 0, rows,
+                                  ctx->d_nan, nd, fold, ctx->d_fold_s, st, lc);
                 else simt_update(g, false, in.lb[k], in.ub[k], ctx->nb, ctx->relax_f[k], ctx->mu[k], nullptr, ctx->n[k], 0, 0, rows, ctx->d_nan, st, lc);
             }
             TRY(snap_img(ctx, snaps, name("t%d_fwd_mu%d", t, k), ctx->mu[k], k, Bc, false, st));
@@ -396,7 +407,8 @@
             if (fused_k) {
                 ProfScope ps(ctx, last ? GNNB_K_LAYER_BWD_SCORE : GNNB_K_LAYER_BWD, nodes, st);
                 tc_fused(g, ctx->plan_bwd[k], ctx->mu[k + 1], true, in.lb[k], in.ub[k], ctx->relax_b[k], ctx->amb_base[k],
-                         mu_k, sc, M(k), ctx->n_hidden, ctx->hidden_off[k], rows, ctx->d_nan, nd, ctx->snapshot ? ctx->nb : nullptr, false, st, lc);
+                         mu_k, sc, M(k), ctx->n_hidden, ctx->hidden_off[k], rows, ctx->d_nan, nd, ctx->snapshot ? ctx->nb : nullptr, false, FOLD_NONE,
+                         nullptr, st, lc);
             } else {
                 ProfScope ps(ctx, GNNB_K_PROP_BWD, nodes, st);
                 if (k == L && tc) prop_tc_property_backward(in.wp, ctx->mu[L + 1], ctx->nb, ctx->n[L], ctx->rowmap[L].nslots, Bc, st, lc);
@@ -407,7 +419,8 @@
             TRY(snap_img(ctx, snaps, name("t%d_bwd_nb%d", t, k), ctx->nb, k, Bc, true, st));
             if (!fused_k) {
                 ProfScope ps(ctx, last ? GNNB_K_UPDATE_BWD_SCORE : GNNB_K_UPDATE_BWD, nodes, st);
-                if (tc) tc_update(g, true, in.lb[k], in.ub[k], ctx->nb, ctx->relax_b[k], ctx->amb_base[k], mu_k, sc, M(k), ctx->n_hidden, ctx->hidden_off[k], rows, ctx->d_nan, nd, st, lc);
+                if (tc) tc_update(g, true, in.lb[k], in.ub[k], ctx->nb, ctx->relax_b[k], ctx->amb_base[k], mu_k, sc, M(k), ctx->n_hidden, ctx->hidden_off[k], rows,
+                                  ctx->d_nan, nd, FOLD_NONE, nullptr, st, lc);
                 else simt_update(g, true, in.lb[k], in.ub[k], ctx->nb, ctx->relax_b[k], ctx->mu[k], sc, ctx->n[k], ctx->n_hidden, ctx->hidden_off[k], rows, ctx->d_nan, st, lc);
             }
             TRY(snap_img(ctx, snaps, name("t%d_bwd_mu%d", t, k), ctx->mu[k], k, Bc, false, st));
@@ -415,8 +428,8 @@
         if (!last && fused) {
             ProfScope ps(ctx, GNNB_K_INPUT_UPDATE, (int64_t)Bc * ctx->n[0], st);
             tc_fused(g, ctx->plan_bwd[0], ctx->mu[1], true, in.lb[0], in.ub[0], nullptr, nullptr, ctx->mu[0], nullptr, M(0), 0, 0, R(0),
-                     ctx->d_nan, nd, nullptr, true, st, lc);
-            TRY(snap_img(ctx, snaps, name("t%d_mu0", t, 0), ctx->mu[0], 0, Bc, false, st));
+                     ctx->d_nan, nd, nullptr, true, FOLD_NONE, nullptr, st, lc);
+            TRY(snap_img(ctx, snaps, name("t%d_mu0", t, 0), ctx->mu[0], 0, Bc, false, st, FOLD_UPDATE));
         } else if (!last) {
             {
                 ProfScope ps(ctx, GNNB_K_PROP_BWD, (int64_t)Bc * ctx->n[0], st);
@@ -428,7 +441,7 @@
                 if (tc) tc_input_update(g, in.lb[0], in.ub[0], ctx->nb, ctx->mu[0], M(0), R(0), st, lc);
                 else simt_input_update(g, in.lb[0], in.ub[0], ctx->nb, ctx->mu[0], R(0), st, lc);
             }
-            TRY(snap_img(ctx, snaps, name("t%d_mu0", t, 0), ctx->mu[0], 0, Bc, false, st));
+            TRY(snap_img(ctx, snaps, name("t%d_mu0", t, 0), ctx->mu[0], 0, Bc, false, st, tc ? FOLD_UPDATE : FOLD_NONE));
         }
     }
     {
@@ -562,20 +575,44 @@
     compose(T_BWD_C, BC4, 1, BC3_1, true);
     compose(T_INP_C, INP_B2, 0, INP_B_1, true);
     compose(T_INP_NB, INP_B2, 1, -1, false);
+    std::vector<float> fw((size_t)N_FOLD * P * 2 * P, 0.f), fc((size_t)N_FOLD * 2 * P, 0.f);
+    for (int f = 0; f < N_FOLD; ++f) {
+        const int src = f == FOLD_EMBED ? INP_F_1 : INP_B2_2;
+        const float* W3 = tensors[2 * FC3];
+        const float* Ws = tensors[2 * src];
+        const float* bs = tensors[2 * src + 1];
+        for (int half = 0; half < 2; ++half)
+            for (int nn = 0; nn < P; ++nn) {
+                const float* w3 = W3 + (size_t)nn * 2 * P + half * P;
+                for (int k = 0; k < P; ++k) {
+                    double acc = 0.0;
+                    for (int j = 0; j < P; ++j) acc += (double)w3[j] * (double)Ws[(size_t)j * P + k];
+                    fw[((size_t)f * P + nn) * 2 * P + half * P + k] = (float)acc;
+                }
+                double cacc = 0.0;
+                for (int j = 0; j < P; ++j) cacc += (double)w3[j] * (double)bs[j];
+                fc[(size_t)f * 2 * P + half * P + nn] = (float)cacc;
+            }
+    }
     std::vector<size_t> o_tc(N_LIN, 0);
     size_t tc_total = 0;
     for (int l = 0; l < N_LIN; ++l)
         if (lin_in(l) >= P && lin_out(l) == P) { o_tc[l] = tc_total; tc_total += (size_t)tc_packed_elems(lin_in(l)); }
-    std::vector<size_t> o_tcx(N_TCLIN, 0);
+    std::vector<size_t> o_tcx(N_TCLIN, 0), o_fold(N_FOLD, 0);
     for (int i = 0; i < N_TCLIN; ++i) { o_tcx[i] = tc_total; tc_total += (size_t)tc_packed_elems(P); }
+    for (int f = 0; f < N_FOLD; ++f) { o_fold[f] = tc_total; tc_total += (size_t)tc_packed_elems(2 * P); }
     std::vector<uint16_t> tcblob(tc_total ? tc_total : 1, 0);
     for (int l = 0; l < N_LIN; ++l)
         if (lin_in(l) >= P && lin_out(l) == P) tc_pack_weight(tensors[2 * l], lin_in(l), &tcblob[o_tc[l]]);
     for (int i = 0; i < N_TCLIN; ++i) tc_pack_weight(&cw[(size_t)i * P * P], P, &tcblob[o_tcx[i]]);
+    for (int f = 0; f < N_FOLD; ++f) tc_pack_weight(&fw[(size_t)f * P * 2 * P], 2 * P, &tcblob[o_fold[f]]);
     const size_t o_cb = total;
     total += cb.size();
+    const size_t o_fc = total;
+    total += fc.size();
     blob.resize(total, 0.f);
     memcpy(&blob[o_cb], cb.data(), cb.size() * sizeof(float));
+    memcpy(&blob[o_fc], fc.data(), fc.size() * sizeof(float));
     CU(cudaDeviceSynchronize());
     if (!ctx->d_gnn) CU(cudaMalloc(&ctx->d_gnn, total * sizeof(float)));
     if (!ctx->d_tc) CU(cudaMalloc(&ctx->d_tc, tcblob.size() * sizeof(uint16_t)));
@@ -589,6 +626,10 @@
     for (int i = 0; i < N_TCLIN; ++i) {
         ctx->gp.tcx_w[i] = ctx->d_tc + o_tcx[i];
         ctx->gp.tcx_b[i] = ctx->d_gnn + o_cb + (size_t)i * P;
+    }
+    for (int f = 0; f < N_FOLD; ++f) {
+        ctx->gp.fold_w[f] = ctx->d_tc + o_fold[f];
+        ctx->gp.fold_c[f] = ctx->d_gnn + o_fc + (size_t)f * 2 * P;
     }
     ctx->gp.T = T;
     if (!ctx->d_train) {
@@ -765,7 +806,33 @@
         o_b[k] = total; total += align4(L.n_out);
     }
     n[n_layers + 1] = 1;
+    const size_t o_fold_s = total;
+    total += align4(n[1]);
     std::vector<float> blob(total, 0.f);
+    {
+        const gnnb_layer_desc& d = layers[0];
+        if (d.kind == GNNB_LAYER_CONV) {
+            for (int co = 0; co < d.c_out; ++co)
+                for (int y = 0; y < d.h_out; ++y)
+                    for (int x = 0; x < d.w_out; ++x) {
+                        double acc = 0.0;
+                        for (int ci = 0; ci < d.c_in; ++ci)
+                            for (int ky = 0; ky < d.ksize; ++ky)
+                                for (int kx = 0; kx < d.ksize; ++kx) {
+                                    const int iy = y * d.stride - d.pad + ky, ix = x * d.stride - d.pad + kx;
+                                    if (iy >= 0 && iy < d.h_in && ix >= 0 && ix < d.w_in)
+                                        acc += d.weight[(((size_t)co * d.c_in + ci) * d.ksize + ky) * d.ksize + kx];
+                                }
+                        blob[o_fold_s + ((size_t)co * d.h_out + y) * d.w_out + x] = (float)acc;
+                    }
+        } else {
+            for (int o = 0; o < n[1]; ++o) {
+                double acc = 0.0;
+                for (int i = 0; i < n[0]; ++i) acc += d.weight[(size_t)o * n[0] + i];
+                blob[o_fold_s + o] = (float)acc;
+            }
+        }
+    }
     for (int k = 0; k < n_layers; ++k) {
         const gnnb_layer_desc& d = layers[k];
         const LayerDev& L = devs[k];
@@ -850,7 +917,7 @@
     for (PropPlan* p : ctx->plan_bwd) prop_plan_free(p);
     for (PropPlan* p : ctx->plan_kw_own) prop_plan_free(p);
     sg.keep = true;
-    ctx->d_net = sg.d_net; ctx->d_maps = sg.d_maps; ctx->d_layers = sg.d_layers; ctx->d_hidden_off = sg.d_hidden_off;
+    ctx->d_net = sg.d_net; ctx->d_fold_s = sg.d_net + o_fold_s; ctx->d_maps = sg.d_maps; ctx->d_layers = sg.d_layers; ctx->d_hidden_off = sg.d_hidden_off;
     ctx->d_random_order = sg.d_random_order; ctx->d_ptrs = sg.d_ptrs;
     ctx->plan_fwd = sg.plan_fwd; ctx->plan_bwd = sg.plan_bwd; ctx->plan_kw_own = sg.plan_kw_own;
     ctx->plan_kw.assign(n_layers, nullptr);
diff --git a/gnn_branching_b200/csrc/gnnb_common.cuh b/gnn_branching_b200/csrc/gnnb_common.cuh
--- a/gnn_branching_b200/csrc/gnnb_common.cuh
+++ b/gnn_branching_b200/csrc/gnnb_common.cuh
@@ -34,12 +34,21 @@
     N_TCLIN
 };
 
+enum InFold : int {
+    FOLD_NONE = -1,
+    FOLD_EMBED = 0,
+    FOLD_UPDATE,
+    N_FOLD
+};
+
 struct GnnParams {
     const float* wt[N_LIN];
     const float* bias[N_LIN];
     const uint16_t* tc[N_LIN];
     const uint16_t* tcx_w[N_TCLIN];
     const float* tcx_b[N_TCLIN];
+    const uint16_t* fold_w[N_FOLD];
+    const float* fold_c[N_FOLD];
     int T;
 };
 
@@ -103,12 +112,12 @@
               int64_t* launches);
 void tc_update(const GnnParams& g, bool backward, const float* lb, const float* ub, const float* nb, const float* relax,
                const int32_t* amb_base, float* mu_out, float* scores, RowMap map, int64_t score_stride, int64_t score_off, int64_t rows,
-               unsigned long long* nan_count, const NanDoms& nan_doms, cudaStream_t st, int64_t* launches);
+               unsigned long long* nan_count, const NanDoms& nan_doms, int fold, const float* fold_s, cudaStream_t st, int64_t* launches);
 struct PropPlan;
 void tc_fused(const GnnParams& g, const PropPlan* plan, const float* mu_in, bool backward, const float* lb, const float* ub,
               const float* relax, const int32_t* amb_base, float* mu_out, float* scores, RowMap map, int64_t score_stride, int64_t score_off,
-              int64_t rows, unsigned long long* nan_count, const NanDoms& nan_doms, float* nb_dbg, bool input_layer, cudaStream_t st,
-              int64_t* launches);
+              int64_t rows, unsigned long long* nan_count, const NanDoms& nan_doms, float* nb_dbg, bool input_layer, int fold,
+              const float* fold_s, cudaStream_t st, int64_t* launches);
 void amb_compact(const float* lb, const float* ub, RowMap map, int64_t rows, int32_t* cnt, int32_t* amb_base, int32_t* amb_rows,
                  cudaStream_t st, int64_t* launches);
 constexpr int AMB_MAX_LAYERS = 16;
@@ -133,6 +142,7 @@
 int tc_init();
 bool tc_available();
 void tc_unpack_tile_image(const float* img, float* out, RowMap map, int64_t rows, bool piece_major, cudaStream_t st);
+void tc_unfold_rows(float* x, int64_t rows, int n, const float* wt, const float* bias, const float* s_node, cudaStream_t st);
 
 int prop_init(int max_smem_bytes);
 void prop_forward(const LayerDev& L, const float* mu_prev, float* nb, int Bc, cudaStream_t st, int64_t* launches);
diff --git a/gnn_branching_b200/csrc/gnnb_tc.cu b/gnn_branching_b200/csrc/gnnb_tc.cu
--- a/gnn_branching_b200/csrc/gnnb_tc.cu
+++ b/gnn_branching_b200/csrc/gnnb_tc.cu
@@ -103,6 +103,17 @@
     }
 }
 
+__device__ __forceinline__ void fold_add16(float (&v)[16], const float* c, float s) {
+#pragma unroll
+    for (int i = 0; i < 4; ++i) {
+        const float4 x = lds4(c + 4 * i);
+        v[4 * i + 0] = fmaf(s, x.x, v[4 * i + 0]);
+        v[4 * i + 1] = fmaf(s, x.y, v[4 * i + 1]);
+        v[4 * i + 2] = fmaf(s, x.z, v[4 * i + 2]);
+        v[4 * i + 3] = fmaf(s, x.w, v[4 * i + 3]);
+    }
+}
+
 __device__ __forceinline__ float4 ldg4_now(const float* p) {
     float4 v;
     asm volatile("ld.global.nc.v4.f32 {%0, %1, %2, %3}, [%4];" : "=f"(v.x), "=f"(v.y), "=f"(v.z), "=f"(v.w) : "l"(p));
@@ -155,7 +166,18 @@
     }
 }
 
-template <bool TO_A>
+__device__ __forceinline__ void stage_mu16(const WG& c, int q, const uint32_t (&w)[16]) {
+#pragma unroll
+    for (int h = 0; h < 2; ++h) {
+        const uint32_t off = swz((uint32_t)c.t, (uint32_t)(q * 2 + h));
+        asm volatile("st.shared.v4.b32 [%0], {%1, %2, %3, %4};" ::"r"(c.land + off), "r"(w[4 * h]), "r"(w[4 * h + 1]),
+                     "r"(w[4 * h + 2]), "r"(w[4 * h + 3]) : "memory");
+        asm volatile("st.shared.v4.b32 [%0], {%1, %2, %3, %4};" ::"r"(c.land + APLANE + off), "r"(w[8 + 4 * h]),
+                     "r"(w[8 + 4 * h + 1]), "r"(w[8 + 4 * h + 2]), "r"(w[8 + 4 * h + 3]) : "memory");
+    }
+}
+
+template <bool TO_A, bool RELU = false>
 __device__ __forceinline__ bool epilogue_to_mu(const WG& c, uint32_t dcol, const float* __restrict__ bias_s, float rowscale,
                                                bool valid, bool stage = true) {
     bool bad = false;
@@ -166,20 +188,13 @@
         lds16(bias_s + q * 16, bb);
 #pragma unroll
         for (int j = 0; j < 16; ++j) {
-            v[j] = (v[j] + bb[j]) * rowscale;
+            v[j] = RELU ? relu_nan(v[j] + bb[j]) : (v[j] + bb[j]) * rowscale;
             bad |= (v[j] != v[j]);
         }
         uint32_t w[16];
 #pragma unroll
         for (int i = 0; i < 8; ++i) split2(v[2 * i], v[2 * i + 1], w[i], w[8 + i]);
-#pragma unroll
-        for (int h = 0; h < 2 && stage; ++h) {
-            const uint32_t off = swz((uint32_t)c.t, (uint32_t)(q * 2 + h));
-            asm volatile("st.shared.v4.b32 [%0], {%1, %2, %3, %4};" ::"r"(c.land + off), "r"(w[4 * h]), "r"(w[4 * h + 1]),
-                         "r"(w[4 * h + 2]), "r"(w[4 * h + 3]) : "memory");
-            asm volatile("st.shared.v4.b32 [%0], {%1, %2, %3, %4};" ::"r"(c.land + APLANE + off), "r"(w[8 + 4 * h]),
-                         "r"(w[8 + 4 * h + 1]), "r"(w[8 + 4 * h + 2]), "r"(w[8 + 4 * h + 3]) : "memory");
-        }
+        if (stage) stage_mu16(c, q, w);
         if (TO_A) tmem_st16(c.tmem + c.acol + 16 * q, w);
     }
     return bad && valid;
@@ -302,6 +317,8 @@
     int Bc;
     unsigned long long* nan_count;
     NanDoms nan_doms;
+    int fold;
+    const float* fold_s;
 };
 
 __device__ __forceinline__ bool nan_watch(const NanDoms& nd, int dom, bool nan_row) {
@@ -322,13 +339,15 @@
     const RowMap map = a.map;
     const int64_t score_stride = a.score_stride, score_off = a.score_off;
     const int l3 = backward ? BC3 : FC3, l4b = backward ? BC4_1 : FC4_2, lc = backward ? T_BWD_C : T_FWD_C;
-    const uint16_t* const wsrc[4] = {g.tc[l3], g.tcx_w[lc], g.tc[l4b], g.tc[FNODE]};
+    const bool fold = a.fold != FOLD_NONE;
+    const uint16_t* const wsrc[4] = {fold ? g.fold_w[a.fold] : g.tc[l3], g.tcx_w[lc], g.tc[l4b], g.tc[FNODE]};
     const uint32_t woff[4] = {UPD_W3, UPD_WC, UPD_W42, UPD_FN};
     const uint32_t wlen[4] = {4 * WPLANE, 2 * WPLANE, 2 * WPLANE, 2 * WPLANE};
     CtaSetup s = cta_setup<true, 4>(smem_raw, UPD_WBYTES, wsrc, woff, wlen);
     Tail& tl = *s.tail;
     copy_vec(tl.bias[0], g.bias[l3], P); copy_vec(tl.bias[1], g.tcx_b[lc], P); copy_vec(tl.bias[2], g.bias[l4b], P);
     copy_vec(tl.bias[3], g.bias[FNODE], P); copy_vec(tl.vec, g.wt[FSCORE], P, 1.0f);
+    if (fold) copy_vec(tl.bias[4], g.fold_c[a.fold], 2 * P);
     const float bscore = g.bias[FSCORE][0];
     __syncthreads();
     mbar_wait(smem_u32(&tl.mbar[0]), 0);
@@ -340,23 +359,26 @@
     bool bad = false;
     GNNB_TR_DECL;
     int64_t nrow_n = -1;
-    float l_n = 0.f, u_n = 1.f;
+    float l_n = 0.f, u_n = 1.f, s_n = 0.f;
     int slot0_n = 0;
     auto fetch_row = [&](int64_t it) {
-        nrow_n = -1; l_n = 0.f; u_n = 1.f; slot0_n = 0;
+        nrow_n = -1; l_n = 0.f; u_n = 1.f; s_n = 0.f; slot0_n = 0;
         if (it >= nitems) return;
         const int d = (int)(it / tiles_per_dom) * NWG + c.wg;
         if (d >= a.Bc) return;
         const int64_t tl_ = (int64_t)d * tiles_per_dom + it % tiles_per_dom;
         nrow_n = natural_row(map, tl_ * TILE + c.t);
-        if (nrow_n >= 0) { l_n = ldg1_now(lb + nrow_n); u_n = ldg1_now(ub + nrow_n); }
+        if (nrow_n >= 0) {
+            l_n = ldg1_now(lb + nrow_n); u_n = ldg1_now(ub + nrow_n);
+            if (fold) s_n = ldg1_now(a.fold_s + (nrow_n - (int64_t)d * map.n));
+        }
         slot0_n = __ldg(amb_base + tl_);
     };
     fetch_row(rank);
     for (int64_t item = rank; item < nitems; item += nranks) {
         const int dom = (int)(item / tiles_per_dom) * NWG + c.wg;
         const int64_t nrow = nrow_n;
-        const float l = l_n, u = u_n;
+        const float l = l_n, u = u_n, srow = s_n;
         const int slot0 = slot0_n;
         if (dom >= a.Bc) {
             fetch_row(item + nranks);
@@ -398,6 +420,7 @@
                 tmem_wait16(rb, b);
             }
             lds16(tl.bias[0] + qd * 16, bb);
+            if (fold) { fold_add16(a, tl.bias[4] + qd * 16, srow); fold_add16(b, tl.bias[5] + qd * 16, srow); }
 #pragma unroll
             for (int j = 0; j < 16; ++j) a[j] = relu_nan(fmaf(q.r0, a[j], fmaf(q.r1, b[j], bb[j])));
             a_store16(c, qd, a);
@@ -474,7 +497,7 @@
 constexpr uint32_t STG_PLANE = 32 * 128;
 constexpr uint32_t STG_WARP = 2 * STG_PLANE;
 constexpr uint32_t STG_BYTES = CW * 4 * STG_WARP;
-constexpr uint32_t INF_WN = 0, INF_WI = 2 * WPLANE, INF_B22 = 4 * WPLANE;
+constexpr uint32_t INF_WN = 0, INF_WI = 2 * WPLANE;
 constexpr int THREADS = 768;
 constexpr int GATHER_WARP0 = 2, GATHER_WARPS = 6, CHAIN_WARP0 = 8;
 constexpr uint32_t ACC_COL = 0, ACC_WIN = PD * 64, D_COL = 256, D_WIN = 128;
@@ -525,7 +548,7 @@
 #define E3TR(i) do {} while (0)
 #endif
 struct NoOp { __device__ __forceinline__ void operator()() const {} };
-template <bool TO_A, class Between = NoOp>
+template <bool TO_A, bool RELU = false, class Between = NoOp>
 __device__ __forceinline__ bool epilogue_to_mu_pair(const WG& c, int h, int pair_bar, uint32_t dcol, const float* __restrict__ bias_s,
                                                     float rowscale, bool valid, unsigned char* img, uint32_t stage, Between between = Between()) {
     bool bad = false;
@@ -553,7 +576,7 @@
             lds16(bias_s + q * 16, bb);
 #pragma unroll
             for (int j = 0; j < 16; ++j) {
-                v[j] = (v[j] + bb[j]) * rowscale;
+                v[j] = RELU ? relu_nan(v[j] + bb[j]) : (v[j] + bb[j]) * rowscale;
                 bad |= (v[j] != v[j]);
             }
             uint32_t w[16];
@@ -614,13 +637,13 @@
     }
 };
 
-template <bool INPUT_LAYER>
+template <bool INPUT_LAYER, bool FOLD>
 __device__ __forceinline__ void fused_body(const FusedArgs& fa) {
     using namespace fz;
     const UpdArgs& a = fa.u;
     const GnnParams& g = a.g;
     const PropPlanDev& plan = fa.plan;
-    const bool with_score = a.scores != nullptr;
+    const bool with_score = !FOLD && a.scores != nullptr;
     const uint32_t wbytes = with_score ? UPD_WBYTES : UPD_FN;
     const int NS = fa.n_stages;
     unsigned char* base = smem_dyn();
@@ -644,26 +667,27 @@
     const uint32_t tmem_base = tl->tmem_slot;
     const int l3 = a.backward ? BC3 : FC3, l4b = a.backward ? BC4_1 : FC4_2, lc = a.backward ? T_BWD_C : T_FWD_C;
     constexpr bool inp = INPUT_LAYER;
+    constexpr bool fold = FOLD;
     if (threadIdx.x == 0) {
         const uint32_t mb = smem_u32(&tl->wts);
         if (!inp) {
             mbar_expect_tx(mb, wbytes);
-            bulk_g2s(W + UPD_W3, g.tc[l3], 4 * WPLANE, mb);
+            bulk_g2s(W + UPD_W3, fold ? g.fold_w[a.fold] : g.tc[l3], 4 * WPLANE, mb);
             bulk_g2s(W + UPD_WC, g.tcx_w[lc], 2 * WPLANE, mb);
             bulk_g2s(W + UPD_W42, g.tc[l4b], 2 * WPLANE, mb);
             if (with_score) bulk_g2s(W + UPD_FN, g.tc[FNODE], 2 * WPLANE, mb);
         } else {
-            mbar_expect_tx(mb, 6 * WPLANE);
+            mbar_expect_tx(mb, 4 * WPLANE);
             bulk_g2s(W + INF_WN, g.tcx_w[T_INP_NB], 2 * WPLANE, mb);
             bulk_g2s(W + INF_WI, g.tcx_w[T_INP_C], 2 * WPLANE, mb);
-            bulk_g2s(W + INF_B22, g.tc[INP_B2_2], 2 * WPLANE, mb);
         }
     }
     if (!inp) {
         copy_vec(tl->bias[0], g.bias[l3], P); copy_vec(tl->bias[1], g.tcx_b[lc], P); copy_vec(tl->bias[2], g.bias[l4b], P);
-        copy_vec(tl->bias[3], g.bias[FNODE], P); copy_vec(tl->vec, g.wt[FSCORE], P, 1.0f);
+        if (!fold) { copy_vec(tl->bias[3], g.bias[FNODE], P); copy_vec(tl->vec, g.wt[FSCORE], P, 1.0f); }
+        else copy_vec(tl->bias[3], g.fold_c[a.fold], 2 * P);
     } else {
-        copy_vec(tl->bias[0], g.tcx_b[T_INP_C], P); copy_vec(tl->bias[1], g.bias[INP_B2_2], P); copy_vec(tl->bias[2], g.bias[INP_B], P);
+        copy_vec(tl->bias[0], g.tcx_b[T_INP_C], P); copy_vec(tl->bias[2], g.bias[INP_B], P);
         copy_vec(tl->bias[3], g.wt[INP_B], 2 * P);
     }
     __syncthreads();
@@ -953,27 +977,8 @@
             if (inp) {
                 gemm_finish(c);
                 if (h == 0 && c.t == 0) mbar_arrive(acc_empty);
-                c.acol = D + 64;
                 CTR(1);
-                {
-                    float v0[16], v1[16];
-                    tmem_ld32_sync(c.tmem + D + h * 32, v0, v1);
-#pragma unroll
-                    for (int qq = 0; qq < 2; ++qq) {
-                        float (&v)[16] = qq ? v1 : v0;
-                        const int qd = Q0 + qq;
-                        float bb[16];
-                        lds16(tl->bias[0] + qd * 16, bb);
-#pragma unroll
-                        for (int i = 0; i < 16; ++i) v[i] = relu_nan(v[i] + bb[i]);
-                        a_store16(c, qd, v);
-                    }
-                }
-                CTR(2);
-                gemm_ts_start(c, W + INF_B22, W + INF_B22 + WPLANE, 64, D);
-                gemm_finish(c);
-                CTR(3);
-                bad |= nan_watch(a.nan_doms, dom, epilogue_to_mu_pair<false>(c, h, pair_bar, D, tl->bias[1], 1.0f, node >= 0, img, stage, advance));
+                bad |= nan_watch(a.nan_doms, dom, epilogue_to_mu_pair<false, true>(c, h, pair_bar, D, tl->bias[0], 1.0f, node >= 0, img, stage, advance));
                 CTR(6);
                 continue;
             }
@@ -981,6 +986,7 @@
             if (h == 0 && c.t == 0) mbar_arrive(acc_empty);
             c.acol = D + 64;
             CTR(1);
+            const float srow = (fold && node >= 0) ? ldg1_now(a.fold_s + node) : 0.f;
 #pragma unroll
             for (int qq = 0; qq < 2; ++qq) {
                 const int qd = Q0 + qq;
@@ -993,6 +999,7 @@
                     tmem_wait16(rb, y);
                 }
                 lds16(tl->bias[0] + qd * 16, bb);
+                if (fold) { fold_add16(x, tl->bias[3] + qd * 16, srow); fold_add16(y, tl->vec + qd * 16, srow); }
 #pragma unroll
                 for (int i = 0; i < 16; ++i) x[i] = relu_nan(fmaf(q.r0, x[i], fmaf(q.r1, y[i], bb[i])));
                 a_store16(c, qd, x);
@@ -1085,8 +1092,9 @@
     if (warp == 0) tmem_dealloc(tmem_base, 512);
 }
 
-__global__ void __launch_bounds__(fz::THREADS, 1) k_tc_fused(FusedArgs fa) { fused_body<false>(fa); }
-__global__ void __launch_bounds__(fz::THREADS, 1) k_tc_fused_input(FusedArgs fa) { fused_body<true>(fa); }
+__global__ void __launch_bounds__(fz::THREADS, 1) k_tc_fused(FusedArgs fa) { fused_body<false, false>(fa); }
+__global__ void __launch_bounds__(fz::THREADS, 1) k_tc_fused_fold(FusedArgs fa) { fused_body<false, true>(fa); }
+__global__ void __launch_bounds__(fz::THREADS, 1) k_tc_fused_input(FusedArgs fa) { fused_body<true, false>(fa); }
 
 constexpr uint32_t RLX_FR = 0, RLX_BC11 = 2 * WPLANE, RLX_BC12 = 4 * WPLANE, RLX_BC2 = 6 * WPLANE, RLX_BR = 12 * WPLANE;
 constexpr uint32_t RLX_WBYTES = 14 * WPLANE;
@@ -1189,48 +1197,60 @@
     cta_teardown(s);
 }
 
-constexpr uint32_t EMB_WBYTES = 2 * WPLANE;
-
 __global__ void __launch_bounds__(128 * NWG, 1) k_tc_input_embed(GnnParams g, const float* __restrict__ lb0,
                                                                  const float* __restrict__ x, const float* __restrict__ ub0,
                                                                  uint16_t* __restrict__ mu0, RowMap map, int64_t rows) {
-    const uint16_t* const wsrc[1] = {g.tc[INP_F_1]};
-    const uint32_t woff[1] = {0};
-    const uint32_t wlen[1] = {2 * WPLANE};
-    CtaSetup s = cta_setup<true, 1>(smem_dyn(), EMB_WBYTES, wsrc, woff, wlen);
+    CtaSetup s;
+    s.base = smem_dyn() + ((1024u - (smem_u32(smem_dyn()) & 1023u)) & 1023u);
+    s.w = smem_u32(s.base);
+    s.tail = reinterpret_cast<Tail*>(s.base + NWG * ABUF);
+    s.tmem_base = 0;
     Tail& tl = *s.tail;
-    copy_vec(tl.bias[0], g.bias[INP_F_1], P); copy_vec(tl.bias[5], g.bias[INP_F], P); copy_vec(tl.w_small[0], g.wt[INP_F], 3 * P);
+    copy_vec(tl.bias[5], g.bias[INP_F], P); copy_vec(tl.w_small[0], g.wt[INP_F], 3 * P);
     __syncthreads();
-    mbar_wait(smem_u32(&tl.mbar[0]), 0);
     pdl_trigger(); pdl_wait();
-    WG c = make_wg(s, EMB_WBYTES);
+    WG c = make_wg(s, 0);
     const int64_t ntiles = (rows + TILE - 1) / TILE;
     for (int64_t tile = (int64_t)blockIdx.x * NWG + c.wg; tile < ntiles; tile += (int64_t)gridDim.x * NWG) {
         const int64_t row0 = tile * TILE, grow = row0 + c.t;
         float feat[3] = {0.f, 0.f, 0.f};
         const int64_t nrow = grow < rows ? natural_row(map, grow) : -1;
         if (nrow >= 0) { feat[0] = lb0[nrow]; feat[1] = x[nrow]; feat[2] = ub0[nrow]; }
-        first_layer_to_a<3>(c, feat, tl.w_small[0], tl.bias[5]);
         if (c.t == 0) bulk_wait_read();
-        gemm_ts(c, s.w, s.w + WPLANE, 64, DCOL);
-        epilogue_to_mu<false>(c, DCOL, tl.bias[0], 1.0f, nrow >= 0);
+        wg_barrier(c);
+#pragma unroll
+        for (int q = 0; q < 4; ++q) {
+            float o[16];
+            lds16(tl.bias[5] + q * 16, o);
+#pragma unroll
+            for (int k = 0; k < 3; ++k) {
+                float w[16];
+                lds16(tl.w_small[0] + k * P + q * 16, w);
+#pragma unroll
+                for (int j = 0; j < 16; ++j) o[j] = fmaf(feat[k], w[j], o[j]);
+            }
+            uint32_t w[16];
+#pragma unroll
+            for (int i = 0; i < 8; ++i) split2(relu_nan(o[2 * i]), relu_nan(o[2 * i + 1]), w[i], w[8 + i]);
+            stage_mu16(c, q, w);
+        }
         commit_tile(c, mu0 + (size_t)tile * (ABUF / 2));
     }
     if (c.t == 0) bulk_wait_all();
-    cta_teardown(s);
-}
-
-constexpr uint32_t INU_WI = 0, INU_WN = 2 * WPLANE, INU_B22 = 4 * WPLANE, INU_WBYTES = 6 * WPLANE;
+    __syncthreads();
+}
+
+constexpr uint32_t INU_WI = 0, INU_WN = 2 * WPLANE, INU_WBYTES = 4 * WPLANE;
 
 __global__ void __launch_bounds__(128 * NWG, 1) k_tc_input_update(GnnParams g, const float* __restrict__ lb0,
                                                                   const float* __restrict__ ub0, const uint16_t* __restrict__ nb_img,
                                                                   uint16_t* __restrict__ mu0, RowMap map, int64_t rows) {
-    const uint16_t* const wsrc[3] = {g.tcx_w[T_INP_C], g.tcx_w[T_INP_NB], g.tc[INP_B2_2]};
-    const uint32_t woff[3] = {INU_WI, INU_WN, INU_B22};
-    const uint32_t wlen[3] = {2 * WPLANE, 2 * WPLANE, 2 * WPLANE};
-    CtaSetup s = cta_setup<true, 3>(smem_dyn(), INU_WBYTES, wsrc, woff, wlen);
+    const uint16_t* const wsrc[2] = {g.tcx_w[T_INP_C], g.tcx_w[T_INP_NB]};
+    const uint32_t woff[2] = {INU_WI, INU_WN};
+    const uint32_t wlen[2] = {2 * WPLANE, 2 * WPLANE};
+    CtaSetup s = cta_setup<true, 2>(smem_dyn(), INU_WBYTES, wsrc, woff, wlen);
     Tail& tl = *s.tail;
-    copy_vec(tl.bias[0], g.tcx_b[T_INP_C], P); copy_vec(tl.bias[1], g.bias[INP_B2_2], P);
+    copy_vec(tl.bias[0], g.tcx_b[T_INP_C], P);
     copy_vec(tl.bias[5], g.bias[INP_B], P); copy_vec(tl.w_small[0], g.wt[INP_B], 2 * P);
     __syncthreads();
     mbar_wait(smem_u32(&tl.mbar[0]), 0);
@@ -1260,9 +1280,7 @@
         }
         c.ph_tma ^= 1u;
         gemm_finish(c);
-        epilogue_to_a<true>(c, DCOL, tl.bias[0]);
-        gemm_ts(c, W + INU_B22, W + INU_B22 + WPLANE, 64, DCOL);
-        epilogue_to_mu<false>(c, DCOL, tl.bias[1], 1.0f, nrow >= 0);
+        epilogue_to_mu<false, true>(c, DCOL, tl.bias[0], 1.0f, nrow >= 0);
         commit_tile(c, mu0 + (size_t)tile * (ABUF / 2));
     }
     if (c.t == 0) bulk_wait_all();
@@ -1290,6 +1308,20 @@
     const __half* hi = reinterpret_cast<const __half*>(img) + tile * (ABUF / 2) + off / 2;
     const __half* lo = hi + APLANE / 2;
     for (int j = 0; j < 8; ++j) out[nrow * P + chunk * 8 + j] = (__half2float(hi[j]) + __half2float(lo[j])) * AINV;
+}
+
+__global__ void k_unfold_rows(float* __restrict__ x, int64_t rows, int n, const float* __restrict__ wt, const float* __restrict__ bias,
+                              const float* __restrict__ s_node) {
+    const int64_t row = (int64_t)blockIdx.x * blockDim.x + threadIdx.x;
+    if (row >= rows) return;
+    float* xr = x + row * P;
+    float in[P], out[P];
+    for (int k = 0; k < P; ++k) in[k] = xr[k];
+    const float sc = s_node ? s_node[row % n] : 1.0f;
+    for (int o = 0; o < P; ++o) out[o] = sc * bias[o];
+    for (int k = 0; k < P; ++k)
+        for (int o = 0; o < P; ++o) out[o] = fmaf(in[k], wt[k * P + o], out[o]);
+    for (int o = 0; o < P; ++o) xr[o] = out[o];
 }
 
 __device__ __forceinline__ bool row_is_ambiguous(const float* __restrict__ lb, const float* __restrict__ ub, const RowMap& map,
@@ -1407,9 +1439,10 @@
     cudaError_t e;
     if ((e = cudaFuncSetAttribute(k_tc_update, cudaFuncAttributeMaxDynamicSharedMemorySize, (int)smem_bytes(UPD_WBYTES, true))) != cudaSuccess) return e;
     if ((e = cudaFuncSetAttribute(k_tc_fused, cudaFuncAttributeMaxDynamicSharedMemorySize, (int)fz::SMEM_MAX)) != cudaSuccess) return e;
+    if ((e = cudaFuncSetAttribute(k_tc_fused_fold, cudaFuncAttributeMaxDynamicSharedMemorySize, (int)fz::SMEM_MAX)) != cudaSuccess) return e;
     if ((e = cudaFuncSetAttribute(k_tc_fused_input, cudaFuncAttributeMaxDynamicSharedMemorySize, (int)fz::SMEM_MAX)) != cudaSuccess) return e;
     if ((e = cudaFuncSetAttribute(k_tc_relax, cudaFuncAttributeMaxDynamicSharedMemorySize, (int)smem_bytes(RLX_WBYTES, false))) != cudaSuccess) return e;
-    if ((e = cudaFuncSetAttribute(k_tc_input_embed, cudaFuncAttributeMaxDynamicSharedMemorySize, (int)smem_bytes(EMB_WBYTES, true))) != cudaSuccess) return e;
+    if ((e = cudaFuncSetAttribute(k_tc_input_embed, cudaFuncAttributeMaxDynamicSharedMemorySize, (int)smem_bytes(0, true))) != cudaSuccess) return e;
     if ((e = cudaFuncSetAttribute(k_tc_input_update, cudaFuncAttributeMaxDynamicSharedMemorySize, (int)smem_bytes(INU_WBYTES, true))) != cudaSuccess) return e;
     return 0;
 }
@@ -1449,15 +1482,19 @@
     a.amb_base = amb_base; a.mu_out = reinterpret_cast<uint16_t*>(mu_out); a.scores = scores; a.map = map;
     a.score_stride = score_stride; a.score_off = score_off; a.Bc = (int)(rows / map.nslots); a.nan_count = nan_count;
     a.nan_doms = nan_doms;
+    a.fold = FOLD_NONE;
+    a.fold_s = nullptr;
     return a;
 }
 }
 
 void tc_update(const GnnParams& g, bool backward, const float* lb, const float* ub, const float* nb, const float* relax,
                const int32_t* amb_base, float* mu_out, float* scores, RowMap map, int64_t score_stride, int64_t score_off, int64_t rows,
-               unsigned long long* nan_count, const NanDoms& nan_doms, cudaStream_t st, int64_t* launches) {
-    const UpdArgs a = make_upd_args(g, backward, lb, ub, nb, relax, amb_base, mu_out, scores, map, score_stride, score_off, rows, nan_count,
-                                    nan_doms);
+               unsigned long long* nan_count, const NanDoms& nan_doms, int fold, const float* fold_s, cudaStream_t st, int64_t* launches) {
+    UpdArgs a = make_upd_args(g, backward, lb, ub, nb, relax, amb_base, mu_out, scores, map, score_stride, score_off, rows, nan_count,
+                              nan_doms);
+    a.fold = fold;
+    a.fold_s = fold_s;
     const int64_t nitems = (int64_t)(map.nslots / TILE) * ((a.Bc + NWG - 1) / NWG);
     launch_pdl(k_tc_update, (int)(nitems < 1 ? 1 : (nitems < 148 ? nitems : 148)), 128 * NWG, smem_bytes(UPD_WBYTES, true), st, a);
     ++*launches;
@@ -1465,12 +1502,14 @@
 
 void tc_fused(const GnnParams& g, const PropPlan* plan, const float* mu_in, bool backward, const float* lb, const float* ub,
               const float* relax, const int32_t* amb_base, float* mu_out, float* scores, RowMap map, int64_t score_stride, int64_t score_off,
-              int64_t rows, unsigned long long* nan_count, const NanDoms& nan_doms, float* nb_dbg, bool input_layer, cudaStream_t st,
-              int64_t* launches) {
+              int64_t rows, unsigned long long* nan_count, const NanDoms& nan_doms, float* nb_dbg, bool input_layer, int fold,
+              const float* fold_s, cudaStream_t st, int64_t* launches) {
     FusedArgs fa;
     fa.input_layer = input_layer ? 1 : 0;
     fa.u = make_upd_args(g, backward, lb, ub, nullptr, relax, amb_base, mu_out, scores, map, score_stride, score_off, rows, nan_count,
                          nan_doms);
+    fa.u.fold = fold;
+    fa.u.fold_s = fold_s;
     fa.plan = prop_plan_dev(plan);
     fa.mu_in = reinterpret_cast<const uint16_t*>(mu_in);
     fa.nb_dbg = reinterpret_cast<uint16_t*>(nb_dbg);
@@ -1481,14 +1520,14 @@
     fa.mma_group = prop_plan_ksteps_per_tile(plan) >= 48.0 ? 4 : 2;
     if (fa.mma_group > fa.n_stages / 2) fa.mma_group = fa.n_stages / 2;
     const int64_t nitems = (int64_t)fa.plan.ntiles * ((fa.u.Bc + fz::PD - 1) / fz::PD);
-    launch_pdl(input_layer ? k_tc_fused_input : k_tc_fused, (int)(nitems < 1 ? 1 : (nitems < 148 ? nitems : 148)), fz::THREADS,
+    launch_pdl(input_layer ? k_tc_fused_input : fold != FOLD_NONE ? k_tc_fused_fold : k_tc_fused, (int)(nitems < 1 ? 1 : (nitems < 148 ? nitems : 148)), fz::THREADS,
                fz::smem_for(wbytes, staging, fa.n_stages), st, fa);
     ++*launches;
 }
 
 void tc_input_embed(const GnnParams& g, const float* lb0, const float* x, const float* ub0, float* mu0, RowMap map, int64_t rows,
                     cudaStream_t st, int64_t* launches) {
-    launch_pdl(k_tc_input_embed, grid_for(rows), 128 * NWG, smem_bytes(EMB_WBYTES, true), st, g, lb0, x, ub0, reinterpret_cast<uint16_t*>(mu0), map, rows);
+    launch_pdl(k_tc_input_embed, grid_for(rows), 128 * NWG, smem_bytes(0, true), st, g, lb0, x, ub0, reinterpret_cast<uint16_t*>(mu0), map, rows);
     ++*launches;
 }
 
@@ -1504,4 +1543,8 @@
     k_unpack_tile_image<<<(unsigned)((n + 255) / 256), 256, 0, st>>>(reinterpret_cast<const uint16_t*>(img), out, map, rows, piece_major ? 1 : 0);
 }
 
-}
+void tc_unfold_rows(float* x, int64_t rows, int n, const float* wt, const float* bias, const float* s_node, cudaStream_t st) {
+    k_unfold_rows<<<(unsigned)((rows + 127) / 128), 128, 0, st>>>(x, rows, n, wt, bias, s_node);
+}
+
+}
```

Result: faster. 286,400, median of 6 (+4.1%).
